# Drjay806/PRO-B-GAN

Measured on NVIDIA B200. Metric: generator+discriminator samples/sec (score_triplets pass, bf16 tensor-core mode), higher is better.
Workload: dtype bf16

## Files before the change

pro-b-gan_b200/csrc/gather.cuh:

```cuda
#pragma once
#include <cuda_bf16.h>
#include <stdint.h>

namespace pbg {

struct GatherParams {
  const float* node_emb;
  const float* rel_emb;
  long long N, R;
  int E, Z;
  const long long* heads; long long head_stride;
  const long long* rels;  long long rel_stride;
  const long long* tails; long long tail_stride;
  const float* h; const float* r; const float* t;
  const float* z;
  void* xg; int ldg;
  void* xd; int ldd;
  long long B;
  int* err_flag;
};

template <typename T>
__device__ __forceinline__ void store4(T* dst, float4 v);
template <>
__device__ __forceinline__ void store4<float>(float* dst, float4 v) {
  *reinterpret_cast<float4*>(dst) = v;
}
template <>
__device__ __forceinline__ void store4<__nv_bfloat16>(__nv_bfloat16* dst, float4 v) {
  __nv_bfloat162 lo = __floats2bfloat162_rn(v.x, v.y), hi = __floats2bfloat162_rn(v.z, v.w);
  uint2 w;
  w.x = *reinterpret_cast<uint32_t*>(&lo);
  w.y = *reinterpret_cast<uint32_t*>(&hi);
  *reinterpret_cast<uint2*>(dst) = w;
}

__device__ __forceinline__ float4 ld_stream4(const float* p) {
  float4 v;
  asm volatile("ld.global.nc.L1::no_allocate.v4.f32 {%0, %1, %2, %3}, [%4];"
               : "=f"(v.x), "=f"(v.y), "=f"(v.z), "=f"(v.w) : "l"(p));
  return v;
}

template <typename T>
__global__ void __launch_bounds__(256) gather_concat_kernel(const GatherParams p) {
  const int lane = threadIdx.x & 31;
  const long long warp_global = (static_cast<long long>(blockIdx.x) * blockDim.x + threadIdx.x) >> 5;
  const long long num_warps = (static_cast<long long>(gridDim.x) * blockDim.x) >> 5;
  const int E4 = p.E >> 2, Z4 = p.Z >> 2;
  T* xg = static_cast<T*>(p.xg);
  T* xd = static_cast<T*>(p.xd);

  for (long long b = warp_global; b < p.B; b += num_warps) {
    const float *hrow, *rrow, *trow = nullptr;
    bool bad = false;
    if (p.heads != nullptr) {
      long long i = p.heads[b * p.head_stride];
      if (i < 0) i += p.N;
      if (i < 0 || i >= p.N) { bad = true; i = 0; }
      hrow = p.node_emb + i * p.E;
    } else {
      hrow = p.h + b * p.E;
    }
    if (p.rels != nullptr) {
      long long i = p.rels[b * p.rel_stride];
      if (i < 0 || i >= p.R) { bad = true; i = 0; }
      rrow = p.rel_emb + i * p.E;
    } else {
      rrow = p.r + b * p.E;
    }
    if (p.tails != nullptr) {
      long long i = p.tails[b * p.tail_stride];
      if (i < 0) i += p.N;
      if (i < 0 || i >= p.N) { bad = true; i = 0; }
      trow = p.node_emb + i * p.E;
    } else if (xd != nullptr) {
      trow = p.t + b * p.E;
    }
    if (bad && lane == 0) atomicOr(p.err_flag, 1);

    T* g = xg ? xg + b * p.ldg : nullptr;
    T* d = xd ? xd + b * p.ldd : nullptr;
    for (int v = lane; v < E4; v += 32) {
      const float4 hv = ld_stream4(hrow + 4 * v);
      const float4 rv = ld_stream4(rrow + 4 * v);
      if (g) { store4<T>(g + 4 * v, hv); store4<T>(g + p.E + 4 * v, rv); }
      if (d) {
        store4<T>(d + 4 * v, hv);
        store4<T>(d + p.E + 4 * v, rv);
        store4<T>(d + 2 * p.E + 4 * v, ld_stream4(trow + 4 * v));
      }
    }
    if (g) {
      const float* zrow = p.z + b * p.Z;
      for (int v = lane; v < Z4; v += 32) store4<T>(g + 2 * p.E + 4 * v, ld_stream4(zrow + 4 * v));
      for (int v = (2 * p.E + p.Z) / 4 + lane; v < p.ldg / 4; v += 32)
        store4<T>(g + 4 * v, make_float4(0.f, 0.f, 0.f, 0.f));
    }
    if (d) {
      for (int v = (3 * p.E) / 4 + lane; v < p.ldd / 4; v += 32)
        store4<T>(d + 4 * v, make_float4(0.f, 0.f, 0.f, 0.f));
    }
  }
}

struct StageParams {
  GatherParams g;
  float* xt;
};
__global__ void __launch_bounds__(128, 12) stage_rows_kernel(const __grid_constant__ StageParams sp) {
  const int lane = threadIdx.x & 31;
  const long long warp_global = (static_cast<long long>(blockIdx.x) * blockDim.x + threadIdx.x) >> 5;
  const long long num_warps = (static_cast<long long>(gridDim.x) * blockDim.x) >> 5;
  const int E = sp.g.E, Z = sp.g.Z, E4 = E >> 2, Z4 = Z >> 2;
  const long long N = sp.g.N;
  __nv_bfloat16* const xg = static_cast<__nv_bfloat16*>(sp.g.xg);
  __nv_bfloat16* const xd = static_cast<__nv_bfloat16*>(sp.g.xd);
  for (long long b = warp_global; b < sp.g.B; b += num_warps) {
    bool bad = false;
    long long hi = sp.g.heads[b * 3], ri = sp.g.rels[b * 3], ti = sp.g.tails[b * 3];
    if (hi < 0) hi += N;
    if (ti < 0) ti += N;
    if (hi < 0 || hi >= N) { bad = true; hi = 0; }
    if (ri < 0 || ri >= sp.g.R) { bad = true; ri = 0; }
    if (ti < 0 || ti >= N) { bad = true; ti = 0; }
    if (bad && lane == 0) atomicOr(sp.g.err_flag, 1);
    const float* hrow = sp.g.node_emb + hi * E;
    const float* rrow = sp.g.rel_emb + ri * E;
    const float* trow = sp.g.node_emb + ti * E;
    __nv_bfloat16* g = xg ? xg + b * sp.g.ldg : nullptr;
    __nv_bfloat16* d = xd ? xd + b * sp.g.ldd : nullptr;
    for (int v = lane; v < E4; v += 32) {
      const float4 hv = ld_stream4(hrow + 4 * v);
      const float4 rv = ld_stream4(rrow + 4 * v);
      const float4 tv = ld_stream4(trow + 4 * v);
      if (g) {
        store4<__nv_bfloat16>(g + 4 * v, hv);
        store4<__nv_bfloat16>(g + E + 4 * v, rv);
      }
      if (d) {
        store4<__nv_bfloat16>(d + 4 * v, hv);
        store4<__nv_bfloat16>(d + E + 4 * v, rv);
        store4<__nv_bfloat16>(d + 2 * E + 4 * v, tv);
      }
      if (sp.xt) store4<float>(sp.xt + b * E + 4 * v, tv);
    }
    if (g) {
      for (int v = lane; v < Z4; v += 32) store4<__nv_bfloat16>(g + 2 * E + 4 * v, ld_stream4(sp.g.z + b * Z + 4 * v));
      for (int v = (2 * E + Z) / 4 + lane; v < sp.g.ldg / 4; v += 32)
        store4<__nv_bfloat16>(g + 4 * v, make_float4(0.f, 0.f, 0.f, 0.f));
    }
    if (d)
      for (int v = (3 * E) / 4 + lane; v < sp.g.ldd / 4; v += 32)
        store4<__nv_bfloat16>(d + 4 * v, make_float4(0.f, 0.f, 0.f, 0.f));
  }
}

__global__ void pack_bf16_kernel(const float* __restrict__ src, __nv_bfloat16* __restrict__ dst, int rows, int cols,
                                 int rows_p, int cols_p) {
  const long long total = static_cast<long long>(rows_p) * cols_p;
  for (long long i = static_cast<long long>(blockIdx.x) * blockDim.x + threadIdx.x; i < total;
       i += static_cast<long long>(gridDim.x) * blockDim.x) {
    const int r = static_cast<int>(i / cols_p), c = static_cast<int>(i % cols_p);
    dst[i] = __float2bfloat16_rn((r < rows && c < cols) ? src[static_cast<long long>(r) * cols + c] : 0.f);
  }
}

__global__ void pad_f32_kernel(const float* __restrict__ src, float* __restrict__ dst, int n, int n_p) {
  for (int i = blockIdx.x * blockDim.x + threadIdx.x; i < n_p; i += gridDim.x * blockDim.x)
    dst[i] = i < n ? src[i] : 0.f;
}

}
```

pro-b-gan_b200/csrc/pass2_kernel.cuh:

```cuda
#pragma once
#include <cuda.h>
#include "ptx.cuh"
#include "gather.cuh"
#include "tc_common.cuh"
#include "pass_common.cuh"

namespace pbg {

#ifndef PBG_STAGES
#define PBG_STAGES 5
#endif
#ifndef PBG_EPI_WARPS
#define PBG_EPI_WARPS 8
#endif
constexpr int kP2Stages = PBG_STAGES;
constexpr int kP2Epi = PBG_EPI_WARPS;
constexpr int kP2Slots = kP2Epi / 4;
constexpr int kP2Threads = 64 + 32 * kP2Epi;
static_assert(kP2Epi == 8 || kP2Epi == 16, "epilogue warps");
#ifndef PBG_ROLES_FIRST
#define PBG_ROLES_FIRST 0
#endif
constexpr int kProdWarp = PBG_ROLES_FIRST ? 0 : kP2Epi;
constexpr int kMmaWarp = PBG_ROLES_FIRST ? 1 : kP2Epi + 1;
constexpr int kEpiWarp0 = PBG_ROLES_FIRST ? 2 : 0;
constexpr int kTraceThread = kEpiWarp0 * 32;
#ifndef PBG_P2RING
#define PBG_P2RING 4
#endif
constexpr int kP2Ring = PBG_P2RING;
constexpr int kP2Rows = 256;
constexpr int kP2GroupsPerBlock = kP2Rows / 4;
constexpr int kP2GatherPerBlock = 4;
constexpr int kP2WarpsPerPair = 2 * kP2Epi;
constexpr int kMaxMirrors = 7;

#ifndef PBG_KB_PROBE
#define PBG_KB_PROBE 0
#endif
#if PBG_KB_PROBE
__device__ int g_probe_n;
#endif

struct P2Layer {
  int num_kb;
  int block_n;
  int n_tiles;
  int epi;
  int dep_kind;
  int out_kind;
  int ldo;
  int bias_off;
  const float* bias;
  __nv_bfloat16* out;
};

struct P2Segment { int kind, n_tiles, start, rb0, kind2, n_tiles2; };

struct alignas(64) Pass2Params {
  CUtensorMap tm_a[5];
  CUtensorMap tm_w[5];
  CUtensorMap tm_o[5];
  P2Layer layer[5];
  GatherParams gather;
  unsigned layer_mask;
  int gather_defer;
  int gather_external;
  int gather_ahead;
  int no_deps;
  int discard;
  const void* dead_xg;
  const void* dead_xd;
  int dead_ldg, dead_ldd;
  int poll_ns;
  int phase0_groups;
  int n_total;
  int n_seg;
  P2Segment seg[16];
  int nrb;
  int rb_cap;
  int M;
  float slope;
  PassSched* sched;
  int* ready;
  int* fin;
  void* gen_out; int out_f32; int n_valid; int ld_gen;
  float* cosine; const float* tail_tab; const long long* tail_idx; long long tail_stride; long long n_ent;
  float* part_g;
  int slots_g;
  const float* w3; float b3; float* logits; float* probs;
  int w3_off;
  float* part_d;
  int slots_d;
  int n_mirror;
  void* mir_gen[kMaxMirrors]; float* mir_cos[kMaxMirrors]; float* mir_logits[kMaxMirrors]; float* mir_probs[kMaxMirrors];
  void* mc_gen; float* mc_cos; float* mc_logits; float* mc_probs;
  long long* trace;
};
static_assert(sizeof(Pass2Params) <= 4096, "kernel parameter space");

struct P2Smem {
  static constexpr int kA = 128 * kBlockK * 2;
  static constexpr int kW = 128 * kBlockK * 2;
  static constexpr int kStage = kA + kW;
  static constexpr int kStagingOff = kP2Stages * kStage;
  static constexpr int kStagingPerWarp = 4096;
  static constexpr int kBiasOff = kStagingOff + kP2Epi * kStagingPerWarp;
  static constexpr int kBiasFloats = 6144;
  static constexpr int kBarOff = kBiasOff + kBiasFloats * 4;
  static constexpr int kXchgOff = kBarOff + 256;
  static constexpr int kXchgBytes = 4 * 32 * 3 * 4;
  static constexpr int kTotal = kXchgOff + kXchgBytes + 256 + 1024 ;
};
static_assert(P2Smem::kTotal <= 232448, "pass2: shared memory budget");

__device__ __forceinline__ void st_cluster_u32x2(uint32_t cluster_addr, uint2 v) {
  asm volatile("st.shared::cluster.v2.u32 [%0], {%1, %2};" ::"r"(cluster_addr), "r"(v.x), "r"(v.y) : "memory");
}
__device__ __forceinline__ void multimem_st_v4(void* mc_addr, uint4 v) {
  asm volatile("multimem.st.relaxed.sys.global.v4.f32 [%0], {%1, %2, %3, %4};" ::"l"(mc_addr), "f"(__uint_as_float(v.x)),
               "f"(__uint_as_float(v.y)), "f"(__uint_as_float(v.z)), "f"(__uint_as_float(v.w)) : "memory");
}
__device__ __forceinline__ void multimem_st_f32(float* mc_addr, float v) {
  asm volatile("multimem.st.relaxed.sys.global.f32 [%0], %1;" ::"l"(mc_addr), "f"(v) : "memory");
}
__device__ __forceinline__ float2 add2(float2 a, float2 b) {
  float2 d;
  asm("{\n\t.reg .b64 ra, rb, rd;\n\tmov.b64 ra, {%2, %3};\n\tmov.b64 rb, {%4, %5};\n\tadd.rn.f32x2 rd, ra, rb;\n\t"
      "mov.b64 {%0, %1}, rd;\n\t}\n"
      : "=f"(d.x), "=f"(d.y) : "f"(a.x), "f"(a.y), "f"(b.x), "f"(b.y));
  return d;
}
__device__ __forceinline__ float2 mul2(float2 a, float2 b) {
  float2 d;
  asm("{\n\t.reg .b64 ra, rb, rd;\n\tmov.b64 ra, {%2, %3};\n\tmov.b64 rb, {%4, %5};\n\tmul.rn.f32x2 rd, ra, rb;\n\t"
      "mov.b64 {%0, %1}, rd;\n\t}\n"
      : "=f"(d.x), "=f"(d.y) : "f"(a.x), "f"(a.y), "f"(b.x), "f"(b.y));
  return d;
}
__device__ __forceinline__ uint32_t bias_leaky_pack(uint32_t a0, uint32_t a1, float b0, float b1, float slope) {
  const float2 y = add2(make_float2(__uint_as_float(a0), __uint_as_float(a1)), make_float2(b0, b1));
  const float2 s = mul2(y, make_float2(slope, slope));
  return pack_bf16x2(fmaxf(y.x, s.x), fmaxf(y.y, s.y));
}

__device__ __forceinline__ int p2_dep_target(const Pass2Params& p, int dep_kind) {
  if (p.no_deps) return 0;
  if (dep_kind == DEP_X) return p.gather_external ? 0 : kP2GroupsPerBlock;
  const int producer = dep_kind == DEP_G0 ? IT_G_L0 : (dep_kind == DEP_D0 ? IT_D_L0 : IT_G_L1);
  return p.layer[producer].n_tiles * kP2WarpsPerPair;
}
__device__ __forceinline__ void p2_arrive(const Pass2Params& p, int dep_kind, int rb, int lane, bool async_stores,
                                          long long* t_wait = nullptr) {
  __syncwarp();
  if (lane == 0) {
    int* ctr = p.ready + dep_kind * p.rb_cap + rb;
    if (async_stores) {
      const long long t0 = t_wait ? clock64() : 0;
      tma_store_wait<0>();
      if (t_wait) *t_wait += clock64() - t0;
      red_relaxed_gpu_add(ctr, 1);
    } else {
      red_release_gpu_add(ctr, 1);
    }
  }
}
__device__ __forceinline__ void p2_arrive_done(const Pass2Params& p, int dep_kind, int rb, int lane) {
  if (lane == 0) red_relaxed_gpu_add(p.ready + dep_kind * p.rb_cap + rb, 1);
}
__device__ __forceinline__ void p2_poll_dep(const Pass2Params& p, int dep_kind, int rb) {
  const int target = p2_dep_target(p, dep_kind);
  const int* ctr = p.ready + dep_kind * p.rb_cap + rb;
  uint32_t spins = 0;
  while (ld_relaxed_gpu(ctr) < target) {
    __nanosleep(p.poll_ns);
#if PBG_HANG_GUARD
    if (++spins > 4000000u) pbg_wait_timed_out("dependency (kind, row block)", dep_kind, rb);
#endif
  }
  fence_proxy_async_all();
}

__device__ __forceinline__ void p2_discard(const void* base, size_t bytes, int part, int nparts, int lane) {
  const char* b = static_cast<const char*>(base);
  for (size_t off = static_cast<size_t>(part) * 4096 + static_cast<size_t>(lane) * 128; off < bytes; off += static_cast<size_t>(nparts) * 4096)
    asm volatile("discard.global.L2 [%0], 128;" ::"l"(b + off) : "memory");
}

__device__ __forceinline__ void p2_tail_load(float4 (&tv)[8], unsigned long long trow_bits, int col0, int n_valid, int lane) {
#pragma unroll
  for (int i = 0; i < 8; ++i) {
    const int r = i * 4 + (lane >> 3), t = lane & 7;
    const float* tp2 = reinterpret_cast<const float*>(__shfl_sync(0xffffffffu, trow_bits, r));
    tv[i] = make_float4(0.f, 0.f, 0.f, 0.f);
    if (tp2 != nullptr && col0 + t * 4 < n_valid) tv[i] = ld_stream4(tp2 + col0 + t * 4);
  }
}
__device__ __forceinline__ void p2_tail_stage(uint8_t* st, const float4 (&tv)[8], int lane) {
#pragma unroll
  for (int i = 0; i < 8; ++i) {
    const int r = i * 4 + (lane >> 3), t = lane & 7;
    *reinterpret_cast<float4*>(st + r * 128 + ((t ^ (r & 7)) << 4)) = tv[i];
  }
  __syncwarp();
}
__device__ __forceinline__ void p2_tail_dot(const uint8_t* st, const float* f, int col0, int n_valid, int lane, float& d, float& pp,
                                            float& tt) {
#pragma unroll
  for (int t = 0; t < 8; ++t) {
    const float4 x = *reinterpret_cast<const float4*>(st + lane * 128 + ((t ^ (lane & 7)) << 4));
    if (col0 + t * 4 < n_valid) {
      d += f[4 * t] * x.x + f[4 * t + 1] * x.y + f[4 * t + 2] * x.z + f[4 * t + 3] * x.w;
      pp += f[4 * t] * f[4 * t] + f[4 * t + 1] * f[4 * t + 1] + f[4 * t + 2] * f[4 * t + 2] + f[4 * t + 3] * f[4 * t + 3];
      tt += x.x * x.x + x.y * x.y + x.z * x.z + x.w * x.w;
    }
  }
  __syncwarp();
}

template <class F>
__device__ __forceinline__ void p2_gather_group_bulk(const GatherParams& g, long long group, int lane, uint8_t* st,
                                                     F&& before_staging, bool keep) {
  const long long r0 = group * 4;
  __nv_bfloat16* xg = static_cast<__nv_bfloat16*>(g.xg);
  __nv_bfloat16* xd = static_cast<__nv_bfloat16*>(g.xd);
  const float* src = nullptr;
  bool bad = false;
  if (lane < 12) {
    const long long row = r0 + lane / 3;
    const int which = lane % 3;
    if (row < g.B) {
      if (which == 0) {
        if (g.heads) { long long i = g.heads[row * g.head_stride]; if (i < 0) i += g.N; if (i < 0 || i >= g.N) { bad = true; i = 0; } src = g.node_emb + i * g.E; }
        else src = g.h + row * g.E;
      } else if (which == 1) {
        if (g.rels) { long long i = g.rels[row * g.rel_stride]; if (i < 0 || i >= g.R) { bad = true; i = 0; } src = g.rel_emb + i * g.E; }
        else src = g.r + row * g.E;
      } else if (g.tails) {
        long long i = g.tails[row * g.tail_stride]; if (i < 0) i += g.N; if (i < 0 || i >= g.N) { bad = true; i = 0; } src = g.node_emb + i * g.E;
      } else if (xd != nullptr) {
        src = g.t + row * g.E;
      }
    }
  }
  if (bad) atomicOr(g.err_flag, 1);
  const unsigned long long sp = reinterpret_cast<unsigned long long>(src);
  const int Z4 = g.Z >> 2;
  const int wg = 2 * g.E + g.Z, wd = 3 * g.E;
  float4 hv[4], rv[4], tv[4], zv[4];
#pragma unroll
  for (int j = 0; j < 4; ++j) {
    const float* ph = reinterpret_cast<const float*>(__shfl_sync(0xffffffffu, sp, j * 3 + 0));
    const float* pr = reinterpret_cast<const float*>(__shfl_sync(0xffffffffu, sp, j * 3 + 1));
    const float* pt = reinterpret_cast<const float*>(__shfl_sync(0xffffffffu, sp, j * 3 + 2));
    const long long row = r0 + j;
    hv[j] = rv[j] = tv[j] = zv[j] = make_float4(0.f, 0.f, 0.f, 0.f);
    if (row < g.B) {
      hv[j] = ld_stream4(ph + 4 * lane);
      rv[j] = ld_stream4(pr + 4 * lane);
      if (xd != nullptr) tv[j] = ld_stream4(pt + 4 * lane);
      if (xg != nullptr && lane < Z4) zv[j] = ld_stream4(g.z + row * g.Z + 4 * lane);
    }
  }
  before_staging();
  const long long nrow = min(4ll, g.B - r0);
  if (xg != nullptr) {
#pragma unroll
    for (int j = 0; j < 4; ++j) {
      __nv_bfloat16* o = reinterpret_cast<__nv_bfloat16*>(st) + j * wg;
      store4<__nv_bfloat16>(o + 4 * lane, hv[j]);
      store4<__nv_bfloat16>(o + g.E + 4 * lane, rv[j]);
      if (lane < Z4) store4<__nv_bfloat16>(o + 2 * g.E + 4 * lane, zv[j]);
    }
    fence_proxy_async_smem();
    __syncwarp();
    if (lane == 0 && nrow > 0) {
      if (keep) bulk_store_1d_hint(xg + r0 * wg, st, static_cast<uint32_t>(nrow * wg * 2), kEvictLast);
      else bulk_store_1d(xg + r0 * wg, st, static_cast<uint32_t>(nrow * wg * 2));
      tma_store_commit();
      if (xd != nullptr) tma_store_wait_read<0>();
    }
    __syncwarp();
  }
  if (xd != nullptr) {
#pragma unroll
    for (int j = 0; j < 4; ++j) {
      __nv_bfloat16* o = reinterpret_cast<__nv_bfloat16*>(st) + j * wd;
      store4<__nv_bfloat16>(o + 4 * lane, hv[j]);
      store4<__nv_bfloat16>(o + g.E + 4 * lane, rv[j]);
      store4<__nv_bfloat16>(o + 2 * g.E + 4 * lane, tv[j]);
    }
    fence_proxy_async_smem();
    __syncwarp();
    if (lane == 0 && nrow > 0) {
      if (keep) bulk_store_1d_hint(xd + r0 * wd, st, static_cast<uint32_t>(nrow * wd * 2), kEvictLast);
      else bulk_store_1d(xd + r0 * wd, st, static_cast<uint32_t>(nrow * wd * 2));
      tma_store_commit();
    }
  }
}

__device__ __forceinline__ uint32_t ring_dep(uint2 it) { return (it.x >> 24) << 3; }

template <bool TR, bool FASTG, bool BIASS>
__global__ void __cluster_dims__(2, 1, 1) __launch_bounds__(kP2Threads, 1)
pbg_pass2_kernel(const __grid_constant__ Pass2Params p) {
  using L = P2Smem;
  extern __shared__ uint8_t smem_raw[];
  uint8_t* smem = smem_raw + ((1024u - (smem_u32(smem_raw) & 1023u)) & 1023u);
  uint64_t* full_bar = reinterpret_cast<uint64_t*>(smem + L::kBarOff);
  uint64_t* empty_bar = full_bar + kP2Stages;
  uint64_t* tmem_full = empty_bar + kP2Stages;
  uint64_t* tmem_empty = tmem_full + 2;
  uint64_t* sched_full = tmem_empty + 2;
  uint64_t* sched_empty = sched_full + kP2Ring;
  uint64_t* bias_bar = sched_empty + kP2Ring;
  uint2* ring = reinterpret_cast<uint2*>(bias_bar + 1);
  uint32_t* tmem_slot = reinterpret_cast<uint32_t*>(ring + kP2Ring);
  int* last_flag = reinterpret_cast<int*>(tmem_slot + 1);
  volatile long long* t_issue = reinterpret_cast<volatile long long*>(smem + L::kXchgOff + L::kXchgBytes);
  float* xchg = reinterpret_cast<float*>(smem + L::kXchgOff);
  float* sbias = reinterpret_cast<float*>(smem + L::kBiasOff);

  const int warp = threadIdx.x >> 5;
  const int lane = threadIdx.x & 31;
  const uint32_t rank = cluster_ctarank();
  const bool leader = rank == 0;
  const long long t_entry = (TR && p.trace && threadIdx.x == 0) ? static_cast<long long>(globaltimer_ns()) : 0;
  asm volatile("griddepcontrol.launch_dependents;" ::: "memory");
  constexpr int kRingConsumers = 2 * (1 + kP2Epi) + 1;

  if (threadIdx.x == 0) {
    for (int i = 0; i < 5; ++i) {
      if (p.layer_mask & (1u << i)) {
        prefetch_tmap(&p.tm_a[i]);
        prefetch_tmap(&p.tm_w[i]);
        if (p.layer[i].epi == PEPI_STORE) prefetch_tmap(&p.tm_o[i]);
      }
    }
    for (int s = 0; s < kP2Stages; ++s) {
      mbar_init(&full_bar[s], 1);
      mbar_init(&empty_bar[s], 1);
    }
    for (int s = 0; s < 2; ++s) {
      mbar_init(&tmem_full[s], 1);
      mbar_init(&tmem_empty[s], kP2WarpsPerPair);
    }
    for (int s = 0; s < kP2Ring; ++s) {
      mbar_init(&sched_full[s], 1);
      mbar_init(&sched_empty[s], kRingConsumers);
    }
    mbar_init(bias_bar, 1);
    fence_mbar_init();
    if (BIASS) {
    uint32_t bytes = 0;
    for (int k = 0; k < 5; ++k)
      if (p.layer_mask & (1u << k)) bytes += static_cast<uint32_t>(p.layer[k].n_tiles * p.layer[k].block_n) * 4u;
    if (p.layer_mask & (1u << IT_D_L1)) bytes += static_cast<uint32_t>(p.layer[IT_D_L1].n_tiles * p.layer[IT_D_L1].block_n) * 4u;
    mbar_arrive_expect_tx(bias_bar, bytes);
    for (int k = 0; k < 5; ++k)
      if (p.layer_mask & (1u << k))
        bulk_load_1d(sbias + p.layer[k].bias_off, p.layer[k].bias, static_cast<uint32_t>(p.layer[k].n_tiles * p.layer[k].block_n) * 4u, bias_bar);
    if (p.layer_mask & (1u << IT_D_L1))
      bulk_load_1d(sbias + p.w3_off, p.w3, static_cast<uint32_t>(p.layer[IT_D_L1].n_tiles * p.layer[IT_D_L1].block_n) * 4u, bias_bar);
    }
  }
  if (warp == kMmaWarp) tmem_alloc_pair<512>(tmem_slot);
  tc_fence_before();
  __syncthreads();
  cluster_sync_all();
  tc_fence_after();
  asm volatile("griddepcontrol.wait;" ::: "memory");
  const uint32_t tmem_base = *tmem_slot;
  long long* const clk0 = reinterpret_cast<long long*>(smem + L::kXchgOff + L::kXchgBytes) + 8;
  if (blockIdx.x == 0 && threadIdx.x == 0) { clk0[0] = clock64(); clk0[1] = static_cast<long long>(globaltimer_ns()); }
  long long* const tr = (TR && p.trace) ? p.trace + kTraceSlots * blockIdx.x : nullptr;
  if (tr && threadIdx.x == 0) { tr[0] = clock64(); tr[14] = static_cast<long long>(globaltimer_ns()); tr[254] = t_entry; }

  const uint32_t lead_tmem_empty = mapa_u32(smem_u32(tmem_empty), 0);
  const uint32_t sched_empty_addr = mapa_u32(smem_u32(sched_empty), 1);
  const uint32_t ring_addr = mapa_u32(smem_u32(ring), 1);
  if (warp == kMmaWarp && !leader) {
    if (lane == 0) {
      uint32_t slot = 0, sphase = 0;
      const uint32_t lead_sched_full = mapa_u32(smem_u32(sched_full), 0);
      for (;;) {
        const int ticket = atomicAdd(&p.sched->q_head, 1);
        uint2 it = make_uint2(IT_END, 0u);
        if (ticket < p.n_total) {
          int sg = 0;
          while (sg + 1 < p.n_seg && ticket >= p.seg[sg + 1].start) ++sg;
          const int i = ticket - p.seg[sg].start;
          const int nt1 = p.seg[sg].n_tiles, nt = nt1 + p.seg[sg].n_tiles2;
          const int j = i % nt;
          it = make_uint2(static_cast<uint32_t>(j < nt1 ? p.seg[sg].kind : p.seg[sg].kind2) | (static_cast<uint32_t>(j < nt1 ? j : j - nt1) << 8),
                          static_cast<uint32_t>(p.seg[sg].rb0 + i / nt));
        }
        if ((it.x & 0xff) != IT_END) p2_poll_dep(p, p.layer[it.x & 0xff].dep_kind, static_cast<int>(it.y));
        mbar_wait_role(&sched_empty[slot], sphase ^ 1);
        ring[slot] = it;
        mbar_arrive(&sched_full[slot]);
        mbar_arrive_cluster(lead_sched_full + slot * 8);
        if (++slot == kP2Ring) { slot = 0; sphase ^= 1; }
        if ((it.x & 0xff) == IT_END) break;
      }
    }
    __syncwarp();
  } else if (warp == kProdWarp) {
    if (lane == 0) {
      uint32_t stage = 0, phase = 0, slot = 0, sphase = 0;
      long long w_dep = 0, w_empty = 0, n_items = 0;
      const uint32_t lead_full = mapa_u32(smem_u32(full_bar), 0);
      for (;;) {
        mbar_wait_role(&sched_full[slot], sphase);
        const uint2 it = ld_cluster_u32x2(ring_addr + slot * 8);
        mbar_arrive_remote(sched_empty_addr + slot * 8 + ring_dep(it));
        if (++slot == kP2Ring) { slot = 0; sphase ^= 1; }
        const int kind = it.x & 0xff;
        if (kind == IT_END) break;
        long long* ti = (tr && n_items < kTraceItems) ? tr + 16 + 4 * n_items : nullptr;
        if (ti) { ti[0] = (clock64() << 20) | (static_cast<long long>(it.y & 0xfff) << 8) | kind; }
        ++n_items;
        const int n_blk = (it.x >> 8) & 0xff;
        const int rb = static_cast<int>(it.y);
        const P2Layer& ly = p.layer[kind];
        const int w_rows = ly.block_n >> 1;
        const uint32_t bytes_pair = 2u * (L::kA + static_cast<uint32_t>(w_rows) * kBlockK * 2);
        const int a_row = rb * kP2Rows + static_cast<int>(rank) * 128;
        const int w_row = n_blk * ly.block_n + static_cast<int>(rank) * w_rows;
        for (int kb = 0; kb < ly.num_kb; ++kb) {
          if (tr) { const long long t = clock64(); mbar_wait_role(&empty_bar[stage], phase ^ 1); w_empty += clock64() - t; }
          else mbar_wait_role(&empty_bar[stage], phase ^ 1);
          uint8_t* sa = smem + stage * L::kStage;
          if (leader) mbar_arrive_expect_tx(&full_bar[stage], bytes_pair);
          if (tr) t_issue[stage] = clock64();
          tma_load_2d_pair(sa + L::kA, &p.tm_w[kind], lead_full + stage * 8, kb * kBlockK, w_row);
          tma_load_2d_pair(sa, &p.tm_a[kind], lead_full + stage * 8, kb * kBlockK, a_row);
          if (++stage == kP2Stages) { stage = 0; phase ^= 1; }
        }
      }
      if (tr) { tr[1] = w_empty; tr[2] = clock64(); tr[12] = n_items; if (leader) tr[11] = w_dep; }
    }
    __syncwarp();
  } else if (warp == kMmaWarp) {
    if (lane == 0) {
      uint32_t stage = 0, phase = 0, acc = 0, acc_phase = 0, slot = 0, sphase = 0;
      long long w_full = 0, w_tmem = 0, w_item = 0, n_kb = 0, lat_sum = 0, lat_n = 0, lat_max = 0;
      int n_it = 0;
#if PBG_KB_PROBE
      long long pr_clk[5] = {0, 0, 0, 0, 0}, pr_item = 0, pr_tmem = 0;
      int pr_tiles[5] = {0, 0, 0, 0, 0};
      const long long pr_begin = clock64();
#endif
      for (;;) {
#if PBG_KB_PROBE
        const long long pr_t0 = clock64();
#endif
        if (tr) { const long long t = clock64(); mbar_wait_role(&sched_full[slot], sphase); w_item += clock64() - t; }
        else mbar_wait_role(&sched_full[slot], sphase);
        const uint2 it = ld_cluster_u32x2(ring_addr + slot * 8);
        mbar_arrive_remote(sched_empty_addr + slot * 8 + ring_dep(it));
        if (++slot == kP2Ring) { slot = 0; sphase ^= 1; }
        const int kind = it.x & 0xff;
        if (kind == IT_END) break;
        const P2Layer& ly = p.layer[kind];
        const uint32_t idesc = make_idesc_bf16(kP2Rows, static_cast<uint32_t>(ly.block_n));
#if PBG_KB_PROBE
        const long long pr_t1 = clock64();
#endif
        if (tr) { const long long t = clock64(); mbar_wait_role(&tmem_empty[acc], acc_phase ^ 1); w_tmem += clock64() - t; }
        else mbar_wait_role(&tmem_empty[acc], acc_phase ^ 1);
        tc_fence_after();
#if PBG_KB_PROBE
        const long long pr_t2 = clock64();
        pr_item += pr_t1 - pr_t0; pr_tmem += pr_t2 - pr_t1;
#endif
        if (tr && n_it < kTraceItems) tr[16 + 4 * n_it + 1] = clock64();
        ++n_it;
        const uint32_t d_tmem = tmem_base + acc * 256;
        for (int kb = 0; kb < ly.num_kb; ++kb) {
          if (tr) {
            const long long t = clock64(); mbar_wait_role(&full_bar[stage], phase); const long long t1 = clock64();
            w_full += t1 - t; ++n_kb;
            const long long lat = t1 - t_issue[stage];
            if (t1 - t > 64) { lat_sum += lat; lat_n += 1; if (lat > lat_max) lat_max = lat; }
          } else mbar_wait_role(&full_bar[stage], phase);
          tc_fence_after();
          const uint32_t sa = smem_u32(smem + stage * L::kStage);
          const uint64_t da = make_kmajor_sw128_desc(sa);
          const uint64_t db = make_kmajor_sw128_desc(sa + L::kA);
#pragma unroll
          for (int k = 0; k < kBlockK / kUmmaK; ++k) umma_bf16_pair(d_tmem, da + 2 * k, db + 2 * k, idesc, (kb | k) != 0);
          umma_commit_pair(&empty_bar[stage], 3);
          if (++stage == kP2Stages) { stage = 0; phase ^= 1; }
        }
        umma_commit_pair(&tmem_full[acc], 3);
        if (++acc == 2) { acc = 0; acc_phase ^= 1; }
#if PBG_KB_PROBE
        pr_clk[kind] += clock64() - pr_t2; pr_tiles[kind] += 1;
#endif
      }
#if PBG_KB_PROBE
      {
        const int n = atomicAdd(&g_probe_n, 1), npairs = static_cast<int>(gridDim.x) / 2, pair = static_cast<int>(blockIdx.x) / 2;
        if (n / npairs == 30 && (pair == 0 || pair == npairs / 2 || pair == npairs - 1))
          printf("probe pair %d of %d (M=%d): MMA thread lifetime %lld clk; waiting for an item %lld, for a free accumulator %lld; "
                 "k-block loops (tiles: clk per tile) G.L0 %d: %lld  D.L0 %d: %lld  G.L1 %d: %lld  D.L1 %d: %lld  G.L2 %d: %lld\n",
                 pair, npairs, p.M, clock64() - pr_begin, pr_item, pr_tmem,
                 pr_tiles[0], pr_tiles[0] ? pr_clk[0] / pr_tiles[0] : 0, pr_tiles[1], pr_tiles[1] ? pr_clk[1] / pr_tiles[1] : 0,
                 pr_tiles[2], pr_tiles[2] ? pr_clk[2] / pr_tiles[2] : 0, pr_tiles[3], pr_tiles[3] ? pr_clk[3] / pr_tiles[3] : 0,
                 pr_tiles[4], pr_tiles[4] ? pr_clk[4] / pr_tiles[4] : 0);
      }
#endif
      if (tr) { tr[3] = w_full; tr[4] = w_tmem; tr[6] = clock64(); tr[9] = n_kb; tr[15] = w_item; tr[237] = lat_sum; tr[238] = lat_n; tr[239] = lat_max; }
    }
    __syncwarp();
  } else {
    const int wep = warp - kEpiWarp0;
    const int q = warp & 3;
    const int half = wep >> 2;
    uint8_t* st = smem + L::kStagingOff + (q * kP2Slots + half) * L::kStagingPerWarp;
    uint32_t acc = 0, acc_phase = 0, slot = 0, sphase = 0;
    long long w_acc = 0, busy = 0, ph_wr = 0, ph_ld = 0, ph_math = 0, ph_st = 0, ph_n = 0, ph_m1 = 0, ph_w2 = 0;
    int item_no = 0;
    const int row_in_blk = static_cast<int>(rank) * 128 + q * 32 + lane;
    bool more_groups = true;
    int pend_rb = -1;
    auto gather_flush = [&]() {
      if (pend_rb >= 0) {
        if (lane == 0) { tma_store_wait<0>(); if (!p.gather_ahead) red_relaxed_gpu_add(p.ready + DEP_X * p.rb_cap + pend_rb, 1); }
        __syncwarp();
        pend_rb = -1;
      }
    };
    auto gather_one = [&]() {
      int g = 0;
      if (lane == 0) g = atomicAdd(&p.sched->p0_next, 1);
      g = __shfl_sync(0xffffffffu, g, 0);
      if (g >= p.phase0_groups) { more_groups = false; return; }
      if (tr && threadIdx.x == kTraceThread) tr[249] = clock64();
      if (FASTG) {
        p2_gather_group_bulk(p.gather, g, lane, st, gather_flush, p.gather_ahead != 0);
        if (tr && threadIdx.x == kTraceThread) tr[250] = clock64();
        pend_rb = static_cast<int>(g / kP2GroupsPerBlock);
        if (!p.gather_defer) gather_flush();
      } else {
        pass_gather_group<2>(p.gather, g, lane);
        if (tr && threadIdx.x == kTraceThread) tr[250] = clock64();
        if (!p.gather_ahead) p2_arrive(p, DEP_X, g / kP2GroupsPerBlock, lane, false);
        else __syncwarp();
      }
    };
    if (!p.gather_ahead) {
      gather_one();
      gather_flush();
    }
    bool bias_ok = !BIASS;
    long long pf_wait = 0, pf_total = 0, pf_n = 0;
    bool pair_pending = false;
    auto pair_settle = [&]() {
      if (pair_pending) {
        if (half == 0 && lane == 0) tma_store_wait_read<0>();
        asm volatile("bar.sync %0, 64;" ::"r"(5 + q) : "memory");
        pair_pending = false;
      }
    };
    for (;;) {
      pair_settle();
      while (more_groups && !__all_sync(0xffffffffu, mbar_test_wait(&sched_full[slot], sphase))) gather_one();
      gather_flush();
      mbar_wait(&sched_full[slot], sphase);
      const uint2 it = ld_cluster_u32x2(ring_addr + slot * 8);
      __syncwarp();
      if (lane == 0) mbar_arrive_remote(sched_empty_addr + slot * 8 + ring_dep(it));
      if (++slot == kP2Ring) { slot = 0; sphase ^= 1; }
      const int kind = it.x & 0xff;
      if (kind == IT_END) break;
      while (more_groups && !__all_sync(0xffffffffu, mbar_test_wait(&tmem_full[acc], acc_phase))) gather_one();
      gather_flush();
      if (tr && threadIdx.x == kTraceThread && tr[5] == 0) tr[5] = clock64();
      if (!bias_ok) { mbar_wait(bias_bar, 0); bias_ok = true; }
      const int n_blk = (it.x >> 8) & 0xff;
      const int rb = static_cast<int>(it.y);
      long long* ti = (tr && threadIdx.x == kTraceThread && item_no < kTraceItems) ? tr + 16 + 4 * item_no : nullptr;
      ++item_no;
      const P2Layer& ly = p.layer[kind];
      const long long grow = static_cast<long long>(rb) * kP2Rows + row_in_blk;
      const bool row_ok = grow < p.M;
      const int n0 = n_blk * ly.block_n;
      const int n_chunks = ly.block_n >> 6;
      const uint32_t taddr = tmem_base + (static_cast<uint32_t>(q * 32) << 16) + acc * 256;

      const bool want_cos = ly.epi == PEPI_TANH && p.cosine != nullptr;
      unsigned long long trow_bits = 0ull;
      float4 tv2[8];
      if (want_cos) {
        const float* trow = nullptr;
        if (row_ok) {
          if (p.tail_idx != nullptr) {
            long long tid = p.tail_idx[grow * p.tail_stride];
            if (tid < 0) tid += p.n_ent;
            tid = (tid < 0 || tid >= p.n_ent) ? 0 : tid;
            trow = p.tail_tab + tid * p.n_valid;
          } else {
            trow = p.tail_tab + grow * p.n_valid;
          }
        }
        trow_bits = reinterpret_cast<unsigned long long>(trow);
        if (half < n_chunks) {
          float4 tv1[8];
          p2_tail_load(tv1, trow_bits, n0 + half * 64, p.n_valid, lane);
          p2_tail_load(tv2, trow_bits, n0 + half * 64 + 32, p.n_valid, lane);
          p2_tail_stage(st, tv1, lane);
        }
      }
      {
        const long long t = (tr && lane == 0) ? clock64() : 0;
        mbar_wait(&tmem_full[acc], acc_phase);
        if (tr && lane == 0) { w_acc += clock64() - t; }
        if (ti) ti[2] = clock64();
      }
      const long long t_busy0 = (tr && lane == 0) ? clock64() : 0;
      tc_fence_after();

      if (ly.epi == PEPI_STORE) {
        const bool tp = tr && threadIdx.x == kTraceThread;
        long long tq0 = 0, tq1 = 0, tq2 = 0, tq3 = 0, tq4 = 0, tq5 = 0, tq6 = 0;
        const float slope = p.slope;
        const float* const bias_tile = (BIASS ? sbias + ly.bias_off : ly.bias) + n0;
        const int row0 = rb * kP2Rows + static_cast<int>(rank) * 128 + q * 32;
        uint32_t va[32], vb[32];
        if (half < n_chunks) tmem_ld_32x32_ptr(taddr + half * 64, va);
        for (int c = half; c < n_chunks; c += kP2Slots) {
          if (tp) tq0 = clock64();
          const float4* b4 = reinterpret_cast<const float4*>(bias_tile + c * 64);
          if (tp) tq1 = clock64();
          uint8_t* sbuf = st;
          tmem_ld_wait();
          tmem_ld_32x32_ptr(taddr + c * 64 + 32, vb);
          if (tp) tq2 = clock64();
          {
            float4 bq[8];
#pragma unroll
            for (int t = 0; t < 8; ++t) bq[t] = b4[t];
            uint4 w[4];
#pragma unroll
            for (int t = 0; t < 4; ++t) {
              const float4 ba = bq[2 * t], bb = bq[2 * t + 1];
              w[t].x = bias_leaky_pack(va[8 * t + 0], va[8 * t + 1], ba.x, ba.y, slope);
              w[t].y = bias_leaky_pack(va[8 * t + 2], va[8 * t + 3], ba.z, ba.w, slope);
              w[t].z = bias_leaky_pack(va[8 * t + 4], va[8 * t + 5], bb.x, bb.y, slope);
              w[t].w = bias_leaky_pack(va[8 * t + 6], va[8 * t + 7], bb.z, bb.w, slope);
            }
            if (lane == 0) tma_store_wait_read<0>();
            __syncwarp();
#pragma unroll
            for (int t = 0; t < 4; ++t) *reinterpret_cast<uint4*>(sbuf + lane * 128 + ((t ^ (lane & 7)) << 4)) = w[t];
          }
          float4 bq[8];
#pragma unroll
          for (int t = 0; t < 8; ++t) bq[t] = b4[8 + t];
          if (tp) tq5 = clock64();
          tmem_ld_wait();
          if (tp) tq6 = clock64();
          if (c + kP2Slots < n_chunks) {
            tmem_ld_32x32_ptr(taddr + (c + kP2Slots) * 64, va);
          } else {
            tc_fence_before();
            __syncwarp();
            if (lane == 0) mbar_arrive_remote(lead_tmem_empty + acc * 8);
          }
#pragma unroll
          for (int t = 0; t < 4; ++t) {
            const float4 ba = bq[2 * t], bb = bq[2 * t + 1];
            uint4 w;
            w.x = bias_leaky_pack(vb[8 * t + 0], vb[8 * t + 1], ba.x, ba.y, slope);
            w.y = bias_leaky_pack(vb[8 * t + 2], vb[8 * t + 3], ba.z, ba.w, slope);
            w.z = bias_leaky_pack(vb[8 * t + 4], vb[8 * t + 5], bb.x, bb.y, slope);
            w.w = bias_leaky_pack(vb[8 * t + 6], vb[8 * t + 7], bb.z, bb.w, slope);
            *reinterpret_cast<uint4*>(sbuf + lane * 128 + (((4 + t) ^ (lane & 7)) << 4)) = w;
          }
          if (tp) tq3 = clock64();
          fence_proxy_async_smem();
          __syncwarp();
          if (lane == 0) {
            tma_store_2d(&p.tm_o[kind], sbuf, n0 + c * 64, row0);
            tma_store_commit();
          }
          if (tp) { tq4 = clock64(); ph_wr += tq1 - tq0; ph_ld += tq2 - tq1; ph_math += tq3 - tq2; ph_st += tq4 - tq3; ph_n += 1; ph_m1 += tq5 - tq2; ph_w2 += tq6 - tq5; }
        }
        if (half >= n_chunks) {
          tc_fence_before();
          __syncwarp();
          if (lane == 0) mbar_arrive_remote(lead_tmem_empty + acc * 8);
        }
        {
          const long long t0 = (tr && threadIdx.x == kTraceThread) ? clock64() : 0;
          p2_arrive(p, ly.out_kind, rb, lane, true, (tr && threadIdx.x == kTraceThread) ? &pf_wait : nullptr);
          if (tr && threadIdx.x == kTraceThread) { pf_total += clock64() - t0; pf_n += 1; }
        }
        if (p.discard && kind == IT_G_L1 && n_blk == 0 && p.dead_xg != nullptr)
          p2_discard(static_cast<const char*>(p.dead_xg) + static_cast<size_t>(rb) * kP2Rows * p.dead_ldg * 2,
                     static_cast<size_t>(kP2Rows) * p.dead_ldg * 2, static_cast<int>(rank) * kP2Epi + wep, kP2WarpsPerPair, lane);
      } else if (ly.epi == PEPI_ROWDOT) {
        const float slope = p.slope;
        float* part = p.part_d + (static_cast<size_t>(rb) * p.slots_d) * kP2Rows;
        for (int c = half; c < n_chunks; c += kP2Slots) {
          uint32_t v[64];
          tmem_ld_32x32_ptr(taddr + c * 64, v);
          tmem_ld_32x32_ptr(taddr + c * 64 + 32, v + 32);
          const float4* b4 = reinterpret_cast<const float4*>((BIASS ? sbias + ly.bias_off : ly.bias) + n0 + c * 64);
          const float4* w4 = reinterpret_cast<const float4*>((BIASS ? sbias + p.w3_off : p.w3) + n0 + c * 64);
          tmem_ld_wait();
          if (c + kP2Slots >= n_chunks) {
            tc_fence_before();
            __syncwarp();
            if (lane == 0) mbar_arrive_remote(lead_tmem_empty + acc * 8);
          }
          float rowdot = 0.f;
#pragma unroll
          for (int j = 0; j < 16; ++j) {
            const float4 b = b4[j], w = w4[j];
            rowdot = fmaf(leaky_max(__uint_as_float(v[4 * j + 0]) + b.x, slope), w.x, rowdot);
            rowdot = fmaf(leaky_max(__uint_as_float(v[4 * j + 1]) + b.y, slope), w.y, rowdot);
            rowdot = fmaf(leaky_max(__uint_as_float(v[4 * j + 2]) + b.z, slope), w.z, rowdot);
            rowdot = fmaf(leaky_max(__uint_as_float(v[4 * j + 3]) + b.w, slope), w.w, rowdot);
          }
          part[((n0 >> 6) + c) * kP2Rows + row_in_blk] = rowdot;
        }
        if (half >= n_chunks) {
          tc_fence_before();
          __syncwarp();
          if (lane == 0) mbar_arrive_remote(lead_tmem_empty + acc * 8);
        }
        if (p.discard && n_blk == 0 && p.dead_xd != nullptr)
          p2_discard(static_cast<const char*>(p.dead_xd) + static_cast<size_t>(rb) * kP2Rows * p.dead_ldd * 2,
                     static_cast<size_t>(kP2Rows) * p.dead_ldd * 2, static_cast<int>(rank) * kP2Epi + wep, kP2WarpsPerPair, lane);
        const int old = warp_publish_fetch(p.fin + FIN_D * p.rb_cap + rb, lane);
        if (old == ly.n_tiles * kP2WarpsPerPair - 1) {
          fence_acq_rel_gpu();
          __syncwarp();
          if (p.discard)
            p2_discard(reinterpret_cast<const char*>(p.layer[IT_D_L0].out) + static_cast<size_t>(rb) * kP2Rows * p.layer[IT_D_L0].ldo * 2,
                       static_cast<size_t>(kP2Rows) * p.layer[IT_D_L0].ldo * 2, 0, 1, lane);
          float s[kP2Rows / 32];
#pragma unroll
          for (int j = 0; j < kP2Rows / 32; ++j) s[j] = 0.f;
          for (int k = 0; k < p.slots_d; ++k) {
            float x[kP2Rows / 32];
#pragma unroll
            for (int j = 0; j < kP2Rows / 32; ++j) x[j] = __ldcg(part + k * kP2Rows + j * 32 + lane);
#pragma unroll
            for (int j = 0; j < kP2Rows / 32; ++j) s[j] += x[j];
          }
#pragma unroll
          for (int j = 0; j < kP2Rows / 32; ++j) {
            const long long gr = static_cast<long long>(rb) * kP2Rows + j * 32 + lane;
            if (gr < p.M) {
              const float logit = s[j] + p.b3;
              const float prob = 1.f / (1.f + __expf(-logit));
              p.logits[gr] = logit;
              if (p.probs != nullptr) p.probs[gr] = prob;
              for (int mi = 0; mi < p.n_mirror; ++mi) {
                p.mir_logits[mi][gr] = logit;
                if (p.mir_probs[mi] != nullptr) p.mir_probs[mi][gr] = prob;
              }
              if (p.mc_logits != nullptr) multimem_st_f32(p.mc_logits + gr, logit);
              if (p.mc_probs != nullptr) multimem_st_f32(p.mc_probs + gr, prob);
            }
          }
        }
      } else {
        const bool tpt = tr && threadIdx.x == kTraceThread;
        if (tpt) tr[232] = clock64();
        const bool want_out = p.gen_out != nullptr;
        const bool in_cta = ly.n_tiles == 1 && n_chunks == 2;
        float* part = p.part_g + (static_cast<size_t>(rb) * p.slots_g) * 3 * kP2Rows;
        for (int c = half; c < n_chunks; c += kP2Slots) {
          const int col0 = n0 + c * 64;
          if (want_cos && c != half) {
            float4 tv1[8];
            p2_tail_load(tv1, trow_bits, col0, p.n_valid, lane);
            p2_tail_load(tv2, trow_bits, col0 + 32, p.n_valid, lane);
            p2_tail_stage(st, tv1, lane);
          }
          uint32_t v[64];
          tmem_ld_32x32_ptr(taddr + c * 64, v);
          tmem_ld_32x32_ptr(taddr + c * 64 + 32, v + 32);
          const float4* b4 = reinterpret_cast<const float4*>((BIASS ? sbias + ly.bias_off : ly.bias) + col0);
          tmem_ld_wait();
          if (c + kP2Slots >= n_chunks) {
            tc_fence_before();
            __syncwarp();
            if (lane == 0) mbar_arrive_remote(lead_tmem_empty + acc * 8);
          }
          float* f = reinterpret_cast<float*>(v);
          if (tpt) tr[233] = clock64();
#pragma unroll
          for (int j = 0; j < 16; ++j) {
            const float4 b = b4[j];
            f[4 * j + 0] = tanh_fast(f[4 * j + 0] + b.x);
            f[4 * j + 1] = tanh_fast(f[4 * j + 1] + b.y);
            f[4 * j + 2] = tanh_fast(f[4 * j + 2] + b.z);
            f[4 * j + 3] = tanh_fast(f[4 * j + 3] + b.w);
          }
          if (tpt) tr[234] = clock64();
          if (want_cos) {
            float cs_dot = 0.f, cs_pp = 0.f, cs_tt = 0.f;
            p2_tail_dot(st, f, col0, p.n_valid, lane, cs_dot, cs_pp, cs_tt);
            p2_tail_stage(st, tv2, lane);
            p2_tail_dot(st, f + 32, col0 + 32, p.n_valid, lane, cs_dot, cs_pp, cs_tt);
            if (tpt) tr[245] = clock64();
            if (in_cta) {
              float* xq = xchg + (q * 32 + lane) * 3;
              if (half == 1) { xq[0] = cs_dot; xq[1] = cs_pp; xq[2] = cs_tt; }
              asm volatile("bar.sync %0, 64;" ::"r"(1 + q) : "memory");
              if (tpt) tr[255] = clock64();
              if (half == 0) {
                const float d = cs_dot + xq[0], pp = cs_pp + xq[1], tt = cs_tt + xq[2];
                if (row_ok) {
                  const float cs = d / (fmaxf(sqrtf(pp), 1e-8f) * fmaxf(sqrtf(tt), 1e-8f));
                  p.cosine[grow] = cs;
                  for (int mi = 0; mi < p.n_mirror; ++mi) p.mir_cos[mi][grow] = cs;
                  if (p.mc_cos != nullptr) multimem_st_f32(p.mc_cos + grow, cs);
                }
              }
              asm volatile("bar.sync %0, 64;" ::"r"(1 + q) : "memory");
            } else if (col0 < p.n_valid) {
              float* mine = part + (col0 >> 6) * 3 * kP2Rows;
              mine[row_in_blk] = cs_dot;
              mine[kP2Rows + row_in_blk] = cs_pp;
              mine[2 * kP2Rows + row_in_blk] = cs_tt;
            }
          }
          if (tpt) tr[235] = clock64();
          const bool bulk_mirror = p.n_mirror > 0 && (p.n_valid & 63) == 0;
          const bool pair_out = want_out && in_cta && !p.out_f32 && p.n_valid == 128 && p.ld_gen == 128;
          if (want_out && row_ok && !pair_out) {
            for (int mi = -1; mi < (bulk_mirror ? 0 : p.n_mirror); ++mi) {
              void* base = mi < 0 ? p.gen_out : p.mir_gen[mi];
              if (p.out_f32) {
                float* orow = static_cast<float*>(base) + grow * p.ld_gen + col0;
#pragma unroll
                for (int t = 0; t < 16; ++t)
                  if (col0 + t * 4 < p.n_valid)
                    *reinterpret_cast<float4*>(orow + t * 4) = make_float4(f[4 * t], f[4 * t + 1], f[4 * t + 2], f[4 * t + 3]);
              } else {
                __nv_bfloat16* orow = static_cast<__nv_bfloat16*>(base) + grow * p.ld_gen + col0;
#pragma unroll
                for (int t = 0; t < 8; ++t) {
                  uint4 w;
                  w.x = pack_bf16x2(f[8 * t + 0], f[8 * t + 1]);
                  w.y = pack_bf16x2(f[8 * t + 2], f[8 * t + 3]);
                  w.z = pack_bf16x2(f[8 * t + 4], f[8 * t + 5]);
                  w.w = pack_bf16x2(f[8 * t + 6], f[8 * t + 7]);
                  if (col0 + t * 8 < p.n_valid) *reinterpret_cast<uint4*>(orow + t * 8) = w;
                }
              }
            }
            if (p.mc_gen != nullptr) {
              if (p.out_f32) {
                char* orow = static_cast<char*>(p.mc_gen) + (static_cast<size_t>(grow) * p.ld_gen + col0) * 4;
#pragma unroll
                for (int t = 0; t < 16; ++t)
                  if (col0 + t * 4 < p.n_valid)
                    multimem_st_v4(orow + t * 16, make_uint4(__float_as_uint(f[4 * t]), __float_as_uint(f[4 * t + 1]),
                                                             __float_as_uint(f[4 * t + 2]), __float_as_uint(f[4 * t + 3])));
              } else {
                char* orow = static_cast<char*>(p.mc_gen) + (static_cast<size_t>(grow) * p.ld_gen + col0) * 2;
#pragma unroll
                for (int t = 0; t < 8; ++t) {
                  uint4 w;
                  w.x = pack_bf16x2(f[8 * t + 0], f[8 * t + 1]);
                  w.y = pack_bf16x2(f[8 * t + 2], f[8 * t + 3]);
                  w.z = pack_bf16x2(f[8 * t + 4], f[8 * t + 5]);
                  w.w = pack_bf16x2(f[8 * t + 6], f[8 * t + 7]);
                  if (col0 + t * 8 < p.n_valid) multimem_st_v4(orow + t * 16, w);
                }
              }
            }
            if (bulk_mirror && col0 < p.n_valid) {
              uint8_t* myrow = st + lane * 128;
              const int rounds = p.out_f32 ? 2 : 1;
              for (int rd = 0; rd < rounds; ++rd) {
                tma_store_wait_read<0>();
                if (p.out_f32) {
#pragma unroll
                  for (int t = 0; t < 8; ++t)
                    *reinterpret_cast<float4*>(myrow + t * 16) =
                        make_float4(f[32 * rd + 4 * t], f[32 * rd + 4 * t + 1], f[32 * rd + 4 * t + 2], f[32 * rd + 4 * t + 3]);
                } else {
#pragma unroll
                  for (int t = 0; t < 8; ++t) {
                    uint4 w;
                    w.x = pack_bf16x2(f[8 * t + 0], f[8 * t + 1]);
                    w.y = pack_bf16x2(f[8 * t + 2], f[8 * t + 3]);
                    w.z = pack_bf16x2(f[8 * t + 4], f[8 * t + 5]);
                    w.w = pack_bf16x2(f[8 * t + 6], f[8 * t + 7]);
                    *reinterpret_cast<uint4*>(myrow + t * 16) = w;
                  }
                }
                fence_proxy_async_smem();
                const size_t es = p.out_f32 ? 4 : 2;
                const size_t byte_off = (static_cast<size_t>(grow) * p.ld_gen + col0) * es + static_cast<size_t>(rd) * 128;
                for (int mi = 0; mi < p.n_mirror; ++mi) bulk_store_1d(static_cast<char*>(p.mir_gen[mi]) + byte_off, myrow, 128);
                tma_store_commit();
              }
            }
          }
          if (pair_out) {
            uint8_t* region = smem + L::kStagingOff + q * kP2Slots * L::kStagingPerWarp;
            asm volatile("bar.sync %0, 64;" ::"r"(5 + q) : "memory");
#pragma unroll
            for (int t = 0; t < 8; ++t) {
              uint4 w;
              w.x = pack_bf16x2(f[8 * t + 0], f[8 * t + 1]);
              w.y = pack_bf16x2(f[8 * t + 2], f[8 * t + 3]);
              w.z = pack_bf16x2(f[8 * t + 4], f[8 * t + 5]);
              w.w = pack_bf16x2(f[8 * t + 6], f[8 * t + 7]);
              *reinterpret_cast<uint4*>(region + lane * 256 + half * 128 + t * 16) = w;
            }
            fence_proxy_async_smem();
            asm volatile("bar.sync %0, 64;" ::"r"(5 + q) : "memory");
            if (half == 0 && lane == 0) {
              const long long row0 = grow - lane;
              const long long nrows = min(32ll, p.M - row0);
              if (nrows > 0) {
                bulk_store_1d(static_cast<char*>(p.gen_out) + row0 * 256, region, static_cast<uint32_t>(nrows * 256));
                for (int mi = 0; mi < p.n_mirror; ++mi)
                  bulk_store_1d(static_cast<char*>(p.mir_gen[mi]) + row0 * 256, region, static_cast<uint32_t>(nrows * 256));
                tma_store_commit();
              }
            }
            if (p.mc_gen != nullptr) {
              const long long row0 = grow - lane;
              const int nbytes = static_cast<int>(min(32ll, p.M - row0)) * 256;
              char* dst = static_cast<char*>(p.mc_gen) + row0 * 256;
#pragma unroll
              for (int i = 0; i < 8; ++i) {
                const int off = (i * 64 + half * 32 + lane) * 16;
                if (off < nbytes) multimem_st_v4(dst + off, *reinterpret_cast<const uint4*>(region + off));
              }
            }
            pair_pending = true;
          }
          if (want_out && p.n_mirror > 0 && !pair_out) {
            tma_store_wait_read<0>();
            __syncwarp();
          }
        }
        if (half >= n_chunks) {
          tc_fence_before();
          __syncwarp();
          if (lane == 0) mbar_arrive_remote(lead_tmem_empty + acc * 8);
        }
        if (p.discard && ly.n_tiles == 1) {
          const int part = static_cast<int>(rank) * kP2Epi + wep;
          p2_discard(reinterpret_cast<const char*>(p.layer[IT_G_L0].out) + static_cast<size_t>(rb) * kP2Rows * p.layer[IT_G_L0].ldo * 2,
                     static_cast<size_t>(kP2Rows) * p.layer[IT_G_L0].ldo * 2, part, kP2WarpsPerPair, lane);
          p2_discard(reinterpret_cast<const char*>(p.layer[IT_G_L1].out) + static_cast<size_t>(rb) * kP2Rows * p.layer[IT_G_L1].ldo * 2,
                     static_cast<size_t>(kP2Rows) * p.layer[IT_G_L1].ldo * 2, part, kP2WarpsPerPair, lane);
        }
        if (tpt) tr[236] = clock64();
        if (want_cos && !in_cta) {
          const int old = warp_publish_fetch(p.fin + FIN_G * p.rb_cap + rb, lane);
          if (old == ly.n_tiles * kP2WarpsPerPair - 1) {
            fence_acq_rel_gpu();
            __syncwarp();
            for (int r = lane; r < kP2Rows; r += 32) {
              const long long gr = static_cast<long long>(rb) * kP2Rows + r;
              float d = 0.f, pp = 0.f, tt = 0.f;
              for (int k = 0; k < p.slots_g; ++k) {
                d += __ldcg(part + (k * 3 + 0) * kP2Rows + r);
                pp += __ldcg(part + (k * 3 + 1) * kP2Rows + r);
                tt += __ldcg(part + (k * 3 + 2) * kP2Rows + r);
              }
              if (gr < p.M) {
                const float cs = d / (fmaxf(sqrtf(pp), 1e-8f) * fmaxf(sqrtf(tt), 1e-8f));
                p.cosine[gr] = cs;
                for (int mi = 0; mi < p.n_mirror; ++mi) p.mir_cos[mi][gr] = cs;
                if (p.mc_cos != nullptr) multimem_st_f32(p.mc_cos + gr, cs);
              }
            }
          }
        }
      }
      if (tr && lane == 0) busy += clock64() - t_busy0;
      if (ti) ti[3] = clock64();
      if (++acc == 2) { acc = 0; acc_phase ^= 1; }
    }
    if (p.gather_ahead) {
      pair_settle();
      while (more_groups) gather_one();
      gather_flush();
    }
    tma_store_wait_read<0>();
    if (tr && threadIdx.x == kTraceThread) {
      tr[7] = w_acc; tr[8] = clock64(); tr[10] = busy;
      tr[240] = ph_ld; tr[241] = ph_math; tr[242] = ph_st; tr[243] = ph_n; tr[244] = ph_wr;
      tr[251] = ph_m1; tr[252] = ph_w2;
      tr[246] = pf_wait; tr[247] = pf_total; tr[248] = pf_n;
    }
  }

  tc_fence_before();
  __syncthreads();
  cluster_sync_all();
  if (warp == kMmaWarp) {
    tc_fence_after();
    tmem_dealloc_pair<512>(tmem_base);
  }
  if (blockIdx.x == 0 && threadIdx.x == 0) {
    p.sched->clk_ticks = clock64() - clk0[0];
    p.sched->clk_ns = static_cast<long long>(globaltimer_ns()) - clk0[1];
  }
  if (threadIdx.x == 0) {
    const int old = atomicAdd(&p.sched->done, 1);
    *last_flag = (old == static_cast<int>(gridDim.x) - 1);
  }
  __syncthreads();
  if (*last_flag) {
    for (int k = 0; k < DEP_KINDS; ++k)
      for (int i = threadIdx.x; i < p.nrb; i += blockDim.x) p.ready[k * p.rb_cap + i] = 0;
    for (int k = 0; k < FIN_KINDS; ++k)
      for (int i = threadIdx.x; i < p.nrb; i += blockDim.x) p.fin[k * p.rb_cap + i] = 0;
    if (threadIdx.x == 0) { p.sched->q_head = 0; p.sched->q_tail = 0; p.sched->p0_next = 0; p.sched->init = 0; p.sched->done = 0; }
    if (tr && threadIdx.x == 0) { tr[13] = clock64(); tr[253] = static_cast<long long>(globaltimer_ns()); }
  }
}

}
```

pro-b-gan_b200/csrc/pass_common.cuh:

```cuda
#pragma once
#include <cuda.h>
#include "ptx.cuh"
#include "gather.cuh"
#include "tc_common.cuh"

namespace pbg {

enum : int { IT_G_L0 = 0, IT_D_L0 = 1, IT_G_L1 = 2, IT_D_L1 = 3, IT_G_L2 = 4, IT_GATHER = 5, IT_END = 255 };
enum : int { DEP_X = 0, DEP_G0 = 1, DEP_D0 = 2, DEP_G1 = 3, DEP_KINDS = 4 };
enum : int { FIN_G = 0, FIN_D = 1, FIN_KINDS = 2 };
enum : int { PEPI_STORE = 0, PEPI_TANH = 1, PEPI_ROWDOT = 2 };

constexpr int kEpiWarps = 8;
constexpr int kPassThreads = 64 + 32 * kEpiWarps;
constexpr int kTraceSlots = 256;
constexpr int kTraceItems = 54;


struct PassSched {
  int q_head;
  int q_tail;
  int p0_next;
  int init;
  int done;
  int pad_;
  long long clk_ticks, clk_ns;
};



__device__ __forceinline__ int ld_relaxed_gpu(const int* p) {
  int v;
  asm volatile("ld.relaxed.gpu.global.s32 %0, [%1];" : "=r"(v) : "l"(p) : "memory");
  return v;
}
__device__ __forceinline__ void fence_acq_rel_gpu() { asm volatile("fence.acq_rel.gpu;" ::: "memory"); }
__device__ __forceinline__ void red_release_gpu_add(int* p, int v) {
  asm volatile("red.release.gpu.global.add.s32 [%0], %1;" ::"l"(p), "r"(v) : "memory");
}
__device__ __forceinline__ void red_relaxed_gpu_add(int* p, int v) {
  asm volatile("red.relaxed.gpu.global.add.s32 [%0], %1;" ::"l"(p), "r"(v) : "memory");
}
__device__ __forceinline__ int atom_relaxed_gpu_add(int* p, int v) {
  int old;
  asm volatile("atom.relaxed.gpu.global.add.s32 %0, [%1], %2;" : "=r"(old) : "l"(p), "r"(v) : "memory");
  return old;
}
__device__ __forceinline__ int atom_release_gpu_add(int* p, int v) {
  int old;
  asm volatile("atom.release.gpu.global.add.s32 %0, [%1], %2;" : "=r"(old) : "l"(p), "r"(v) : "memory");
  return old;
}
__device__ __forceinline__ unsigned long long globaltimer_ns() {
  unsigned long long t;
  asm volatile("mov.u64 %0, %%globaltimer;" : "=l"(t));
  return t;
}
__device__ __forceinline__ void fence_proxy_async_all() { asm volatile("fence.proxy.async;" ::: "memory"); }

__device__ __forceinline__ void tmem_ld_32x32_ptr(uint32_t taddr, uint32_t* v) {
  asm volatile(
      "tcgen05.ld.sync.aligned.32x32b.x32.b32 "
      "{%0, %1, %2, %3, %4, %5, %6, %7, %8, %9, %10, %11, %12, %13, %14, %15, "
      "%16, %17, %18, %19, %20, %21, %22, %23, %24, %25, %26, %27, %28, %29, %30, %31}, [%32];"
      : "=r"(v[0]), "=r"(v[1]), "=r"(v[2]), "=r"(v[3]), "=r"(v[4]), "=r"(v[5]), "=r"(v[6]), "=r"(v[7]),
        "=r"(v[8]), "=r"(v[9]), "=r"(v[10]), "=r"(v[11]), "=r"(v[12]), "=r"(v[13]), "=r"(v[14]), "=r"(v[15]),
        "=r"(v[16]), "=r"(v[17]), "=r"(v[18]), "=r"(v[19]), "=r"(v[20]), "=r"(v[21]), "=r"(v[22]), "=r"(v[23]),
        "=r"(v[24]), "=r"(v[25]), "=r"(v[26]), "=r"(v[27]), "=r"(v[28]), "=r"(v[29]), "=r"(v[30]), "=r"(v[31])
      : "r"(taddr)
      : "memory");
}

__device__ __forceinline__ float leaky_max(float x, float slope) { return fmaxf(x, x * slope); }

template <int MODE = 0>
__device__ __forceinline__ void pass_gather_group(const GatherParams& g, long long group, int lane) {
  const long long r0 = group * 4;
  __nv_bfloat16* xg = static_cast<__nv_bfloat16*>(g.xg);
  __nv_bfloat16* xd = static_cast<__nv_bfloat16*>(g.xd);
  const float* src = nullptr;
  bool bad = false;
  if (lane < 12) {
    const long long row = r0 + lane / 3;
    const int which = lane % 3;
    if (row < g.B) {
      if (which == 0) {
        if (g.heads) { long long i = g.heads[row * g.head_stride]; if (i < 0) i += g.N; if (i < 0 || i >= g.N) { bad = true; i = 0; } src = g.node_emb + i * g.E; }
        else src = g.h + row * g.E;
      } else if (which == 1) {
        if (g.rels) { long long i = g.rels[row * g.rel_stride]; if (i < 0 || i >= g.R) { bad = true; i = 0; } src = g.rel_emb + i * g.E; }
        else src = g.r + row * g.E;
      } else if (g.tails) {
        long long i = g.tails[row * g.tail_stride]; if (i < 0) i += g.N; if (i < 0 || i >= g.N) { bad = true; i = 0; } src = g.node_emb + i * g.E;
      } else if (xd != nullptr) {
        src = g.t + row * g.E;
      }
    }
  }
  if (bad) atomicOr(g.err_flag, 1);
  const unsigned long long sp = reinterpret_cast<unsigned long long>(src);
  const int E4 = g.E >> 2, Z4 = g.Z >> 2;
  if (MODE == 1 || (MODE == 0 && E4 == 32 && Z4 <= 32)) {
    float4 hv[4], rv[4], tv[4], zv[4];
#pragma unroll
    for (int j = 0; j < 4; ++j) {
      const float* ph = reinterpret_cast<const float*>(__shfl_sync(0xffffffffu, sp, j * 3 + 0));
      const float* pr = reinterpret_cast<const float*>(__shfl_sync(0xffffffffu, sp, j * 3 + 1));
      const float* pt = reinterpret_cast<const float*>(__shfl_sync(0xffffffffu, sp, j * 3 + 2));
      const long long row = r0 + j;
      hv[j] = rv[j] = tv[j] = zv[j] = make_float4(0.f, 0.f, 0.f, 0.f);
      if (row < g.B) {
        hv[j] = ld_stream4(ph + 4 * lane);
        rv[j] = ld_stream4(pr + 4 * lane);
        if (xd != nullptr) tv[j] = ld_stream4(pt + 4 * lane);
        if (xg != nullptr && lane < Z4) zv[j] = ld_stream4(g.z + row * g.Z + 4 * lane);
      }
    }
#pragma unroll
    for (int j = 0; j < 4; ++j) {
      const long long row = r0 + j;
      if (row >= g.B) continue;
      if (xg != nullptr) {
        __nv_bfloat16* o = xg + row * g.ldg;
        store4<__nv_bfloat16>(o + 4 * lane, hv[j]);
        store4<__nv_bfloat16>(o + g.E + 4 * lane, rv[j]);
        if (lane < Z4) store4<__nv_bfloat16>(o + 2 * g.E + 4 * lane, zv[j]);
        for (int v = (2 * g.E + g.Z) / 4 + lane; v < g.ldg / 4; v += 32)
          store4<__nv_bfloat16>(o + 4 * v, make_float4(0.f, 0.f, 0.f, 0.f));
      }
      if (xd != nullptr) {
        __nv_bfloat16* o = xd + row * g.ldd;
        store4<__nv_bfloat16>(o + 4 * lane, hv[j]);
        store4<__nv_bfloat16>(o + g.E + 4 * lane, rv[j]);
        store4<__nv_bfloat16>(o + 2 * g.E + 4 * lane, tv[j]);
        for (int v = (3 * g.E) / 4 + lane; v < g.ldd / 4; v += 32)
          store4<__nv_bfloat16>(o + 4 * v, make_float4(0.f, 0.f, 0.f, 0.f));
      }
    }
  } else {
    for (int j = 0; j < 4; ++j) {
      const float* ph = reinterpret_cast<const float*>(__shfl_sync(0xffffffffu, sp, j * 3 + 0));
      const float* pr = reinterpret_cast<const float*>(__shfl_sync(0xffffffffu, sp, j * 3 + 1));
      const float* pt = reinterpret_cast<const float*>(__shfl_sync(0xffffffffu, sp, j * 3 + 2));
      const long long row = r0 + j;
      if (row >= g.B) continue;
      __nv_bfloat16* og = xg ? xg + row * g.ldg : nullptr;
      __nv_bfloat16* od = xd ? xd + row * g.ldd : nullptr;
      for (int v = lane; v < E4; v += 32) {
        const float4 h4 = ld_stream4(ph + 4 * v), r4 = ld_stream4(pr + 4 * v);
        if (og) { store4<__nv_bfloat16>(og + 4 * v, h4); store4<__nv_bfloat16>(og + g.E + 4 * v, r4); }
        if (od) {
          store4<__nv_bfloat16>(od + 4 * v, h4);
          store4<__nv_bfloat16>(od + g.E + 4 * v, r4);
          store4<__nv_bfloat16>(od + 2 * g.E + 4 * v, ld_stream4(pt + 4 * v));
        }
      }
      if (og) {
        for (int v = lane; v < Z4; v += 32) store4<__nv_bfloat16>(og + 2 * g.E + 4 * v, ld_stream4(g.z + row * g.Z + 4 * v));
        for (int v = (2 * g.E + g.Z) / 4 + lane; v < g.ldg / 4; v += 32)
          store4<__nv_bfloat16>(og + 4 * v, make_float4(0.f, 0.f, 0.f, 0.f));
      }
      if (od)
        for (int v = (3 * g.E) / 4 + lane; v < g.ldd / 4; v += 32)
          store4<__nv_bfloat16>(od + 4 * v, make_float4(0.f, 0.f, 0.f, 0.f));
    }
  }
}

__device__ __forceinline__ void warp_publish(int* counter, int lane) {
  __syncwarp();
  if (lane == 0) red_release_gpu_add(counter, 1);
}
__device__ __forceinline__ int warp_publish_fetch(int* counter, int lane) {
  __syncwarp();
  int old = 0;
  if (lane == 0) old = atom_release_gpu_add(counter, 1);
  return __shfl_sync(0xffffffffu, old, 0);
}


}
```

pro-b-gan_b200/csrc/pbg.cu:

```cuda
#include <cuda.h>
#include <cuda_runtime.h>
#include <cuda_bf16.h>

#include <algorithm>
#include <cstdarg>
#include <cstdio>
#include <cstring>
#include <cstdlib>
#include <map>
#include <tuple>
#include <new>
#include <string>
#include <vector>

#include "../../include/pbg.h"
#include "gather.cuh"
#include "gemm_f32.cuh"
#include "tc_common.cuh"
#include "pass_common.cuh"
#include "pass2_kernel.cuh"
#include "topk_kernel.cuh"
#include "index_rows.cuh"
#include "json_out.cuh"
#include "latent.cuh"

using namespace pbg;

namespace {

constexpr long long kMaxChunk = 65536;
constexpr int kPartSlotsG = 16;
constexpr int kPartSlotsD = 64;

inline int round_up(int v, int m) { return (v + m - 1) / m * m; }

struct Linear {
  int n = 0, k = 0;
  int np = 0, kp = 0;
  float* w_f32 = nullptr;
  float* b_f32 = nullptr;
  __nv_bfloat16* w_bf16 = nullptr;
  float* b_pad = nullptr;
  CUtensorMap tmap_w128;
  CUtensorMap tmap_w64;
};

struct Workspace {
  long long rows = 0;
  void *xg0 = nullptr, *xd0 = nullptr, *bufA = nullptr, *bufB = nullptr, *bufD = nullptr;
  CUtensorMap tm_xg0, tm_xd0, tm_bufA_g, tm_bufA_d, tm_bufB_g, tm_bufD_d;
  CUtensorMap tmo_bufA, tmo_bufB, tmo_bufD;
  int mb_cap = 0;
  int* ready = nullptr;
  int* fin = nullptr;
  PassSched* sched = nullptr;
  float* part_g = nullptr;
  float* part_d = nullptr;
};

struct TopkState {
  const float* table = nullptr; long long N = 0, n_pad = 0;
  __nv_bfloat16* tn = nullptr; float* inv_t = nullptr; CUtensorMap tm_t;
  long long q_cap = 0; __nv_bfloat16* qn = nullptr; float* inv_q = nullptr; CUtensorMap tm_q;
  size_t cand_cap = 0; unsigned* cand_grp = nullptr; unsigned* cand_mask = nullptr; int* cand_cnt = nullptr;
  size_t samp_cap = 0; int* samp_keys = nullptr;
  float* tau = nullptr; int* flag = nullptr;
  long long last_rows = 0; bool last_filtered = false;
  size_t score_cap = 0; float* score_buf = nullptr;
};

struct StageSlot {
  long long cap = 0;
  void *xg0 = nullptr, *xd0 = nullptr;
  float* xt = nullptr;
  float* z = nullptr;
  CUtensorMap tm_xg0, tm_xd0;
  long long B = -1;
  bool has_g = false, has_d = false;
  bool has_xt = false;
  const float* node_emb = nullptr; long long N = 0; const long long* tails = nullptr;
};

thread_local std::string g_create_error;

typedef CUresult (*EncodeTiledFn)(CUtensorMap*, CUtensorMapDataType, cuuint32_t, void*, const cuuint64_t*,
                                  const cuuint64_t*, const cuuint32_t*, const cuuint32_t*, CUtensorMapInterleave,
                                  CUtensorMapSwizzle, CUtensorMapL2promotion, CUtensorMapFloatOOBfill);

}

struct pbg_ctx {
  pbg_dims dims{};
  int num_sms = 0;
  int max_threads_sm = 0;
  bool g_loaded = false, d_loaded = false;
  int kg0 = 0, kg0p = 0, kd0 = 0, kd0p = 0, hgp = 0, hdp = 0, hd2 = 0, hmax = 0;
  Linear g[3], d[2];
  float* d_w3 = nullptr;
  float* d_w3_pad = nullptr;
  float d_b3 = 0.f;
  Workspace ws_bf16, ws_f32;
  StageSlot stage[2];
  int* err_flag = nullptr;
  int* err_flag_host = nullptr;
  cudaStream_t own_stream = nullptr;
  long long host_cap = 0;
  char* st_block = nullptr;
  EncodeTiledFn encode = nullptr;
  TopkState tk;
  bool lat_on = false;
  unsigned long long lat_seed = 0;
  LatentStream* lat_st = nullptr;
  long long lat_cap = 0;
  float* lat_z = nullptr;
  long long launches = 0;
  int launch_ctas = 0;
  int discard = 1;
  bool host_block = false;
  cudaEvent_t host_evt = nullptr;
  int n_mirror = 0;
  void* mir_gen[kMaxMirrors] = {}; float* mir_cos[kMaxMirrors] = {}; float* mir_logits[kMaxMirrors] = {}; float* mir_probs[kMaxMirrors] = {};
  void* mc_gen = nullptr; float *mc_cos = nullptr, *mc_logits = nullptr, *mc_probs = nullptr;
  bool profiling = false;
  long long* trace = nullptr;
  struct ProfRec { cudaEvent_t a, b; int kind; };
  std::vector<ProfRec> prof;
  std::string err;
};

namespace {

int fail(pbg_ctx* c, int code, const char* fmt, ...) {
  char buf[512];
  va_list ap;
  va_start(ap, fmt);
  vsnprintf(buf, sizeof buf, fmt, ap);
  va_end(ap);
  if (c) c->err = buf; else g_create_error = buf;
  return code;
}

struct LaunchScope {
  pbg_ctx* c; cudaStream_t s; cudaEvent_t b = nullptr;
  LaunchScope(pbg_ctx* c_, int kind, cudaStream_t s_) : c(c_), s(s_) {
    c->launches += 1;
    if (c->profiling) {
      cudaEvent_t a;
      cudaEventCreate(&a); cudaEventCreate(&b);
      cudaEventRecord(a, s);
      c->prof.push_back({a, b, kind});
    }
  }
  ~LaunchScope() { if (b) cudaEventRecord(b, s); }
};

#define PBG_CUDA(c, expr)                                                                               \
  do {                                                                                                  \
    cudaError_t e_ = (expr);                                                                            \
    if (e_ != cudaSuccess) return fail((c), PBG_ERR_CUDA, "%s failed: %s", #expr, cudaGetErrorString(e_)); \
  } while (0)

#define PBG_TRY(expr)            \
  do {                           \
    int s_ = (expr);             \
    if (s_ != PBG_OK) return s_; \
  } while (0)

int make_tmap(pbg_ctx* c, CUtensorMap* tm, const void* base, long long rows, int cols, int box_rows) {
  cuuint64_t dims[2] = {static_cast<cuuint64_t>(cols), static_cast<cuuint64_t>(rows)};
  cuuint64_t strides[1] = {static_cast<cuuint64_t>(cols) * 2};
  cuuint32_t box[2] = {static_cast<cuuint32_t>(kBlockK), static_cast<cuuint32_t>(box_rows)};
  cuuint32_t estr[2] = {1, 1};
  CUresult r = c->encode(tm, CU_TENSOR_MAP_DATA_TYPE_BFLOAT16, 2, const_cast<void*>(base), dims, strides, box, estr,
                         CU_TENSOR_MAP_INTERLEAVE_NONE, CU_TENSOR_MAP_SWIZZLE_128B, CU_TENSOR_MAP_L2_PROMOTION_L2_256B,
                         CU_TENSOR_MAP_FLOAT_OOB_FILL_NONE);
  if (r != CUDA_SUCCESS) return fail(c, PBG_ERR_CUDA, "cuTensorMapEncodeTiled failed (%d) rows=%lld cols=%d", (int)r, rows, cols);
  return PBG_OK;
}

void free_linear(Linear& l) {
  cudaFree(l.w_f32); cudaFree(l.b_f32); cudaFree(l.w_bf16); cudaFree(l.b_pad);
  l = Linear{};
}

void free_ws(Workspace& w) {
  cudaFree(w.xg0); cudaFree(w.xd0); cudaFree(w.bufA); cudaFree(w.bufB); cudaFree(w.bufD);
  cudaFree(w.ready); cudaFree(w.fin); cudaFree(w.sched); cudaFree(w.part_g); cudaFree(w.part_d);
  w = Workspace{};
}

int upload_linear(pbg_ctx* c, Linear& l, int n, int k, int kp, const float* w_host, const float* b_host) {
  free_linear(l);
  l.n = n; l.k = k; l.kp = kp;
  l.np = round_up(n, 128);
  PBG_CUDA(c, cudaMalloc(&l.w_f32, sizeof(float) * n * k));
  PBG_CUDA(c, cudaMalloc(&l.b_f32, sizeof(float) * n));
  PBG_CUDA(c, cudaMalloc(&l.w_bf16, sizeof(__nv_bfloat16) * (size_t)l.np * l.kp));
  PBG_CUDA(c, cudaMalloc(&l.b_pad, sizeof(float) * l.np));
  PBG_CUDA(c, cudaMemcpyAsync(l.w_f32, w_host, sizeof(float) * n * k, cudaMemcpyHostToDevice, c->own_stream));
  PBG_CUDA(c, cudaMemcpyAsync(l.b_f32, b_host, sizeof(float) * n, cudaMemcpyHostToDevice, c->own_stream));
  { LaunchScope ls(c, PBG_K_OTHER, c->own_stream);
    pack_bf16_kernel<<<c->num_sms * 4, 256, 0, c->own_stream>>>(l.w_f32, l.w_bf16, n, k, l.np, l.kp); }
  { LaunchScope ls(c, PBG_K_OTHER, c->own_stream);
    pad_f32_kernel<<<8, 256, 0, c->own_stream>>>(l.b_f32, l.b_pad, n, l.np); }
  PBG_CUDA(c, cudaGetLastError());
  PBG_CUDA(c, cudaStreamSynchronize(c->own_stream));
  PBG_TRY(make_tmap(c, &l.tmap_w128, l.w_bf16, l.np, l.kp, 128));
  return make_tmap(c, &l.tmap_w64, l.w_bf16, l.np, l.kp, 64);
}

int begin_growth(pbg_ctx* c, cudaStream_t s, const char* what) {
  cudaStreamCaptureStatus st = cudaStreamCaptureStatusNone;
  if (cudaStreamIsCapturing(s, &st) == cudaSuccess && st != cudaStreamCaptureStatusNone)
    return fail(c, PBG_ERR_INVALID, "%s must grow while the stream is being captured: call pbg_reserve() first", what);
  PBG_CUDA(c, cudaDeviceSynchronize());
  return PBG_OK;
}

long long pow2_cap(long long rows) {
  long long cap = 1024;
  while (cap < rows) cap *= 2;
  return std::min(cap, kMaxChunk);
}

template <class T>
int realloc_dev(pbg_ctx* c, T*& p, size_t bytes) {
  cudaFree(p); p = nullptr;
  PBG_CUDA(c, cudaMalloc(&p, bytes));
  return PBG_OK;
}

void free_stage(StageSlot& st) {
  cudaFree(st.xg0); cudaFree(st.xd0); cudaFree(st.xt); cudaFree(st.z);
  st = StageSlot{};
}

int ensure_ws(pbg_ctx* c, int prec, long long rows, cudaStream_t stream) {
  Workspace& w = prec == PBG_PREC_BF16 ? c->ws_bf16 : c->ws_f32;
  if (w.rows >= rows) return PBG_OK;
  PBG_TRY(begin_growth(c, stream, "the workspace"));
  const long long cap = pow2_cap(rows);
  free_ws(w);
  if (prec == PBG_PREC_BF16) {
    const size_t es = sizeof(__nv_bfloat16);
    PBG_CUDA(c, cudaMalloc(&w.xg0, es * cap * c->kg0p));
    PBG_CUDA(c, cudaMalloc(&w.xd0, es * cap * c->kd0p));
    PBG_CUDA(c, cudaMalloc(&w.bufA, es * cap * c->hmax));
    PBG_CUDA(c, cudaMalloc(&w.bufB, es * cap * c->hmax));
    PBG_CUDA(c, cudaMalloc(&w.bufD, es * cap * c->hdp));
    PBG_TRY(make_tmap(c, &w.tm_bufD_d, w.bufD, cap, c->hdp, kBlockM));
    PBG_TRY(make_tmap(c, &w.tmo_bufA, w.bufA, cap, c->hgp, 32));
    PBG_TRY(make_tmap(c, &w.tmo_bufB, w.bufB, cap, c->hgp, 32));
    PBG_TRY(make_tmap(c, &w.tmo_bufD, w.bufD, cap, c->hdp, 32));
    w.mb_cap = static_cast<int>(cap / kBlockM);
    PBG_CUDA(c, cudaMalloc(&w.ready, sizeof(int) * DEP_KINDS * w.mb_cap));
    PBG_CUDA(c, cudaMalloc(&w.fin, sizeof(int) * FIN_KINDS * w.mb_cap));
    PBG_CUDA(c, cudaMalloc(&w.sched, sizeof(PassSched)));
    PBG_CUDA(c, cudaMalloc(&w.part_g, sizeof(float) * w.mb_cap * kPartSlotsG * 3 * kBlockM));
    PBG_CUDA(c, cudaMalloc(&w.part_d, sizeof(float) * w.mb_cap * kPartSlotsD * kBlockM));
    PBG_CUDA(c, cudaMemset(w.ready, 0, sizeof(int) * DEP_KINDS * w.mb_cap));
    PBG_CUDA(c, cudaMemset(w.fin, 0, sizeof(int) * FIN_KINDS * w.mb_cap));
    PBG_CUDA(c, cudaMemset(w.sched, 0, sizeof(PassSched)));
    PBG_TRY(make_tmap(c, &w.tm_xg0, w.xg0, cap, c->kg0p, kBlockM));
    PBG_TRY(make_tmap(c, &w.tm_xd0, w.xd0, cap, c->kd0p, kBlockM));
    PBG_TRY(make_tmap(c, &w.tm_bufA_g, w.bufA, cap, c->hgp, kBlockM));
    PBG_TRY(make_tmap(c, &w.tm_bufA_d, w.bufA, cap, c->hdp, kBlockM));
    PBG_TRY(make_tmap(c, &w.tm_bufB_g, w.bufB, cap, c->hgp, kBlockM));
  } else {
    const size_t es = sizeof(float);
    const int hm = std::max(std::max(c->dims.g_hidden, c->dims.d_hidden), c->dims.embed_dim);
    PBG_CUDA(c, cudaMalloc(&w.xg0, es * cap * c->kg0));
    PBG_CUDA(c, cudaMalloc(&w.xd0, es * cap * c->kd0));
    PBG_CUDA(c, cudaMalloc(&w.bufA, es * cap * hm));
    PBG_CUDA(c, cudaMalloc(&w.bufB, es * cap * hm));
  }
  w.rows = cap;
  return PBG_OK;
}

int ensure_stage(pbg_ctx* c, StageSlot& st, long long rows, cudaStream_t stream) {
  if (st.cap >= rows) return PBG_OK;
  PBG_TRY(begin_growth(c, stream, "a staging slot"));
  const long long cap = pow2_cap(rows);
  free_stage(st);
  const size_t es = sizeof(__nv_bfloat16);
  PBG_CUDA(c, cudaMalloc(&st.xg0, es * cap * c->kg0p));
  PBG_CUDA(c, cudaMalloc(&st.xd0, es * cap * c->kd0p));
  PBG_CUDA(c, cudaMalloc(&st.xt, sizeof(float) * cap * c->dims.embed_dim));
  PBG_CUDA(c, cudaMalloc(&st.z, sizeof(float) * cap * c->dims.noise_dim));
  PBG_TRY(make_tmap(c, &st.tm_xg0, st.xg0, cap, c->kg0p, kBlockM));
  PBG_TRY(make_tmap(c, &st.tm_xd0, st.xd0, cap, c->kd0p, kBlockM));
  st.cap = cap;
  return PBG_OK;
}

int ensure_latents(pbg_ctx* c, long long rows, cudaStream_t stream) {
  if (c->lat_cap >= rows) return PBG_OK;
  PBG_TRY(begin_growth(c, stream, "the latent workspace"));
  const long long cap = pow2_cap(rows);
  c->lat_cap = 0;
  PBG_TRY(realloc_dev(c, c->lat_z, sizeof(float) * cap * c->dims.noise_dim));
  c->lat_cap = cap;
  return PBG_OK;
}

int check_draw_size(pbg_ctx* c, long long total_rows) {
  if (total_rows < 1) return fail(c, PBG_ERR_INVALID, "latent draw: total_rows must be positive");
  if (total_rows > 0x7fffffffll / c->dims.noise_dim)
    return fail(c, PBG_ERR_UNSUPPORTED, "latent draw: %lld x %d elements is above the 2^31 - 1 of one torch launch",
                total_rows, c->dims.noise_dim);
  return PBG_OK;
}

int launch_draw(pbg_ctx* c, unsigned long long seed, unsigned long long offset, LatentStream* st, bool advance,
                long long total_rows, long long row_begin, long long rows, float* out, cudaStream_t s) {
  if (rows <= 0) return PBG_OK;
  const long long Z = c->dims.noise_dim;
  const LatentGeometry g = latent_geometry(total_rows * Z, c->num_sms, c->max_threads_sm);
  LatentParams p{};
  p.seed = seed; p.offset = offset; p.st = st; p.advance = advance ? 1 : 0; p.inc = g.inc; p.T = g.T;
  p.e_begin = row_begin * Z; p.e_end = (row_begin + rows) * Z; p.out = out;
  const long long r_lo = p.e_begin / (4 * g.T), r_hi = (p.e_end - 1) / (4 * g.T);
  p.slot_begin = r_lo * g.T;
  const long long blocks = (r_hi - r_lo + 1) * g.T / kLatentThreads;
  { LaunchScope ls(c, PBG_K_OTHER, s);
    latent_draw_kernel<<<static_cast<unsigned>(blocks), kLatentThreads, 0, s>>>(p); }
  PBG_CUDA(c, cudaGetLastError());
  return PBG_OK;
}

int draw_stream(pbg_ctx* c, long long B, float* out, cudaStream_t s) {
  PBG_TRY(check_draw_size(c, B));
  return launch_draw(c, c->lat_seed, 0, c->lat_st, true, B, 0, B, out, s);
}

template <int ACT>
int launch_f32(pbg_ctx* c, int kind, const Linear& l, const float* A, long long lda, float* out, long long ldo, long long M,
               cudaStream_t s) {
  F32GemmParams p{A, lda, l.w_f32, l.k, l.b_f32, out, ldo, (int)M, l.n, l.k, c->dims.leaky_slope};
  dim3 grid((l.n + 63) / 64, (unsigned)((M + 63) / 64));
  { LaunchScope ls(c, kind, s);
    gemm_f32_kernel<ACT><<<grid, 256, 0, s>>>(p); }
  PBG_CUDA(c, cudaGetLastError());
  return PBG_OK;
}


int pass_grid(const pbg_ctx* c) {
  static const int env = [] { const char* e = getenv("PBG_GRID"); return e ? atoi(e) : 0; }();
  const int want = c->launch_ctas > 0 ? c->launch_ctas : env;
  return (want > 0 && want < c->num_sms) ? std::max(2, want) : c->num_sms;
}

struct Pass;
int launch_pass2(pbg_ctx* c, Workspace& w, const Pass& a, const GatherParams& gp, long long off, long long rows,
                 void* gen_out, float* scores, bool external_gather, const StageSlot* slot = nullptr, bool gather_ahead = false);

struct Pass {
  const float* node_emb = nullptr; long long N = 0;
  const float* rel_emb = nullptr;  long long R = 0;
  const long long *heads = nullptr, *rels = nullptr, *tails = nullptr;
  long long hs = 1, rs = 1, ts = 1;
  const float *h = nullptr, *r = nullptr, *t = nullptr, *z = nullptr;
  bool draw_z = false;
  void* gen_out = nullptr; int out_dtype = PBG_DT_F32;
  float *gen_scores = nullptr, *logits = nullptr, *probs = nullptr;
  bool run_g = false, run_d = false;
  long long B = 0; int prec = PBG_PREC_BF16; cudaStream_t stream = nullptr;
};

int run_chunk(pbg_ctx* c, const Pass& a, long long off, long long rows) {
  const int E = c->dims.embed_dim, Z = c->dims.noise_dim;
  const bool bf = a.prec == PBG_PREC_BF16;
  Workspace& w = bf ? c->ws_bf16 : c->ws_f32;
  cudaStream_t s = a.stream;

  GatherParams gp{};
  gp.node_emb = a.node_emb; gp.rel_emb = a.rel_emb; gp.N = a.N; gp.R = a.R; gp.E = E; gp.Z = Z;
  gp.heads = a.heads ? a.heads + off * a.hs : nullptr; gp.head_stride = a.hs;
  gp.rels = a.rels ? a.rels + off * a.rs : nullptr;    gp.rel_stride = a.rs;
  gp.tails = a.tails ? a.tails + off * a.ts : nullptr; gp.tail_stride = a.ts;
  gp.h = a.h ? a.h + off * E : nullptr; gp.r = a.r ? a.r + off * E : nullptr; gp.t = a.t ? a.t + off * E : nullptr;
  gp.z = a.z ? a.z + off * Z : nullptr;
  if (a.draw_z) {
    PBG_TRY(launch_draw(c, c->lat_seed, 0, c->lat_st, off + rows == a.B, a.B, off, rows, c->lat_z, s));
    gp.z = c->lat_z;
  }
  gp.xg = a.run_g ? w.xg0 : nullptr; gp.ldg = bf ? c->kg0p : c->kg0;
  gp.xd = a.run_d ? w.xd0 : nullptr; gp.ldd = bf ? c->kd0p : c->kd0;
  gp.B = rows; gp.err_flag = c->err_flag;
  const int gather_blocks = (int)std::min<long long>((rows + 7) / 8, (long long)c->num_sms * 8);
  if (!bf && (c->n_mirror > 0 || c->mc_gen || c->mc_cos || c->mc_logits || c->mc_probs))
    return fail(c, PBG_ERR_UNSUPPORTED, "result mirrors / multicast are a bf16-mode feature");
  static const bool split_env = [] { const char* e = getenv("PBG_SPLIT_GATHER"); return e && atoi(e) != 0; }();
  const bool split = bf && split_env && rows > 0;
  if (!bf) {
    LaunchScope ls(c, PBG_K_GATHER, s);
    gather_concat_kernel<float><<<gather_blocks, 256, 0, s>>>(gp);
  } else if (split) {
    LaunchScope ls(c, PBG_K_GATHER, s);
    gather_concat_kernel<__nv_bfloat16><<<gather_blocks, 256, 0, s>>>(gp);
  }
  PBG_CUDA(c, cudaGetLastError());

  const size_t out_es = a.out_dtype == PBG_DT_BF16 ? 2 : 4;
  void* gen_out = a.gen_out ? static_cast<char*>(a.gen_out) + (size_t)off * E * out_es : nullptr;
  float* scores = a.gen_scores ? a.gen_scores + off : nullptr;

  if (bf) {
    return launch_pass2(c, w, a, gp, off, rows, gen_out, scores, split);
  } else {
    float *xg0 = (float*)w.xg0, *xd0 = (float*)w.xd0, *bufA = (float*)w.bufA, *bufB = (float*)w.bufB;
    const int row_blocks = (int)std::min<long long>((rows + 7) / 8, (long long)c->num_sms * 8);
    if (a.run_g) {
      const int H = c->dims.g_hidden;
      PBG_TRY(launch_f32<ACT_LEAKY>(c, PBG_K_G_L0, c->g[0], xg0, c->kg0, bufA, H, rows, s));
      PBG_TRY(launch_f32<ACT_LEAKY>(c, PBG_K_G_L1, c->g[1], bufA, H, bufB, H, rows, s));
      float* pred = gen_out ? (float*)gen_out : bufA;
      PBG_TRY(launch_f32<ACT_TANH>(c, PBG_K_G_L2, c->g[2], bufB, H, pred, E, rows, s));
      if (scores) {
        { LaunchScope ls(c, PBG_K_OTHER, s);
          cosine_f32_kernel<<<row_blocks, 256, 0, s>>>(pred, E, a.node_emb, a.N, a.tails + off * a.ts, a.ts, E, rows,
                                                       scores); }
        PBG_CUDA(c, cudaGetLastError());
      }
    }
    if (a.run_d) {
      const int H = c->dims.d_hidden, H2 = c->hd2;
      PBG_TRY(launch_f32<ACT_LEAKY>(c, PBG_K_D_L0, c->d[0], xd0, c->kd0, bufA, H, rows, s));
      PBG_TRY(launch_f32<ACT_LEAKY>(c, PBG_K_D_L1, c->d[1], bufA, H, bufB, H2, rows, s));
      { LaunchScope ls(c, PBG_K_OTHER, s);
        rowdot_f32_kernel<<<row_blocks, 256, 0, s>>>(bufB, H2, c->d_w3, c->d_b3, H2, rows, a.logits + off,
                                                     a.probs ? a.probs + off : nullptr); }
      PBG_CUDA(c, cudaGetLastError());
    }
  }
  return PBG_OK;
}


template <class... KArgs, class... Args>
cudaError_t launch_pdl(bool pdl, void (*kern)(KArgs...), unsigned grid, unsigned block, size_t smem, cudaStream_t s, Args&&... args) {
  cudaLaunchConfig_t cfg = {};
  cfg.gridDim = dim3(grid); cfg.blockDim = dim3(block); cfg.dynamicSmemBytes = smem; cfg.stream = s;
  cudaLaunchAttribute at[1];
  at[0].id = cudaLaunchAttributeProgrammaticStreamSerialization;
  at[0].val.programmaticStreamSerializationAllowed = 1;
  cfg.attrs = at; cfg.numAttrs = pdl ? 1 : 0;
  return cudaLaunchKernelEx(&cfg, kern, static_cast<KArgs>(args)...);
}

using Pass2Kernel = void (*)(Pass2Params);
const Pass2Kernel kPass2[8] = {
    pbg_pass2_kernel<false, false, false>, pbg_pass2_kernel<false, false, true>, pbg_pass2_kernel<false, true, false>,
    pbg_pass2_kernel<false, true, true>,   pbg_pass2_kernel<true, false, false>, pbg_pass2_kernel<true, false, true>,
    pbg_pass2_kernel<true, true, false>,   pbg_pass2_kernel<true, true, true>};

const int kEpiOf[5] = {PEPI_STORE, PEPI_STORE, PEPI_STORE, PEPI_ROWDOT, PEPI_TANH};
const int kPredOf[5] = {DEP_X, DEP_X, DEP_G0, DEP_D0, DEP_G1};
const int kOutOf[5] = {DEP_G0, DEP_D0, DEP_G1, -1, -1};

void set_layer(Pass2Params& p, int k, const Linear& l, const CUtensorMap& amap, const CUtensorMap* omap,
               __nv_bfloat16* out, int ldo) {
  const int bn = (l.np % 256 == 0) ? 256 : 128;
  p.tm_a[k] = amap;
  p.tm_w[k] = bn == 256 ? l.tmap_w128 : l.tmap_w64;
  if (omap) p.tm_o[k] = *omap;
  p.layer[k] = P2Layer{l.kp / kBlockK, bn, l.np / bn, kEpiOf[k], kPredOf[k], kOutOf[k], ldo, -1, l.b_pad, out};
  p.layer_mask |= 1u << k;
}

int launch_pass2(pbg_ctx* c, Workspace& w, const Pass& a, const GatherParams& gp, long long off, long long rows,
                 void* gen_out, float* scores, bool external_gather, const StageSlot* slot, bool gather_ahead) {
  const int grid = pass_grid(c) & ~1;
  Pass2Params p;
  memset(&p, 0, sizeof p);
  const Linear* lin[5] = {&c->g[0], &c->d[0], &c->g[1], &c->d[1], &c->g[2]};
  const CUtensorMap* amap[5] = {slot ? &slot->tm_xg0 : &w.tm_xg0, slot ? &slot->tm_xd0 : &w.tm_xd0, &w.tm_bufA_g, &w.tm_bufD_d,
                                &w.tm_bufB_g};
  const CUtensorMap* omap[5] = {&w.tmo_bufA, &w.tmo_bufD, &w.tmo_bufB, nullptr, nullptr};
  const bool on[5] = {a.run_g, a.run_d, a.run_g, a.run_d, a.run_g};
  const int nrb = static_cast<int>((rows + kP2Rows - 1) / kP2Rows);
  __nv_bfloat16* outs[5] = {(__nv_bfloat16*)w.bufA, (__nv_bfloat16*)w.bufD, (__nv_bfloat16*)w.bufB, nullptr, nullptr};
  const int ldos[5] = {c->hgp, c->hdp, c->hgp, 0, 0};
  long long total = 0;
  for (int k = 0; k < 5; ++k) {
    if (!on[k]) continue;
    set_layer(p, k, *lin[k], *amap[k], omap[k], outs[k], ldos[k]);
    if (p.layer[k].n_tiles > 255) return fail(c, PBG_ERR_UNSUPPORTED, "layer too wide for the tile index");
    total += static_cast<long long>(nrb) * p.layer[k].n_tiles;
  }
  bool biass = false;
  {
    int off = 0;
    for (int k = 0; k < 5; ++k) if (on[k]) { p.layer[k].bias_off = off; off += lin[k]->np; }
    p.w3_off = off;
    if (on[IT_D_L1]) off += lin[IT_D_L1]->np;
    biass = off <= P2Smem::kBiasFloats;
  }
  if (on[IT_D_L1] && lin[IT_D_L1]->np / 64 > kPartSlotsD) return fail(c, PBG_ERR_UNSUPPORTED, "d_hidden too wide for the partial buffer");
  if (on[IT_G_L2] && lin[IT_G_L2]->np / 64 > kPartSlotsG / 2) return fail(c, PBG_ERR_UNSUPPORTED, "embed_dim too wide for the partial buffer");
  p.phase0_groups = external_gather ? 0 : nrb * kP2GroupsPerBlock;
  p.gather_external = external_gather ? 1 : 0;
  if (gather_ahead) {
    p.phase0_groups = static_cast<int>((gp.B + 3) / 4);
    p.gather_ahead = 1;
  }
  {
    static const int waves_env = [] { const char* e = getenv("PBG_WAVES"); return e ? atoi(e) : 1; }();
    const int waves = std::max(1, std::min(waves_env, std::min(nrb, 3)));
    static const int mix_env = [] { const char* e = getenv("PBG_MIX"); return e ? atoi(e) : 0; }();
    const bool mix = on[IT_D_L1] && on[IT_G_L2] && mix_env != 0;
    int start = 0;
    auto add_seg = [&](int k, int rb_lo, int rb_hi, int k2 = -1) {
      if (k < 0 || !on[k] || rb_hi == rb_lo) return;
      const int nt2 = (k2 >= 0 && on[k2]) ? p.layer[k2].n_tiles : 0;
      p.seg[p.n_seg++] = P2Segment{k, p.layer[k].n_tiles, start, rb_lo, nt2 ? k2 : k, nt2};
      start += (rb_hi - rb_lo) * (p.layer[k].n_tiles + nt2);
    };
    for (int wv = 0; wv < waves; ++wv) {
      const int rb_lo = static_cast<int>(static_cast<long long>(nrb) * wv / waves);
      const int rb_hi = static_cast<int>(static_cast<long long>(nrb) * (wv + 1) / waves);
      add_seg(IT_G_L0, rb_lo, rb_hi);
      add_seg(IT_D_L0, rb_lo, rb_hi);
    }
    add_seg(IT_G_L1, 0, nrb);
    if (mix) {
      add_seg(IT_D_L1, 0, nrb, IT_G_L2);
    } else {
      add_seg(IT_D_L1, 0, nrb);
      add_seg(IT_G_L2, 0, nrb);
    }
    if (start != total) return fail(c, PBG_ERR_INVALID, "internal: static item list does not cover the pass");
    p.n_total = start;
  }
  p.gather = gp;
  static const int poll_env = [] { const char* e = getenv("PBG_POLL_NS"); return e ? atoi(e) : 40; }();
  p.poll_ns = poll_env;
  static const int defer_env = [] { const char* e = getenv("PBG_GATHER_DEFER"); return e ? atoi(e) : 1; }();
  p.gather_defer = defer_env;
  p.discard = c->discard;
  if (!external_gather) {
    p.dead_xg = gp.xg; p.dead_xd = gp.xd;
  } else if (gather_ahead && slot) {
    p.dead_xg = a.run_g ? slot->xg0 : nullptr; p.dead_xd = a.run_d ? slot->xd0 : nullptr;
  }
  p.dead_ldg = c->kg0p; p.dead_ldd = c->kd0p;
  p.nrb = nrb; p.rb_cap = w.mb_cap; p.M = static_cast<int>(rows); p.slope = c->dims.leaky_slope;
  p.sched = w.sched; p.ready = w.ready; p.fin = w.fin;
  p.gen_out = gen_out; p.out_f32 = a.out_dtype == PBG_DT_F32; p.n_valid = c->dims.embed_dim; p.ld_gen = c->dims.embed_dim;
  if (scores && slot && slot->has_xt) {
    p.cosine = scores; p.tail_tab = slot->xt; p.n_ent = slot->cap; p.tail_idx = nullptr; p.tail_stride = 0;
  } else if (scores && slot) {
    p.cosine = scores; p.tail_tab = slot->node_emb; p.n_ent = slot->N; p.tail_idx = slot->tails; p.tail_stride = 3;
  } else if (scores) {
    p.cosine = scores; p.tail_tab = a.node_emb; p.n_ent = a.N;
    p.tail_idx = a.tails + off * a.ts; p.tail_stride = a.ts;
  }
  p.part_g = w.part_g; p.slots_g = on[IT_G_L2] ? (c->dims.embed_dim + 63) / 64 : 0;
  p.w3 = c->d_w3_pad; p.b3 = c->d_b3;
  p.logits = a.logits ? a.logits + off : nullptr;
  p.probs = a.probs ? a.probs + off : nullptr;
  p.part_d = w.part_d; p.slots_d = on[IT_D_L1] ? lin[IT_D_L1]->np / 64 : 0;
  p.trace = c->trace;
  p.n_mirror = c->n_mirror;
  for (int i = 0; i < c->n_mirror; ++i) {
    if (gen_out && !c->mir_gen[i]) return fail(c, PBG_ERR_INVALID, "result mirror %d has no gen_out buffer", i);
    if (scores && !c->mir_cos[i]) return fail(c, PBG_ERR_INVALID, "result mirror %d has no gen_scores buffer", i);
    if (a.logits && !c->mir_logits[i]) return fail(c, PBG_ERR_INVALID, "result mirror %d has no logits buffer", i);
    const size_t es = a.out_dtype == PBG_DT_BF16 ? 2 : 4;
    p.mir_gen[i] = c->mir_gen[i] ? static_cast<char*>(c->mir_gen[i]) + static_cast<size_t>(off) * c->dims.embed_dim * es : nullptr;
    p.mir_cos[i] = c->mir_cos[i] ? c->mir_cos[i] + off : nullptr;
    p.mir_logits[i] = c->mir_logits[i] ? c->mir_logits[i] + off : nullptr;
    p.mir_probs[i] = (c->mir_probs[i] && a.probs) ? c->mir_probs[i] + off : nullptr;
  }
  {
    const size_t es = a.out_dtype == PBG_DT_BF16 ? 2 : 4;
    p.mc_gen = (c->mc_gen && gen_out) ? static_cast<char*>(c->mc_gen) + static_cast<size_t>(off) * c->dims.embed_dim * es : nullptr;
    p.mc_cos = (c->mc_cos && scores) ? c->mc_cos + off : nullptr;
    p.mc_logits = (c->mc_logits && a.logits) ? c->mc_logits + off : nullptr;
    p.mc_probs = (c->mc_probs && a.probs) ? c->mc_probs + off : nullptr;
  }
  static const bool pdl = [] { const char* e = getenv("PBG_PDL"); return !e || atoi(e) != 0; }();
  const bool fastg = c->dims.embed_dim == 128 && c->dims.noise_dim % 4 == 0 && c->dims.noise_dim <= 128 &&
                     c->kg0p == c->kg0 && c->kd0p == c->kd0;
  const Pass2Kernel kern = kPass2[(p.trace ? 4 : 0) | (fastg ? 2 : 0) | (biass ? 1 : 0)];
  cudaError_t le;
  { LaunchScope ls(c, PBG_K_PASS, a.stream);
    le = launch_pdl(pdl, kern, grid, kP2Threads, P2Smem::kTotal, a.stream, p); }
  if (le == cudaSuccess) le = cudaGetLastError();
  if (le != cudaSuccess) {
    cudaFuncAttributes fa{};
    cudaFuncGetAttributes(&fa, kern);
    return fail(c, PBG_ERR_CUDA, "pass kernel launch failed: %s (grid %d x %d threads, %d regs/thread, %zu B static + %d B dynamic smem, "
                "max threads/block %d, max dynamic smem %d)", cudaGetErrorString(le), grid, kP2Threads, fa.numRegs,
                fa.sharedSizeBytes, P2Smem::kTotal, fa.maxThreadsPerBlock, fa.maxDynamicSharedSizeBytes);
  }
  return PBG_OK;
}

int run_pass(pbg_ctx* c, Pass a) {
  if (!c) return PBG_ERR_INVALID;
  if (a.B < 0) return fail(c, PBG_ERR_INVALID, "negative batch");
  if (a.prec != PBG_PREC_F32 && a.prec != PBG_PREC_BF16) return fail(c, PBG_ERR_INVALID, "unknown precision %d", a.prec);
  if (a.run_g && !c->g_loaded) return fail(c, PBG_ERR_NOT_LOADED, "generator weights not loaded");
  if (a.run_d && !c->d_loaded) return fail(c, PBG_ERR_NOT_LOADED, "discriminator weights not loaded");
  if (a.run_g && a.z == nullptr && !c->lat_on) return fail(c, PBG_ERR_INVALID, "generator needs latents z");
  a.draw_z = a.run_g && a.z == nullptr && a.B > 0;
  if (a.draw_z) PBG_TRY(check_draw_size(c, a.B));
  if (a.run_g && a.gen_out && a.prec == PBG_PREC_F32 && a.out_dtype != PBG_DT_F32)
    return fail(c, PBG_ERR_INVALID, "fp32 mode writes fp32 output");
  if (a.gen_scores && a.tails == nullptr) return fail(c, PBG_ERR_INVALID, "gen_scores needs tail ids");
  if (a.B == 0 || (!a.run_g && !a.run_d)) return PBG_OK;
  PBG_CUDA(c, cudaSetDevice(c->dims.device));
  const long long chunk = std::min(a.B, kMaxChunk);
  PBG_TRY(ensure_ws(c, a.prec, chunk, a.stream));
  if (a.draw_z) PBG_TRY(ensure_latents(c, chunk, a.stream));
  for (long long off = 0; off < a.B; off += chunk) PBG_TRY(run_chunk(c, a, off, std::min(chunk, a.B - off)));
  return PBG_OK;
}

}

extern "C" {

int pbg_abi_version(void) { return PBG_ABI_VERSION; }

const char* pbg_last_error(const pbg_ctx* ctx) { return ctx ? ctx->err.c_str() : g_create_error.c_str(); }

int64_t pbg_launch_count(const pbg_ctx* ctx) { return ctx ? ctx->launches : 0; }

int64_t pbg_format_f32_json(const float* v, size_t rows, int cols, int indent, int depth, char* out, size_t cap) {
  if ((!v && rows) || cols < 0 || depth < 0) return -(int64_t)fail(nullptr, PBG_ERR_INVALID, "format_f32_json: bad arguments");
  return (int64_t)pbg_host::format_rows<float>(v, rows, cols, indent, depth, out, cap, pbg_host::put_py_float);
}

int64_t pbg_format_i64_json(const int64_t* v, size_t rows, int cols, int indent, int depth, char* out, size_t cap) {
  if ((!v && rows) || cols < 0 || depth < 0) return -(int64_t)fail(nullptr, PBG_ERR_INVALID, "format_i64_json: bad arguments");
  return (int64_t)pbg_host::format_rows<int64_t>(v, rows, cols, indent, depth, out, cap, pbg_host::put_i64);
}

int64_t pbg_parse_index_rows(const char* text, size_t len, int cols, int64_t* out, size_t cap_rows) {
  if (!text || cols < 1 || cols > 8) return -(int64_t)fail(nullptr, PBG_ERR_INVALID, "parse_index_rows: null text or cols outside 1..8");
  const char* msg = nullptr;
  size_t off = 0;
  const long long rows = pbg_host::parse_index_rows(text, len, cols, out, cap_rows, &msg, &off);
  if (rows < 0) return -(int64_t)fail(nullptr, PBG_ERR_INVALID, "parse_index_rows: %s at byte %zu", msg, off);
  return rows;
}

int pbg_topk_prepare(pbg_ctx* c, const float* table, int64_t N, void* stream) {
  if (!c) return PBG_ERR_INVALID;
  if (!table || N <= 0) return fail(c, PBG_ERR_INVALID, "topk: null or empty table");
  const int E = c->dims.embed_dim;
  if (E % 4) return fail(c, PBG_ERR_UNSUPPORTED, "topk: embed_dim must be a multiple of 4");
  PBG_CUDA(c, cudaSetDevice(c->dims.device));
  cudaStream_t s = (cudaStream_t)stream;
  TopkState& t = c->tk;
  const long long n_pad = (N + 255) / 256 * 256;
  if (n_pad != t.n_pad) {
    PBG_TRY(begin_growth(c, s, "the top-k table"));
    t.n_pad = 0;
    PBG_TRY(realloc_dev(c, t.tn, sizeof(__nv_bfloat16) * n_pad * E));
    PBG_TRY(realloc_dev(c, t.inv_t, sizeof(float) * n_pad));
    t.n_pad = n_pad;
    if (E == 128) PBG_TRY(make_tmap(c, &t.tm_t, t.tn, n_pad, E, 128));
  }
  t.table = table; t.N = N;
  { LaunchScope ls(c, PBG_K_OTHER, s);
    if (E <= 128) topk_prepare_kernel<8, 1><<<c->num_sms * 8, 256, 0, s>>>(table, N, n_pad, E, t.tn, t.inv_t);
    else topk_prepare_kernel<2, 4><<<c->num_sms * 8, 256, 0, s>>>(table, N, n_pad, E, t.tn, t.inv_t); }
  PBG_CUDA(c, cudaGetLastError());
  return PBG_OK;
}

constexpr int kTkGeneralMaxK = 512;

namespace {
int topk_general(pbg_ctx* c, TopkState& t, const float* q, long long rows, int k, long long* oi, float* os, cudaStream_t s) {
  const int E = c->dims.embed_dim;
  const long long chunk = std::max<long long>(64, std::min<long long>(rows, (512ll << 20) / (4 * t.N)));
  const size_t need = static_cast<size_t>(chunk) * t.N;
  if (t.score_cap < need) {
    PBG_TRY(begin_growth(c, s, "the top-k score buffer"));
    t.score_cap = 0;
    PBG_TRY(realloc_dev(c, t.score_buf, sizeof(float) * need));
    t.score_cap = need;
  }
  const int threads = std::max(32, std::min(256, (200 * 1024 / (k * 8)) / 32 * 32));
  const size_t smem = static_cast<size_t>(E) * 4 + static_cast<size_t>(threads) * k * 8;
  for (long long off = 0; off < rows; off += chunk) {
    const long long r = std::min(chunk, rows - off);
    F32GemmParams gp{q + off * E, E, t.table, E, nullptr, t.score_buf, t.N, (int)r, (int)t.N, E, 0.f};
    dim3 grid((unsigned)((t.N + 63) / 64), (unsigned)((r + 63) / 64));
    { LaunchScope ls(c, PBG_K_OTHER, s);
      gemm_f32_kernel<ACT_NONE><<<grid, 256, 0, s>>>(gp); }
    PBG_CUDA(c, cudaGetLastError());
    { LaunchScope ls(c, PBG_K_OTHER, s);
      topk_select_kernel<<<static_cast<unsigned>(std::min<long long>(r, 6ll * c->num_sms)), kSelThreads, 0, s>>>(
          t.score_buf, t.inv_q + off, t.inv_t, t.N, k, r, oi + off * k, os + off * k, t.flag + off); }
    PBG_CUDA(c, cudaGetLastError());
    { LaunchScope ls(c, PBG_K_OTHER, s);
      topk_exact_kernel<<<static_cast<unsigned>(std::min<long long>(r, 2ll * c->num_sms)), threads, smem, s>>>(
          q + off * E, t.inv_q + off, t.table, t.inv_t, t.N, E, k, t.flag + off, 0, t.score_buf, oi + off * k, os + off * k, r); }
    PBG_CUDA(c, cudaGetLastError());
  }
  return PBG_OK;
}
}

int pbg_topk(pbg_ctx* c, const float* queries, int64_t B, int k, int64_t* out_idx, float* out_scores, void* stream) {
  if (!c) return PBG_ERR_INVALID;
  TopkState& t = c->tk;
  if (B < 0) return fail(c, PBG_ERR_INVALID, "negative batch");
  if (B == 0) return PBG_OK;
  if (!t.table) return fail(c, PBG_ERR_NOT_LOADED, "topk: no table prepared (pbg_topk_prepare)");
  if (!queries || !out_idx || !out_scores) return fail(c, PBG_ERR_INVALID, "null tensor");
  if (k < 1) return fail(c, PBG_ERR_INVALID, "topk: k must be positive");
  if (k > t.N) return fail(c, PBG_ERR_INVALID, "topk: k = %d exceeds the %lld rows of the table", k, t.N);
  if (k > kTkGeneralMaxK) return fail(c, PBG_ERR_UNSUPPORTED, "topk: k = %d is above the %d this library selects on the device", k, kTkGeneralMaxK);
  PBG_CUDA(c, cudaSetDevice(c->dims.device));
  cudaStream_t s = (cudaStream_t)stream;
  const int E = c->dims.embed_dim;
  const long long kChunk = k > 16 ? 4096 : 16384;
  const int stride = tk_sample_stride(k);
  const bool filter = E == 128 && k <= kTkMaxK && t.N >= std::max<long long>(16 * 256, 64ll * stride * k);
  for (long long off = 0; off < B; off += kChunk) {
    const long long rows = std::min(kChunk, B - off);
    const long long rows_pad = (rows + 255) / 256 * 256;
    const float* q = queries + off * E;
    if (t.q_cap < rows_pad) {
      PBG_TRY(begin_growth(c, s, "the top-k query buffers"));
      t.q_cap = 0;
      PBG_TRY(realloc_dev(c, t.qn, sizeof(__nv_bfloat16) * rows_pad * E));
      PBG_TRY(realloc_dev(c, t.inv_q, sizeof(float) * rows_pad));
      PBG_TRY(realloc_dev(c, t.flag, sizeof(int) * rows_pad));
      PBG_TRY(realloc_dev(c, t.tau, sizeof(float) * rows_pad));
      t.q_cap = rows_pad;
      if (E == 128) PBG_TRY(make_tmap(c, &t.tm_q, t.qn, rows_pad, E, 128));
    }
    { LaunchScope ls(c, PBG_K_OTHER, s);
      const unsigned pg = static_cast<unsigned>(std::min<long long>(c->num_sms * 8, (rows_pad + 7) / 8));
      if (E <= 128) topk_prepare_kernel<8, 1><<<pg, 256, 0, s>>>(q, rows, rows_pad, E, t.qn, t.inv_q);
      else topk_prepare_kernel<2, 4><<<pg, 256, 0, s>>>(q, rows, rows_pad, E, t.qn, t.inv_q); }
    PBG_CUDA(c, cudaGetLastError());
    long long* oi = reinterpret_cast<long long*>(out_idx) + off * k;
    float* os = out_scores + off * k;
    t.last_rows = rows; t.last_filtered = filter;
    if (!filter) {
      PBG_TRY(topk_general(c, t, q, rows, k, oi, os, s));
      continue;
    }
    const int grid = pass_grid(c) & ~1;
    const int npairs = grid / 2;
    const int n_rb = static_cast<int>(rows_pad / 256);
    const int n_tiles = static_cast<int>(t.n_pad / 256);
    auto split = [&](int tiles, TopkParams& p, bool align) {
      p.n_rb = n_rb;
      p.n_tiles = tiles;
      p.total = n_rb * tiles;
      p.span = std::max({1, (p.total + npairs - 1) / npairs, (tiles + kTkMaxRanges - 2) / (kTkMaxRanges - 1)});
      if (align && p.span < tiles) { const int pieces = std::max(1, tiles / p.span); p.span = (tiles + pieces - 1) / pieces; }
      p.n_ranges = 1;
      for (int rb = 0; rb < n_rb; ++rb)
        p.n_ranges = std::max(p.n_ranges, ((rb + 1) * tiles - 1) / p.span - (rb * tiles) / p.span + 1);
    };
    TopkParams ps, pm;
    memset(&ps, 0, sizeof ps); memset(&pm, 0, sizeof pm);
    ps.tm_q = pm.tm_q = t.tm_q; ps.tm_t = pm.tm_t = t.tm_t; ps.N = pm.N = t.N;
    ps.tile_stride = stride; pm.tile_stride = 1;
    split((n_tiles + stride - 1) / stride, ps, true);
    split(n_tiles, pm, false);
    const int n_slists = ps.n_ranges * 2, n_lists = pm.n_ranges * 2;
    const size_t need = static_cast<size_t>(rows_pad) * n_lists * kTkCand;
    const size_t sneed = static_cast<size_t>(rows_pad) * n_slists * kTkKeys;
    if (t.cand_cap < need || t.samp_cap < sneed) {
      PBG_TRY(begin_growth(c, s, "the top-k candidate buffers"));
      t.cand_cap = t.samp_cap = 0;
      PBG_TRY(realloc_dev(c, t.cand_grp, sizeof(unsigned) * need));
      PBG_TRY(realloc_dev(c, t.cand_mask, sizeof(unsigned) * need));
      PBG_TRY(realloc_dev(c, t.cand_cnt, sizeof(int) * need / kTkCand));
      PBG_TRY(realloc_dev(c, t.samp_keys, sizeof(int) * sneed));
      t.cand_cap = need; t.samp_cap = sneed;
    }
    ps.samp_keys = t.samp_keys;
    pm.tau = t.tau; pm.cand_grp = t.cand_grp; pm.cand_mask = t.cand_mask; pm.cand_cnt = t.cand_cnt;
    { LaunchScope ls(c, PBG_K_TOPK, s);
      PBG_CUDA(c, launch_pdl(true, pbg_topk_scan_kernel<TK_SAMPLE>, std::min(grid, 2 * ((ps.total + ps.span - 1) / ps.span)), kPassThreads, TkSmem::kTotal, s, ps)); }
    { LaunchScope ls(c, PBG_K_OTHER, s);
      PBG_CUDA(c, launch_pdl(false, topk_tau_kernel, static_cast<unsigned>((rows_pad + 7) / 8), 256, 0, s, t.samp_keys, n_slists, rows, rows_pad, k, t.tau)); }
    { LaunchScope ls(c, PBG_K_TOPK, s);
      PBG_CUDA(c, launch_pdl(true, pbg_topk_scan_kernel<TK_SCAN>, std::min(grid, 2 * ((pm.total + pm.span - 1) / pm.span)), kPassThreads, TkSmem::kTotal, s, pm)); }
    { LaunchScope ls(c, PBG_K_OTHER, s);
      PBG_CUDA(c, launch_pdl(false, topk_rescore_kernel, static_cast<unsigned>((rows + kTkRescoreWarps - 1) / kTkRescoreWarps), 32 * kTkRescoreWarps, 0, s,
                             q, t.inv_q, t.table, t.inv_t, t.cand_grp, t.cand_mask, t.cand_cnt, t.tau, n_lists, rows, t.N, k, oi, os, t.flag)); }
    {
      LaunchScope ls(c, PBG_K_OTHER, s);
      PBG_CUDA(c, launch_pdl(true, topk_exact_kernel, static_cast<unsigned>(std::min<long long>(rows, 2ll * c->num_sms)), 256,
                             static_cast<size_t>(E * 4 + 256 * k * 8), s, q, t.inv_q, t.table, t.inv_t, t.N, E, k, t.flag, 0, nullptr, oi, os, rows)); }
  }
  return PBG_OK;
}

int64_t pbg_topk_last_flagged(pbg_ctx* c, void* stream) {
  if (!c) return -1;
  TopkState& t = c->tk;
  if (!t.last_filtered || t.last_rows <= 0) return 0;
  if (cudaSetDevice(c->dims.device) != cudaSuccess) return -1;
  std::vector<int> h(static_cast<size_t>(t.last_rows));
  if (cudaMemcpyAsync(h.data(), t.flag, sizeof(int) * h.size(), cudaMemcpyDeviceToHost, (cudaStream_t)stream) != cudaSuccess) return -1;
  if (cudaStreamSynchronize((cudaStream_t)stream) != cudaSuccess) return -1;
  int64_t n = 0, why[5] = {0, 0, 0, 0, 0};
  for (int v : h) { n += v != 0; why[(v >= 0 && v <= 4) ? v : 0] += 1; }
  char buf[160];
  snprintf(buf, sizeof buf, "topk: %lld of %lld rows to the exact scan (list overflow %lld, too many candidates %lld, too few %lld, proof failed %lld)",
           (long long)n, t.last_rows, (long long)why[1], (long long)why[2], (long long)why[3], (long long)why[4]);
  c->err = buf;
  return n;
}

int pbg_set_result_mirrors(pbg_ctx* c, int n, void* const* gen_out, float* const* gen_scores, float* const* logits,
                           float* const* probs) {
  if (!c) return PBG_ERR_INVALID;
  if (n < 0 || n > kMaxMirrors) return fail(c, PBG_ERR_INVALID, "at most %d result mirrors", kMaxMirrors);
  c->n_mirror = n;
  for (int i = 0; i < kMaxMirrors; ++i) {
    c->mir_gen[i] = (i < n && gen_out) ? gen_out[i] : nullptr;
    c->mir_cos[i] = (i < n && gen_scores) ? gen_scores[i] : nullptr;
    c->mir_logits[i] = (i < n && logits) ? logits[i] : nullptr;
    c->mir_probs[i] = (i < n && probs) ? probs[i] : nullptr;
  }
  return PBG_OK;
}

int pbg_set_result_multicast(pbg_ctx* c, void* gen_out_mc, float* gen_scores_mc, float* logits_mc, float* probs_mc) {
  if (!c) return PBG_ERR_INVALID;
  c->mc_gen = gen_out_mc; c->mc_cos = gen_scores_mc; c->mc_logits = logits_mc; c->mc_probs = probs_mc;
  return PBG_OK;
}

int pbg_set_launch_width(pbg_ctx* c, int n_ctas) {
  if (!c) return PBG_ERR_INVALID;
  if (n_ctas < 0) return fail(c, PBG_ERR_INVALID, "launch width must be >= 0");
  c->launch_ctas = n_ctas;
  return PBG_OK;
}

int pbg_last_pass_sm_clock(pbg_ctx* c, void* stream, double* mhz_out) {
  if (!c || !mhz_out) return PBG_ERR_INVALID;
  *mhz_out = 0.0;
  Workspace& w = c->ws_bf16;
  if (!w.sched) return fail(c, PBG_ERR_INVALID, "no bf16-mode pass has run on this ctx");
  PBG_CUDA(c, cudaSetDevice(c->dims.device));
  cudaStream_t s = (cudaStream_t)stream;
  PassSched h;
  PBG_CUDA(c, cudaMemcpyAsync(&h, w.sched, sizeof h, cudaMemcpyDeviceToHost, s));
  PBG_CUDA(c, cudaStreamSynchronize(s));
  if (h.clk_ns > 0) *mhz_out = static_cast<double>(h.clk_ticks) / static_cast<double>(h.clk_ns) * 1e3;
  return PBG_OK;
}

int pbg_set_workspace_discard(pbg_ctx* c, int on) {
  if (!c) return PBG_ERR_INVALID;
  c->discard = on ? 1 : 0;
  return PBG_OK;
}

int pbg_create(pbg_ctx** out, const pbg_dims* dims) {
  if (!out || !dims) return fail(nullptr, PBG_ERR_INVALID, "null argument");
  *out = nullptr;
  const int E = dims->embed_dim, Z = dims->noise_dim, HG = dims->g_hidden, HD = dims->d_hidden;
  if (E <= 0 || Z <= 0 || HG <= 0 || HD <= 0) return fail(nullptr, PBG_ERR_INVALID, "dims must be positive");
  if (!(dims->leaky_slope >= 0.f && dims->leaky_slope <= 1.f))
    return fail(nullptr, PBG_ERR_UNSUPPORTED, "leaky_slope must be in [0, 1]");
  if (E % 8 || Z % 8 || HG % 8 || HD % 16)
    return fail(nullptr, PBG_ERR_UNSUPPORTED, "embed_dim, noise_dim, g_hidden must be multiples of 8 and d_hidden of 16");
  int ndev = 0;
  cudaError_t e = cudaGetDeviceCount(&ndev);
  if (e != cudaSuccess || ndev == 0)
    return fail(nullptr, PBG_ERR_UNSUPPORTED, "no CUDA device (%s); this library has no CPU fallback",
                e == cudaSuccess ? "device count 0" : cudaGetErrorString(e));
  if (dims->device < 0 || dims->device >= ndev) return fail(nullptr, PBG_ERR_INVALID, "device %d out of range", dims->device);
  cudaDeviceProp prop;
  if ((e = cudaGetDeviceProperties(&prop, dims->device)) != cudaSuccess)
    return fail(nullptr, PBG_ERR_CUDA, "cudaGetDeviceProperties: %s", cudaGetErrorString(e));
  if (prop.major != 10)
    return fail(nullptr, PBG_ERR_UNSUPPORTED, "device %d is sm_%d%d; the kernels are sm_100a only (no fallback)",
                dims->device, prop.major, prop.minor);
  pbg_ctx* c = new (std::nothrow) pbg_ctx();
  if (!c) return fail(nullptr, PBG_ERR_NOMEM, "out of host memory");
  c->dims = *dims;
  c->num_sms = prop.multiProcessorCount;
  c->max_threads_sm = prop.maxThreadsPerMultiProcessor;
  if (const char* e = getenv("PBG_DISCARD")) c->discard = atoi(e) != 0;
  if (const char* e = getenv("PBG_HOST_SYNC")) c->host_block = strcmp(e, "block") == 0;
  c->kg0 = 2 * E + Z; c->kg0p = round_up(c->kg0, kBlockK);
  c->kd0 = 3 * E;     c->kd0p = round_up(c->kd0, kBlockK);
  c->hgp = round_up(HG, 128); c->hdp = round_up(HD, 128);
  c->hd2 = HD / 2;
  c->hmax = std::max(c->hgp, c->hdp);
  auto bail = [&](int code) { g_create_error = c->err; pbg_destroy(c); return code; };
  if (cudaSetDevice(dims->device) != cudaSuccess) { c->err = "cudaSetDevice failed"; return bail(PBG_ERR_CUDA); }
  e = cudaSuccess;
  for (Pass2Kernel k : kPass2)
    if (e == cudaSuccess) e = cudaFuncSetAttribute(k, cudaFuncAttributeMaxDynamicSharedMemorySize, P2Smem::kTotal);
  if (e == cudaSuccess) e = cudaFuncSetAttribute(pbg_topk_scan_kernel<TK_SAMPLE>, cudaFuncAttributeMaxDynamicSharedMemorySize, TkSmem::kTotal);
  if (e == cudaSuccess) e = cudaFuncSetAttribute(pbg_topk_scan_kernel<TK_SCAN>, cudaFuncAttributeMaxDynamicSharedMemorySize, TkSmem::kTotal);
  if (e == cudaSuccess) e = cudaFuncSetAttribute(topk_exact_kernel, cudaFuncAttributeMaxDynamicSharedMemorySize, 220 * 1024);
  if (e != cudaSuccess) { c->err = std::string("cudaFuncSetAttribute failed: ") + cudaGetErrorString(e); return bail(PBG_ERR_CUDA); }
  void* fn = nullptr;
  cudaDriverEntryPointQueryResult qres;
  if (cudaGetDriverEntryPoint("cuTensorMapEncodeTiled", &fn, cudaEnableDefault, &qres) != cudaSuccess || !fn) {
    c->err = "cuTensorMapEncodeTiled not available from the driver";
    return bail(PBG_ERR_CUDA);
  }
  c->encode = reinterpret_cast<EncodeTiledFn>(fn);
  if (cudaStreamCreateWithFlags(&c->own_stream, cudaStreamNonBlocking) != cudaSuccess ||
      cudaMalloc(&c->err_flag, sizeof(int)) != cudaSuccess ||
      cudaMemset(c->err_flag, 0, sizeof(int)) != cudaSuccess ||
      cudaMallocHost(&c->err_flag_host, sizeof(int)) != cudaSuccess ||
      cudaMalloc(&c->lat_st, sizeof(LatentStream)) != cudaSuccess ||
      cudaMemset(c->lat_st, 0, sizeof(LatentStream)) != cudaSuccess) {
    c->err = std::string("ctx allocation failed: ") + cudaGetErrorString(cudaGetLastError());
    return bail(PBG_ERR_CUDA);
  }
  *c->err_flag_host = 0;
  *out = c;
  return PBG_OK;
}

void pbg_destroy(pbg_ctx* c) {
  if (!c) return;
  cudaSetDevice(c->dims.device);
  cudaDeviceSynchronize();
  for (auto& l : c->g) free_linear(l);
  for (auto& l : c->d) free_linear(l);
  cudaFree(c->d_w3); cudaFree(c->d_w3_pad);
  free_ws(c->ws_bf16); free_ws(c->ws_f32);
  free_stage(c->stage[0]); free_stage(c->stage[1]);
  cudaFree(c->err_flag); cudaFree(c->trace);
  cudaFree(c->lat_st); cudaFree(c->lat_z);
  cudaFree(c->tk.tn); cudaFree(c->tk.inv_t); cudaFree(c->tk.qn); cudaFree(c->tk.inv_q);
  cudaFree(c->tk.cand_grp); cudaFree(c->tk.cand_mask); cudaFree(c->tk.cand_cnt); cudaFree(c->tk.flag);
  cudaFree(c->tk.samp_keys); cudaFree(c->tk.tau); cudaFree(c->tk.score_buf);

  if (c->err_flag_host) cudaFreeHost(c->err_flag_host);
  if (c->host_evt) cudaEventDestroy(c->host_evt);
  cudaFree(c->st_block);
  if (c->own_stream) cudaStreamDestroy(c->own_stream);
  delete c;
}

int pbg_load_generator(pbg_ctx* c, const float* p, size_t n_floats) {
  if (!c || !p) return PBG_ERR_INVALID;
  const size_t E = c->dims.embed_dim, H = c->dims.g_hidden, K0 = c->kg0;
  const size_t want = H * K0 + H + H * H + H + E * H + E;
  if (n_floats != want) return fail(c, PBG_ERR_INVALID, "generator blob has %zu floats, expected %zu", n_floats, want);
  PBG_CUDA(c, cudaSetDevice(c->dims.device));
  c->g_loaded = false;
  const float* w1 = p;            const float* b1 = w1 + H * K0;
  const float* w2 = b1 + H;       const float* b2 = w2 + H * H;
  const float* w3 = b2 + H;       const float* b3 = w3 + E * H;
  PBG_TRY(upload_linear(c, c->g[0], (int)H, (int)K0, c->kg0p, w1, b1));
  PBG_TRY(upload_linear(c, c->g[1], (int)H, (int)H, c->hgp, w2, b2));
  PBG_TRY(upload_linear(c, c->g[2], (int)E, (int)H, c->hgp, w3, b3));
  c->g_loaded = true;
  return PBG_OK;
}

int pbg_load_discriminator(pbg_ctx* c, const float* p, size_t n_floats) {
  if (!c || !p) return PBG_ERR_INVALID;
  const size_t H = c->dims.d_hidden, H2 = c->hd2, K0 = c->kd0;
  const size_t want = H * K0 + H + H2 * H + H2 + H2 + 1;
  if (n_floats != want) return fail(c, PBG_ERR_INVALID, "discriminator blob has %zu floats, expected %zu", n_floats, want);
  PBG_CUDA(c, cudaSetDevice(c->dims.device));
  c->d_loaded = false;
  const float* w1 = p;            const float* b1 = w1 + H * K0;
  const float* w2 = b1 + H;       const float* b2 = w2 + H2 * H;
  const float* w3 = b2 + H2;      const float* b3 = w3 + H2;
  PBG_TRY(upload_linear(c, c->d[0], (int)H, (int)K0, c->kd0p, w1, b1));
  PBG_TRY(upload_linear(c, c->d[1], (int)H2, (int)H, c->hdp, w2, b2));
  cudaFree(c->d_w3); cudaFree(c->d_w3_pad); c->d_w3 = c->d_w3_pad = nullptr;
  const int np = c->d[1].np;
  PBG_CUDA(c, cudaMalloc(&c->d_w3, sizeof(float) * H2));
  PBG_CUDA(c, cudaMalloc(&c->d_w3_pad, sizeof(float) * np));
  PBG_CUDA(c, cudaMemcpyAsync(c->d_w3, w3, sizeof(float) * H2, cudaMemcpyHostToDevice, c->own_stream));
  { LaunchScope ls(c, PBG_K_OTHER, c->own_stream);
    pad_f32_kernel<<<8, 256, 0, c->own_stream>>>(c->d_w3, c->d_w3_pad, (int)H2, np); }
  PBG_CUDA(c, cudaGetLastError());
  PBG_CUDA(c, cudaStreamSynchronize(c->own_stream));
  c->d_b3 = *b3;
  c->d_loaded = true;
  return PBG_OK;
}

int pbg_generator_forward(pbg_ctx* c, const float* h, const float* r, const float* z, void* out, int64_t B,
                          int precision, int out_dtype, void* stream) {
  if (!c) return PBG_ERR_INVALID;
  if (B > 0 && (!h || !r || !out)) return fail(c, PBG_ERR_INVALID, "null tensor");
  Pass a; a.h = h; a.r = r; a.z = z; a.gen_out = out; a.out_dtype = out_dtype; a.run_g = true;
  a.B = B; a.prec = precision; a.stream = (cudaStream_t)stream;
  return run_pass(c, a);
}

int pbg_generator_forward_gather(pbg_ctx* c, const float* node_emb, int64_t N, const float* rel_emb, int64_t R,
                                 const int64_t* heads, int64_t head_stride, const int64_t* rels, int64_t rel_stride,
                                 const float* z, void* out, int64_t B, int precision, int out_dtype, void* stream) {
  if (!c) return PBG_ERR_INVALID;
  if (B > 0 && (!node_emb || !rel_emb || !heads || !rels || !out)) return fail(c, PBG_ERR_INVALID, "null tensor");
  Pass a; a.node_emb = node_emb; a.N = N; a.rel_emb = rel_emb; a.R = R;
  a.heads = (const long long*)heads; a.hs = head_stride; a.rels = (const long long*)rels; a.rs = rel_stride;
  a.z = z; a.gen_out = out; a.out_dtype = out_dtype; a.run_g = true;
  a.B = B; a.prec = precision; a.stream = (cudaStream_t)stream;
  return run_pass(c, a);
}

int pbg_discriminator_forward(pbg_ctx* c, const float* h, const float* r, const float* t, float* logits, float* probs,
                              int64_t B, int precision, void* stream) {
  if (!c) return PBG_ERR_INVALID;
  if (B > 0 && (!h || !r || !t || !logits)) return fail(c, PBG_ERR_INVALID, "null tensor");
  Pass a; a.h = h; a.r = r; a.t = t; a.logits = logits; a.probs = probs; a.run_d = true;
  a.B = B; a.prec = precision; a.stream = (cudaStream_t)stream;
  return run_pass(c, a);
}

int pbg_discriminator_score_triplets(pbg_ctx* c, const float* node_emb, int64_t N, const float* rel_emb, int64_t R,
                                     const int64_t* triplets, float* logits, float* probs, int64_t B, int precision,
                                     void* stream) {
  return pbg_score_triplets(c, node_emb, N, rel_emb, R, triplets, nullptr, nullptr, PBG_DT_F32, nullptr, logits, probs,
                            B, precision, stream);
}

int pbg_score_triplets(pbg_ctx* c, const float* node_emb, int64_t N, const float* rel_emb, int64_t R,
                       const int64_t* triplets, const float* z, void* gen_out, int out_dtype, float* gen_scores,
                       float* logits, float* probs, int64_t B, int precision, void* stream) {
  if (!c) return PBG_ERR_INVALID;
  if (B > 0 && (!node_emb || !rel_emb || !triplets)) return fail(c, PBG_ERR_INVALID, "null tensor");
  Pass a; a.node_emb = node_emb; a.N = N; a.rel_emb = rel_emb; a.R = R;
  const long long* t = (const long long*)triplets;
  a.heads = t; a.rels = t + 1; a.tails = t + 2; a.hs = a.rs = a.ts = 3;
  a.z = z; a.gen_out = gen_out; a.out_dtype = out_dtype; a.gen_scores = gen_scores;
  a.logits = logits; a.probs = probs;
  a.run_g = (gen_out != nullptr || gen_scores != nullptr); a.run_d = (logits != nullptr);
  a.B = B; a.prec = precision; a.stream = (cudaStream_t)stream;
  return run_pass(c, a);
}

int pbg_reserve(pbg_ctx* c, int64_t rows, int precision, int stage_slots) {
  if (!c) return PBG_ERR_INVALID;
  if (rows <= 0) return fail(c, PBG_ERR_INVALID, "reserve: rows must be positive");
  if (precision != PBG_PREC_F32 && precision != PBG_PREC_BF16) return fail(c, PBG_ERR_INVALID, "unknown precision %d", precision);
  if (stage_slots < 0 || stage_slots > 2) return fail(c, PBG_ERR_INVALID, "reserve: stage_slots must be 0, 1 or 2");
  PBG_CUDA(c, cudaSetDevice(c->dims.device));
  const long long chunk = std::min<long long>(rows, kMaxChunk);
  PBG_TRY(ensure_ws(c, precision, chunk, nullptr));
  PBG_TRY(ensure_latents(c, chunk, nullptr));
  for (int i = 0; i < stage_slots; ++i) PBG_TRY(ensure_stage(c, c->stage[i], chunk, nullptr));
  return PBG_OK;
}

int pbg_draw_latents(pbg_ctx* c, uint64_t seed, uint64_t offset, int64_t total_rows, int64_t row_begin, int64_t rows,
                     float* z_out, uint64_t* offset_after, void* stream) {
  if (!c) return PBG_ERR_INVALID;
  PBG_TRY(check_draw_size(c, total_rows));
  if (row_begin < 0 || rows < 0 || row_begin + rows > total_rows)
    return fail(c, PBG_ERR_INVALID, "latent draw: rows [%lld, %lld) outside the %lld of the draw", (long long)row_begin,
                (long long)(row_begin + rows), (long long)total_rows);
  if (rows > 0 && !z_out) return fail(c, PBG_ERR_INVALID, "null tensor");
  if (offset % 4) return fail(c, PBG_ERR_INVALID, "latent draw: the Philox offset must be a multiple of 4, as torch's");
  PBG_CUDA(c, cudaSetDevice(c->dims.device));
  PBG_TRY(launch_draw(c, seed, offset, nullptr, false, total_rows, row_begin, rows, z_out, (cudaStream_t)stream));
  if (offset_after)
    *offset_after = offset + latent_geometry(total_rows * c->dims.noise_dim, c->num_sms, c->max_threads_sm).inc;
  return PBG_OK;
}

int pbg_set_latent_stream(pbg_ctx* c, int enable, uint64_t seed, uint64_t offset) {
  if (!c) return PBG_ERR_INVALID;
  if (offset % 4) return fail(c, PBG_ERR_INVALID, "latent stream: the Philox offset must be a multiple of 4, as torch's");
  PBG_CUDA(c, cudaSetDevice(c->dims.device));
  PBG_CUDA(c, cudaDeviceSynchronize());
  const LatentStream st{offset, 0u};
  PBG_CUDA(c, cudaMemcpy(c->lat_st, &st, sizeof st, cudaMemcpyHostToDevice));
  c->lat_on = enable != 0;
  c->lat_seed = seed;
  return PBG_OK;
}

int pbg_get_latent_stream(pbg_ctx* c, uint64_t* seed, uint64_t* offset, void* stream) {
  if (!c || !seed || !offset) return PBG_ERR_INVALID;
  PBG_CUDA(c, cudaSetDevice(c->dims.device));
  LatentStream st{};
  PBG_CUDA(c, cudaMemcpyAsync(&st, c->lat_st, sizeof st, cudaMemcpyDeviceToHost, (cudaStream_t)stream));
  PBG_CUDA(c, cudaStreamSynchronize((cudaStream_t)stream));
  *seed = c->lat_seed;
  *offset = st.offset;
  return PBG_OK;
}

namespace {
GatherParams slot_gather(const pbg_ctx* c, const StageSlot& st, const float* node_emb, long long N, const float* rel_emb,
                         long long R, const long long* t, const float* z, long long B, bool gen, bool disc) {
  GatherParams gp{};
  gp.node_emb = node_emb; gp.rel_emb = rel_emb; gp.N = N; gp.R = R; gp.E = c->dims.embed_dim; gp.Z = c->dims.noise_dim;
  gp.heads = t; gp.rels = t + 1; gp.tails = t + 2; gp.head_stride = gp.rel_stride = gp.tail_stride = 3;
  gp.z = z;
  gp.xg = gen ? st.xg0 : nullptr; gp.ldg = c->kg0p;
  gp.xd = disc ? st.xd0 : nullptr; gp.ldd = c->kd0p;
  gp.B = B; gp.err_flag = c->err_flag;
  return gp;
}

int staged_pass(pbg_ctx* c, int slot, void* gen_out, int out_dtype, float* gen_scores, float* logits, float* probs,
                void* stream, Pass& a) {
  if (slot < 0 || slot > 1) return fail(c, PBG_ERR_INVALID, "score_staged: slot must be 0 or 1");
  const StageSlot& st = c->stage[slot];
  if (st.B <= 0) return fail(c, PBG_ERR_INVALID, "score_staged: nothing staged in slot %d", slot);
  a.gen_out = gen_out; a.out_dtype = out_dtype; a.gen_scores = gen_scores; a.logits = logits; a.probs = probs;
  a.run_g = (gen_out != nullptr || gen_scores != nullptr); a.run_d = (logits != nullptr);
  if (a.run_g && !st.has_g) return fail(c, PBG_ERR_INVALID, "score_staged: slot %d holds no generator operands", slot);
  if (a.run_d && !st.has_d) return fail(c, PBG_ERR_INVALID, "score_staged: slot %d holds no discriminator operands", slot);
  a.B = st.B; a.prec = PBG_PREC_BF16; a.stream = (cudaStream_t)stream;
  return PBG_OK;
}
}

int pbg_stage_triplets(pbg_ctx* c, int slot, const float* node_emb, int64_t N, const float* rel_emb, int64_t R,
                       const int64_t* triplets, const float* z, int64_t B, int want_gen, int want_disc, void* stream) {
  if (!c) return PBG_ERR_INVALID;
  if (slot < 0 || slot > 1) return fail(c, PBG_ERR_INVALID, "stage: slot must be 0 or 1");
  if (B <= 0 || B > kMaxChunk) return fail(c, PBG_ERR_INVALID, "stage: B must be in [1, %lld]", kMaxChunk);
  if (!node_emb || !rel_emb || !triplets) return fail(c, PBG_ERR_INVALID, "null tensor");
  if (!want_gen && !want_disc) return fail(c, PBG_ERR_INVALID, "stage: nothing to stage");
  if (want_gen && !c->g_loaded) return fail(c, PBG_ERR_NOT_LOADED, "generator weights not loaded");
  if (want_disc && !c->d_loaded) return fail(c, PBG_ERR_NOT_LOADED, "discriminator weights not loaded");
  if (want_gen && !z && !c->lat_on) return fail(c, PBG_ERR_INVALID, "generator needs latents z");
  PBG_CUDA(c, cudaSetDevice(c->dims.device));
  cudaStream_t s = (cudaStream_t)stream;
  StageSlot& st = c->stage[slot];
  PBG_TRY(ensure_stage(c, st, B, s));
  if (want_gen && !z) {
    PBG_TRY(draw_stream(c, B, st.z, s));
    z = st.z;
  }
  const long long* t = (const long long*)triplets;
  StageParams sp{};
  sp.g = slot_gather(c, st, node_emb, N, rel_emb, R, t, z, B, want_gen != 0, want_disc != 0);
  sp.xt = want_gen ? st.xt : nullptr;
  const int blocks = (int)std::min<long long>((B + 3) / 4, (long long)c->num_sms * 16);
  { LaunchScope ls(c, PBG_K_GATHER, s);
    stage_rows_kernel<<<blocks, 128, 0, s>>>(sp); }
  PBG_CUDA(c, cudaGetLastError());
  st.B = B; st.has_g = want_gen != 0; st.has_d = want_disc != 0; st.has_xt = want_gen != 0;
  st.node_emb = node_emb; st.N = N; st.tails = t + 2;
  return PBG_OK;
}

int pbg_score_staged(pbg_ctx* c, int slot, void* gen_out, int out_dtype, float* gen_scores, float* logits, float* probs,
                     void* stream) {
  if (!c) return PBG_ERR_INVALID;
  Pass a;
  PBG_TRY(staged_pass(c, slot, gen_out, out_dtype, gen_scores, logits, probs, stream, a));
  if (!a.run_g && !a.run_d) return PBG_OK;
  PBG_CUDA(c, cudaSetDevice(c->dims.device));
  PBG_TRY(ensure_ws(c, PBG_PREC_BF16, a.B, a.stream));
  GatherParams gp{};
  return launch_pass2(c, c->ws_bf16, a, gp, 0, a.B, gen_out, gen_scores, true, &c->stage[slot]);
}

int pbg_score_staged_stage_next(pbg_ctx* c, int slot, void* gen_out, int out_dtype, float* gen_scores, float* logits, float* probs,
                                const float* node_emb, int64_t N, const float* rel_emb, int64_t R, const int64_t* next_triplets,
                                const float* next_z, int64_t next_B, void* stream) {
  if (!c) return PBG_ERR_INVALID;
  Pass a;
  PBG_TRY(staged_pass(c, slot, gen_out, out_dtype, gen_scores, logits, probs, stream, a));
  StageSlot& st = c->stage[slot];
  StageSlot& nx = c->stage[1 - slot];
  if (next_B <= 0 || next_B > kMaxChunk) return fail(c, PBG_ERR_INVALID, "stage next: B must be in [1, %lld]", kMaxChunk);
  if (!node_emb || !rel_emb || !next_triplets) return fail(c, PBG_ERR_INVALID, "null tensor");
  if (!a.run_g && !a.run_d) return fail(c, PBG_ERR_INVALID, "score_staged_stage_next: no result requested");
  if (a.run_g && !next_z && !c->lat_on) return fail(c, PBG_ERR_INVALID, "generator needs latents z");
  PBG_CUDA(c, cudaSetDevice(c->dims.device));
  PBG_TRY(ensure_ws(c, PBG_PREC_BF16, a.B, a.stream));
  PBG_TRY(ensure_stage(c, nx, next_B, a.stream));
  if (a.run_g && !next_z) {
    PBG_TRY(draw_stream(c, next_B, nx.z, a.stream));
    next_z = nx.z;
  }
  const long long* t = reinterpret_cast<const long long*>(next_triplets);
  const GatherParams gp = slot_gather(c, nx, node_emb, N, rel_emb, R, t, next_z, next_B, a.run_g, a.run_d);
  PBG_TRY(launch_pass2(c, c->ws_bf16, a, gp, 0, a.B, gen_out, gen_scores, true, &st, true));
  st.B = -1;
  nx.B = next_B; nx.has_g = a.run_g; nx.has_d = a.run_d; nx.has_xt = false;
  nx.node_emb = node_emb; nx.N = N; nx.tails = t + 2;
  return PBG_OK;
}

int pbg_linear_bf16(pbg_ctx* c, int model, int layer, const void* a, void* out, int64_t M, void* stream) {
  if (!c || !a || !out || M <= 0) return c ? fail(c, PBG_ERR_INVALID, "bad argument") : PBG_ERR_INVALID;
  if (model == 0 && !c->g_loaded) return fail(c, PBG_ERR_NOT_LOADED, "generator weights not loaded");
  if (model == 1 && !c->d_loaded) return fail(c, PBG_ERR_NOT_LOADED, "discriminator weights not loaded");
  if (model < 0 || model > 1 || layer < 0 || layer > (model == 0 ? 2 : 1)) return fail(c, PBG_ERR_INVALID, "no such layer");
  if (M > kMaxChunk) return fail(c, PBG_ERR_INVALID, "linear_bf16: at most %lld rows", kMaxChunk);
  PBG_CUDA(c, cudaSetDevice(c->dims.device));
  cudaStream_t s = (cudaStream_t)stream;
  PBG_TRY(ensure_ws(c, PBG_PREC_BF16, M, s));
  Workspace& w = c->ws_bf16;
  static const int kind_of[2][3] = {{IT_G_L0, IT_G_L1, IT_G_L2}, {IT_D_L0, IT_D_L1, -1}};
  const int k = kind_of[model][layer];
  const Linear& l = model == 0 ? c->g[layer] : c->d[layer];
  const bool store = kEpiOf[k] == PEPI_STORE;
  CUtensorMap amap, omap;
  PBG_TRY(make_tmap(c, &amap, a, M, l.kp, kBlockM));
  if (store) PBG_TRY(make_tmap(c, &omap, out, M, l.np, 32));
  Pass2Params p;
  memset(&p, 0, sizeof p);
  set_layer(p, k, l, amap, store ? &omap : nullptr, store ? static_cast<__nv_bfloat16*>(out) : nullptr, l.np);
  const int nrb = static_cast<int>((M + kP2Rows - 1) / kP2Rows);
  p.seg[0] = P2Segment{k, p.layer[k].n_tiles, 0, 0, k, 0};
  p.n_seg = 1; p.n_total = nrb * p.layer[k].n_tiles;
  p.no_deps = 1; p.gather_external = 1; p.phase0_groups = 0;
  p.poll_ns = 40; p.gather_defer = 1;
  p.nrb = nrb; p.rb_cap = w.mb_cap; p.M = static_cast<int>(M); p.slope = c->dims.leaky_slope;
  p.sched = w.sched; p.ready = w.ready; p.fin = w.fin;
  p.part_g = w.part_g; p.part_d = w.part_d;
  if (k == IT_G_L2) {
    p.gen_out = out; p.out_f32 = 1; p.n_valid = c->dims.embed_dim; p.ld_gen = c->dims.embed_dim;
    p.slots_g = (c->dims.embed_dim + 63) / 64;
  }
  if (k == IT_D_L1) {
    if (l.np / 64 > kPartSlotsD) return fail(c, PBG_ERR_UNSUPPORTED, "d_hidden too wide for the partial buffer");
    p.w3 = c->d_w3_pad; p.b3 = c->d_b3; p.logits = static_cast<float*>(out); p.slots_d = l.np / 64;
  }
  p.w3_off = -1;
  const int grid = pass_grid(c) & ~1;
  cudaError_t le;
  { LaunchScope ls(c, model == 0 ? PBG_K_G_L0 + layer : PBG_K_D_L0 + layer, s);
    le = launch_pdl(false, kPass2[0], grid, kP2Threads, P2Smem::kTotal, s, p); }
  if (le == cudaSuccess) le = cudaGetLastError();
  if (le != cudaSuccess) return fail(c, PBG_ERR_CUDA, "single-layer pass launch failed: %s", cudaGetErrorString(le));
  return PBG_OK;
}

int pbg_profile_enable(pbg_ctx* c, int enable) {
  if (!c) return PBG_ERR_INVALID;
  c->profiling = enable != 0;
  return PBG_OK;
}

int pbg_profile_read(pbg_ctx* c, double* ms, int64_t* count) {
  if (!c || !ms || !count) return PBG_ERR_INVALID;
  PBG_CUDA(c, cudaSetDevice(c->dims.device));
  PBG_CUDA(c, cudaDeviceSynchronize());
  for (auto& r : c->prof) {
    float t = 0.f;
    if (cudaEventElapsedTime(&t, r.a, r.b) == cudaSuccess && r.kind >= 0 && r.kind < PBG_NUM_KERNEL_KINDS) {
      ms[r.kind] += t; count[r.kind] += 1;
    }
    cudaEventDestroy(r.a); cudaEventDestroy(r.b);
  }
  c->prof.clear();
  return PBG_OK;
}

int pbg_debug_trace(pbg_ctx* c, int enable, int64_t* host_out, int64_t n_slots) {
  if (!c) return PBG_ERR_INVALID;
  PBG_CUDA(c, cudaSetDevice(c->dims.device));
  PBG_CUDA(c, cudaDeviceSynchronize());
  const size_t n = static_cast<size_t>(c->num_sms) * kTraceSlots;
  if (host_out && c->trace) {
    std::vector<long long> tmp(n);
    PBG_CUDA(c, cudaMemcpy(tmp.data(), c->trace, n * sizeof(long long), cudaMemcpyDeviceToHost));
    for (size_t i = 0; i < n && i < static_cast<size_t>(n_slots); ++i) host_out[i] = tmp[i];
  }
  if (enable && !c->trace) {
    PBG_CUDA(c, cudaMalloc(&c->trace, n * sizeof(long long)));
  } else if (!enable && c->trace) {
    cudaFree(c->trace); c->trace = nullptr;
  }
  if (c->trace) PBG_CUDA(c, cudaMemset(c->trace, 0, n * sizeof(long long)));
  return PBG_OK;
}

int pbg_check_indices(pbg_ctx* c, void* stream) {
  if (!c) return PBG_ERR_INVALID;
  cudaStream_t s = (cudaStream_t)stream;
  PBG_CUDA(c, cudaSetDevice(c->dims.device));
  PBG_CUDA(c, cudaMemcpyAsync(c->err_flag_host, c->err_flag, sizeof(int), cudaMemcpyDeviceToHost, s));
  if (c->host_block) {
    if (!c->host_evt) PBG_CUDA(c, cudaEventCreateWithFlags(&c->host_evt, cudaEventBlockingSync | cudaEventDisableTiming));
    PBG_CUDA(c, cudaEventRecord(c->host_evt, s));
    PBG_CUDA(c, cudaEventSynchronize(c->host_evt));
  } else {
    PBG_CUDA(c, cudaStreamSynchronize(s));
  }
  if (*c->err_flag_host != 0) {
    PBG_CUDA(c, cudaMemsetAsync(c->err_flag, 0, sizeof(int), s));
    PBG_CUDA(c, cudaStreamSynchronize(s));
    return fail(c, PBG_ERR_INDEX, "index out of range in embedding gather");
  }
  return PBG_OK;
}

namespace {
int score_host(pbg_ctx* c, const float* node_emb, int64_t N, const float* rel_emb, int64_t R, const int64_t* triplets_host,
               const float* z_host, float* gen_out_host, float* gen_scores_host, float* logits_host, float* probs_host,
               int64_t B, int precision, bool packed) {
  if (!c) return PBG_ERR_INVALID;
  if (B < 0) return fail(c, PBG_ERR_INVALID, "negative batch");
  if (B == 0) return PBG_OK;
  if (!triplets_host) return fail(c, PBG_ERR_INVALID, "null triplets");
  const bool run_g = gen_out_host || gen_scores_host;
  if (run_g && !z_host && !c->lat_on) return fail(c, PBG_ERR_INVALID, "generator needs latents z");
  PBG_CUDA(c, cudaSetDevice(c->dims.device));
  const int E = c->dims.embed_dim, Z = c->dims.noise_dim;
  cudaStream_t s = c->own_stream;
  if (c->host_cap < B) {
    PBG_TRY(begin_growth(c, s, "the host staging block"));
    c->host_cap = 0;
    const size_t per_row = sizeof(long long) * 3 + sizeof(float) * (Z + 3 + E);
    PBG_TRY(realloc_dev(c, c->st_block, per_row * B + 64));
    c->host_cap = B;
  }
  auto up16 = [](size_t v) { return (v + 15) & ~static_cast<size_t>(15); };
  char* b0 = c->st_block;
  size_t off = 0;
  long long* trip = reinterpret_cast<long long*>(b0 + off);  off = up16(off + sizeof(long long) * 3 * B);
  float* z = reinterpret_cast<float*>(b0 + off);             off += sizeof(float) * Z * B;
  float* scores = reinterpret_cast<float*>(b0 + off);        off += sizeof(float) * B;
  float* logits = reinterpret_cast<float*>(b0 + off);        off += sizeof(float) * B;
  float* probs = reinterpret_cast<float*>(b0 + off);         off = up16(off + sizeof(float) * B);
  float* gen = reinterpret_cast<float*>(b0 + off);
  const bool one_h2d = packed && z_host && reinterpret_cast<char*>(z) == reinterpret_cast<char*>(trip) + sizeof(long long) * 3 * B;
  if (one_h2d) {
    PBG_CUDA(c, cudaMemcpyAsync(trip, triplets_host, sizeof(long long) * 3 * B + sizeof(float) * Z * B, cudaMemcpyHostToDevice, s));
  } else {
    PBG_CUDA(c, cudaMemcpyAsync(trip, triplets_host, sizeof(long long) * 3 * B, cudaMemcpyHostToDevice, s));
    if (run_g && z_host) PBG_CUDA(c, cudaMemcpyAsync(z, z_host, sizeof(float) * Z * B, cudaMemcpyHostToDevice, s));
  }
  PBG_TRY(pbg_score_triplets(c, node_emb, N, rel_emb, R, (const int64_t*)trip, run_g && z_host ? z : nullptr,
                             gen_out_host ? gen : nullptr, PBG_DT_F32, gen_scores_host ? scores : nullptr,
                             logits_host ? logits : nullptr, probs_host ? probs : nullptr, B, precision, s));
  if (packed) {
    PBG_CUDA(c, cudaMemcpyAsync(gen_scores_host, scores, sizeof(float) * 3 * B, cudaMemcpyDeviceToHost, s));
  } else {
    if (gen_scores_host) PBG_CUDA(c, cudaMemcpyAsync(gen_scores_host, scores, sizeof(float) * B, cudaMemcpyDeviceToHost, s));
    if (logits_host) PBG_CUDA(c, cudaMemcpyAsync(logits_host, logits, sizeof(float) * B, cudaMemcpyDeviceToHost, s));
    if (probs_host) PBG_CUDA(c, cudaMemcpyAsync(probs_host, probs, sizeof(float) * B, cudaMemcpyDeviceToHost, s));
  }
  if (gen_out_host) PBG_CUDA(c, cudaMemcpyAsync(gen_out_host, gen, sizeof(float) * E * B, cudaMemcpyDeviceToHost, s));
  return pbg_check_indices(c, s);
}
}

int pbg_score_triplets_host(pbg_ctx* c, const float* node_emb, int64_t N, const float* rel_emb, int64_t R,
                            const int64_t* triplets_host, const float* z_host, float* gen_out_host,
                            float* gen_scores_host, float* logits_host, float* probs_host, int64_t B, int precision) {
  return score_host(c, node_emb, N, rel_emb, R, triplets_host, z_host, gen_out_host, gen_scores_host, logits_host, probs_host, B,
                    precision, false);
}

int pbg_score_triplets_host_packed(pbg_ctx* c, const float* node_emb, int64_t N, const float* rel_emb, int64_t R,
                                   const void* in_block_host, float* out_block_host, int64_t B, int precision) {
  if (!c) return PBG_ERR_INVALID;
  if (B > 0 && (!in_block_host || !out_block_host)) return fail(c, PBG_ERR_INVALID, "null block");
  const int64_t* trip = static_cast<const int64_t*>(in_block_host);
  const float* z = reinterpret_cast<const float*>(static_cast<const char*>(in_block_host) + sizeof(long long) * 3 * B);
  return score_host(c, node_emb, N, rel_emb, R, trip, z, nullptr, out_block_host, out_block_host + B, out_block_host + 2 * B, B,
                    precision, true);
}

int pbg_score_triplets_host_ids(pbg_ctx* c, const float* node_emb, int64_t N, const float* rel_emb, int64_t R,
                                const int64_t* triplets_host, float* out_block_host, int64_t B, int precision) {
  if (!c) return PBG_ERR_INVALID;
  if (!c->lat_on) return fail(c, PBG_ERR_INVALID, "score_triplets_host_ids draws the latents: enable the latent stream first");
  if (B > 0 && (!triplets_host || !out_block_host)) return fail(c, PBG_ERR_INVALID, "null block");
  return score_host(c, node_emb, N, rel_emb, R, triplets_host, nullptr, nullptr, out_block_host, out_block_host + B,
                    out_block_host + 2 * B, B, precision, true);
}

}
```

Baseline: 178.5 million.

## Fold relation-embedding slice of first layers into a per-relation partial table

Splits the first generator and discriminator layers so the relation-embedding K-slice is computed once per distinct relation (a small bf16 table of relation rows) into an fp32 partial-product buffer. The main layer GEMM then skips those K blocks, and the epilogue adds the partial product back into TMEM, selected by each row's relation id. This removes the redundant relation columns from the per-sample matmul. In exchange it adds new item kinds, dependency counters with acquire loads, extra fp32 loads and TMEM read-modify-writes in the epilogue, and relation-table copy work in the gather phase.

```diff
diff --git a/pro-b-gan_b200/csrc/gather.cuh b/pro-b-gan_b200/csrc/gather.cuh
--- a/pro-b-gan_b200/csrc/gather.cuh
+++ b/pro-b-gan_b200/csrc/gather.cuh
@@ -18,6 +18,8 @@
   void* xd; int ldd;
   long long B;
   int* err_flag;
+  int* rid;
+  __nv_bfloat16* relc; int rel_rows;
 };
 
 template <typename T>
@@ -40,6 +42,16 @@
   asm volatile("ld.global.nc.L1::no_allocate.v4.f32 {%0, %1, %2, %3}, [%4];"
                : "=f"(v.x), "=f"(v.y), "=f"(v.z), "=f"(v.w) : "l"(p));
   return v;
+}
+
+__device__ __forceinline__ void rel_copy_group(const GatherParams& g, long long group, int lane) {
+  for (int j = 0; j < 4; ++j) {
+    const long long row = group * 4 + j;
+    for (int v = lane; v < g.E / 4; v += 32) {
+      const float4 x = row < g.R ? ld_stream4(g.rel_emb + row * g.E + 4 * v) : make_float4(0.f, 0.f, 0.f, 0.f);
+      store4<__nv_bfloat16>(g.relc + row * g.E + 4 * v, x);
+    }
+  }
 }
 
 template <typename T>
@@ -116,7 +128,9 @@
   const long long N = sp.g.N;
   __nv_bfloat16* const xg = static_cast<__nv_bfloat16*>(sp.g.xg);
   __nv_bfloat16* const xd = static_cast<__nv_bfloat16*>(sp.g.xd);
-  for (long long b = warp_global; b < sp.g.B; b += num_warps) {
+  const long long n_rel = sp.g.relc ? sp.g.rel_rows / 4 : 0;
+  for (long long b = warp_global; b < sp.g.B + n_rel; b += num_warps) {
+    if (b >= sp.g.B) { rel_copy_group(sp.g, b - sp.g.B, lane); continue; }
     bool bad = false;
     long long hi = sp.g.heads[b * 3], ri = sp.g.rels[b * 3], ti = sp.g.tails[b * 3];
     if (hi < 0) hi += N;
@@ -125,6 +139,7 @@
     if (ri < 0 || ri >= sp.g.R) { bad = true; ri = 0; }
     if (ti < 0 || ti >= N) { bad = true; ti = 0; }
     if (bad && lane == 0) atomicOr(sp.g.err_flag, 1);
+    if (sp.g.rid && lane == 0) sp.g.rid[b] = static_cast<int>(ri);
     const float* hrow = sp.g.node_emb + hi * E;
     const float* rrow = sp.g.rel_emb + ri * E;
     const float* trow = sp.g.node_emb + ti * E;
diff --git a/pro-b-gan_b200/csrc/pass2_kernel.cuh b/pro-b-gan_b200/csrc/pass2_kernel.cuh
--- a/pro-b-gan_b200/csrc/pass2_kernel.cuh
+++ b/pro-b-gan_b200/csrc/pass2_kernel.cuh
@@ -53,15 +53,21 @@
   int bias_off;
   const float* bias;
   __nv_bfloat16* out;
+  int a_k0, w_k0;
+  int skip0, nskip;
+  int dep2;
+  float* prel;
+  int ldp;
+  int p_rows;
 };
 
 struct P2Segment { int kind, n_tiles, start, rb0, kind2, n_tiles2; };
 
 struct alignas(64) Pass2Params {
-  CUtensorMap tm_a[5];
+  CUtensorMap tm_a[IT_KINDS];
   CUtensorMap tm_w[5];
   CUtensorMap tm_o[5];
-  P2Layer layer[5];
+  P2Layer layer[IT_KINDS];
   GatherParams gather;
   unsigned layer_mask;
   int gather_defer;
@@ -74,6 +80,10 @@
   int dead_ldg, dead_ldd;
   int poll_ns;
   int phase0_groups;
+  int rel_groups;
+  int rel_table, rel_nrb;
+  const int* rid;
+  const long long* rel_idx; long long rel_stride; long long n_rel;
   int n_total;
   int n_seg;
   P2Segment seg[16];
@@ -144,11 +154,19 @@
   return pack_bf16x2(fmaxf(y.x, s.x), fmaxf(y.y, s.y));
 }
 
+__device__ __forceinline__ int w_layer(int kind) { return kind == IT_G_R ? IT_G_L0 : kind == IT_D_R ? IT_D_L0 : kind; }
+
 __device__ __forceinline__ int p2_dep_target(const Pass2Params& p, int dep_kind) {
   if (p.no_deps) return 0;
   if (dep_kind == DEP_X) return p.gather_external ? 0 : kP2GroupsPerBlock;
+  if (dep_kind == DEP_REL) return p.gather_external ? 0 : p.rel_groups;
+  if (dep_kind == DEP_PG || dep_kind == DEP_PD)
+    return p.layer[dep_kind == DEP_PG ? IT_G_R : IT_D_R].n_tiles * kP2WarpsPerPair * (p.rel_table ? p.rel_nrb : 1);
   const int producer = dep_kind == DEP_G0 ? IT_G_L0 : (dep_kind == DEP_D0 ? IT_D_L0 : IT_G_L1);
   return p.layer[producer].n_tiles * kP2WarpsPerPair;
+}
+__device__ __forceinline__ int p2_dep_index(const Pass2Params& p, int dep_kind, int rb) {
+  return (p.rel_table && dep_kind >= DEP_REL) ? 0 : rb;
 }
 __device__ __forceinline__ void p2_arrive(const Pass2Params& p, int dep_kind, int rb, int lane, bool async_stores,
                                           long long* t_wait = nullptr) {
@@ -168,11 +186,11 @@
 __device__ __forceinline__ void p2_arrive_done(const Pass2Params& p, int dep_kind, int rb, int lane) {
   if (lane == 0) red_relaxed_gpu_add(p.ready + dep_kind * p.rb_cap + rb, 1);
 }
-__device__ __forceinline__ void p2_poll_dep(const Pass2Params& p, int dep_kind, int rb) {
+__device__ __forceinline__ void p2_poll_dep(const Pass2Params& p, int dep_kind, int rb, bool acquire = false) {
   const int target = p2_dep_target(p, dep_kind);
-  const int* ctr = p.ready + dep_kind * p.rb_cap + rb;
+  const int* ctr = p.ready + dep_kind * p.rb_cap + p2_dep_index(p, dep_kind, rb);
   uint32_t spins = 0;
-  while (ld_relaxed_gpu(ctr) < target) {
+  while ((acquire ? ld_acquire_gpu(ctr) : ld_relaxed_gpu(ctr)) < target) {
     __nanosleep(p.poll_ns);
 #if PBG_HANG_GUARD
     if (++spins > 4000000u) pbg_wait_timed_out("dependency (kind, row block)", dep_kind, rb);
@@ -234,7 +252,10 @@
         if (g.heads) { long long i = g.heads[row * g.head_stride]; if (i < 0) i += g.N; if (i < 0 || i >= g.N) { bad = true; i = 0; } src = g.node_emb + i * g.E; }
         else src = g.h + row * g.E;
       } else if (which == 1) {
-        if (g.rels) { long long i = g.rels[row * g.rel_stride]; if (i < 0 || i >= g.R) { bad = true; i = 0; } src = g.rel_emb + i * g.E; }
+        if (g.rels) {
+          long long i = g.rels[row * g.rel_stride]; if (i < 0 || i >= g.R) { bad = true; i = 0; } src = g.rel_emb + i * g.E;
+          if (g.rid) g.rid[row] = static_cast<int>(i);
+        }
         else src = g.r + row * g.E;
       } else if (g.tails) {
         long long i = g.tails[row * g.tail_stride]; if (i < 0) i += g.N; if (i < 0 || i >= g.N) { bad = true; i = 0; } src = g.node_emb + i * g.E;
@@ -299,6 +320,19 @@
     }
   }
 }
+
+__device__ __forceinline__ void tmem_st_32x32_ptr(uint32_t taddr, const uint32_t* v) {
+  asm volatile(
+      "tcgen05.st.sync.aligned.32x32b.x32.b32 [%0], "
+      "{%1, %2, %3, %4, %5, %6, %7, %8, %9, %10, %11, %12, %13, %14, %15, %16, "
+      "%17, %18, %19, %20, %21, %22, %23, %24, %25, %26, %27, %28, %29, %30, %31, %32};"
+      ::"r"(taddr), "r"(v[0]), "r"(v[1]), "r"(v[2]), "r"(v[3]), "r"(v[4]), "r"(v[5]), "r"(v[6]), "r"(v[7]),
+        "r"(v[8]), "r"(v[9]), "r"(v[10]), "r"(v[11]), "r"(v[12]), "r"(v[13]), "r"(v[14]), "r"(v[15]),
+        "r"(v[16]), "r"(v[17]), "r"(v[18]), "r"(v[19]), "r"(v[20]), "r"(v[21]), "r"(v[22]), "r"(v[23]),
+        "r"(v[24]), "r"(v[25]), "r"(v[26]), "r"(v[27]), "r"(v[28]), "r"(v[29]), "r"(v[30]), "r"(v[31])
+      : "memory");
+}
+__device__ __forceinline__ void tmem_st_wait() { asm volatile("tcgen05.wait::st.sync.aligned;" ::: "memory"); }
 
 __device__ __forceinline__ uint32_t ring_dep(uint2 it) { return (it.x >> 24) << 3; }
 
@@ -331,10 +365,10 @@
   constexpr int kRingConsumers = 2 * (1 + kP2Epi) + 1;
 
   if (threadIdx.x == 0) {
-    for (int i = 0; i < 5; ++i) {
+    for (int i = 0; i < IT_KINDS; ++i) {
       if (p.layer_mask & (1u << i)) {
         prefetch_tmap(&p.tm_a[i]);
-        prefetch_tmap(&p.tm_w[i]);
+        if (i < 5) prefetch_tmap(&p.tm_w[i]);
         if (p.layer[i].epi == PEPI_STORE) prefetch_tmap(&p.tm_o[i]);
       }
     }
@@ -396,7 +430,11 @@
           it = make_uint2(static_cast<uint32_t>(j < nt1 ? p.seg[sg].kind : p.seg[sg].kind2) | (static_cast<uint32_t>(j < nt1 ? j : j - nt1) << 8),
                           static_cast<uint32_t>(p.seg[sg].rb0 + i / nt));
         }
-        if ((it.x & 0xff) != IT_END) p2_poll_dep(p, p.layer[it.x & 0xff].dep_kind, static_cast<int>(it.y));
+        if ((it.x & 0xff) != IT_END) {
+          const P2Layer& ly = p.layer[it.x & 0xff];
+          p2_poll_dep(p, ly.dep_kind, static_cast<int>(it.y));
+          if (ly.dep2 >= 0) p2_poll_dep(p, ly.dep2, static_cast<int>(it.y), true);
+        }
         mbar_wait_role(&sched_empty[slot], sphase ^ 1);
         ring[slot] = it;
         mbar_arrive(&sched_full[slot]);
@@ -429,13 +467,14 @@
         const int a_row = rb * kP2Rows + static_cast<int>(rank) * 128;
         const int w_row = n_blk * ly.block_n + static_cast<int>(rank) * w_rows;
         for (int kb = 0; kb < ly.num_kb; ++kb) {
+          if (kb == ly.skip0) kb += ly.nskip;
           if (tr) { const long long t = clock64(); mbar_wait_role(&empty_bar[stage], phase ^ 1); w_empty += clock64() - t; }
           else mbar_wait_role(&empty_bar[stage], phase ^ 1);
           uint8_t* sa = smem + stage * L::kStage;
           if (leader) mbar_arrive_expect_tx(&full_bar[stage], bytes_pair);
           if (tr) t_issue[stage] = clock64();
-          tma_load_2d_pair(sa + L::kA, &p.tm_w[kind], lead_full + stage * 8, kb * kBlockK, w_row);
-          tma_load_2d_pair(sa, &p.tm_a[kind], lead_full + stage * 8, kb * kBlockK, a_row);
+          tma_load_2d_pair(sa + L::kA, &p.tm_w[w_layer(kind)], lead_full + stage * 8, ly.w_k0 + kb * kBlockK, w_row);
+          tma_load_2d_pair(sa, &p.tm_a[kind], lead_full + stage * 8, ly.a_k0 + kb * kBlockK, a_row);
           if (++stage == kP2Stages) { stage = 0; phase ^= 1; }
         }
       }
@@ -448,8 +487,8 @@
       long long w_full = 0, w_tmem = 0, w_item = 0, n_kb = 0, lat_sum = 0, lat_n = 0, lat_max = 0;
       int n_it = 0;
 #if PBG_KB_PROBE
-      long long pr_clk[5] = {0, 0, 0, 0, 0}, pr_item = 0, pr_tmem = 0;
-      int pr_tiles[5] = {0, 0, 0, 0, 0};
+      long long pr_clk[IT_KINDS] = {}, pr_item = 0, pr_tmem = 0;
+      int pr_tiles[IT_KINDS] = {};
       const long long pr_begin = clock64();
 #endif
       for (;;) {
@@ -479,6 +518,8 @@
         ++n_it;
         const uint32_t d_tmem = tmem_base + acc * 256;
         for (int kb = 0; kb < ly.num_kb; ++kb) {
+          if (kb == ly.skip0) kb += ly.nskip;
+          const bool first = kb == (ly.skip0 == 0 ? ly.nskip : 0);
           if (tr) {
             const long long t = clock64(); mbar_wait_role(&full_bar[stage], phase); const long long t1 = clock64();
             w_full += t1 - t; ++n_kb;
@@ -490,7 +531,7 @@
           const uint64_t da = make_kmajor_sw128_desc(sa);
           const uint64_t db = make_kmajor_sw128_desc(sa + L::kA);
 #pragma unroll
-          for (int k = 0; k < kBlockK / kUmmaK; ++k) umma_bf16_pair(d_tmem, da + 2 * k, db + 2 * k, idesc, (kb | k) != 0);
+          for (int k = 0; k < kBlockK / kUmmaK; ++k) umma_bf16_pair(d_tmem, da + 2 * k, db + 2 * k, idesc, !first || k != 0);
           umma_commit_pair(&empty_bar[stage], 3);
           if (++stage == kP2Stages) { stage = 0; phase ^= 1; }
         }
@@ -538,6 +579,13 @@
       if (lane == 0) g = atomicAdd(&p.sched->p0_next, 1);
       g = __shfl_sync(0xffffffffu, g, 0);
       if (g >= p.phase0_groups) { more_groups = false; return; }
+      if (g < p.rel_groups) {
+        rel_copy_group(p.gather, g, lane);
+        if (!p.gather_ahead) p2_arrive(p, DEP_REL, 0, lane, false);
+        else __syncwarp();
+        return;
+      }
+      g -= p.rel_groups;
       if (tr && threadIdx.x == kTraceThread) tr[249] = clock64();
       if (FASTG) {
         p2_gather_group_bulk(p.gather, g, lane, st, gather_flush, p.gather_ahead != 0);
@@ -556,6 +604,7 @@
       gather_flush();
     }
     bool bias_ok = !BIASS;
+    bool p_acquired = false;
     long long pf_wait = 0, pf_total = 0, pf_n = 0;
     bool pair_pending = false;
     auto pair_settle = [&]() {
@@ -614,6 +663,29 @@
           p2_tail_stage(st, tv1, lane);
         }
       }
+      const float* prow = nullptr;
+      if (ly.dep2 >= 0 && row_ok) {
+        long long pi = grow;
+        if (p.rel_table) {
+          if (p.rid != nullptr) {
+            pi = p.rid[grow];
+          } else {
+            pi = p.rel_idx[grow * p.rel_stride];
+            if (pi < 0 || pi >= p.n_rel) pi = 0;
+          }
+        }
+        prow = ly.prel + pi * ly.ldp + n0;
+      }
+      if (ly.dep2 >= 0) {
+        if (!p_acquired) {
+          if (lane == 0) (void)ld_acquire_gpu(p.ready + ly.dep2 * p.rb_cap);
+          __syncwarp();
+          p_acquired = true;
+        }
+        if (prow != nullptr)
+          for (int c = half * 2; c < 2 * n_chunks; c += ((c & 1) ? 2 * kP2Slots - 1 : 1))
+            asm volatile("prefetch.global.L1 [%0];" ::"l"(prow + c * 32));
+      }
       {
         const long long t = (tr && lane == 0) ? clock64() : 0;
         mbar_wait(&tmem_full[acc], acc_phase);
@@ -629,6 +701,26 @@
         const float slope = p.slope;
         const float* const bias_tile = (BIASS ? sbias + ly.bias_off : ly.bias) + n0;
         const int row0 = rb * kP2Rows + static_cast<int>(rank) * 128 + q * 32;
+        if (ly.dep2 >= 0) {
+          for (int c = half * 2; c < 2 * n_chunks; c += ((c & 1) ? 2 * kP2Slots - 1 : 1)) {
+            float4 pv[8];
+#pragma unroll
+            for (int t = 0; t < 8; ++t)
+              pv[t] = prow != nullptr ? __ldca(reinterpret_cast<const float4*>(prow + c * 32) + t) : make_float4(0.f, 0.f, 0.f, 0.f);
+            uint32_t v[32];
+            tmem_ld_32x32_ptr(taddr + c * 32, v);
+            tmem_ld_wait();
+#pragma unroll
+            for (int t = 0; t < 8; ++t) {
+              v[4 * t + 0] = __float_as_uint(__uint_as_float(v[4 * t + 0]) + pv[t].x);
+              v[4 * t + 1] = __float_as_uint(__uint_as_float(v[4 * t + 1]) + pv[t].y);
+              v[4 * t + 2] = __float_as_uint(__uint_as_float(v[4 * t + 2]) + pv[t].z);
+              v[4 * t + 3] = __float_as_uint(__uint_as_float(v[4 * t + 3]) + pv[t].w);
+            }
+            tmem_st_32x32_ptr(taddr + c * 32, v);
+          }
+          tmem_st_wait();
+        }
         uint32_t va[32], vb[32];
         if (half < n_chunks) tmem_ld_32x32_ptr(taddr + half * 64, va);
         for (int c = half; c < n_chunks; c += kP2Slots) {
@@ -702,6 +794,31 @@
         if (p.discard && kind == IT_G_L1 && n_blk == 0 && p.dead_xg != nullptr)
           p2_discard(static_cast<const char*>(p.dead_xg) + static_cast<size_t>(rb) * kP2Rows * p.dead_ldg * 2,
                      static_cast<size_t>(kP2Rows) * p.dead_ldg * 2, static_cast<int>(rank) * kP2Epi + wep, kP2WarpsPerPair, lane);
+      } else if (ly.epi == PEPI_F32) {
+        const long long prow_i = static_cast<long long>(rb) * kP2Rows + row_in_blk;
+        float* orow = ly.prel + prow_i * ly.ldp + n0;
+        for (int c = half; c < n_chunks; c += kP2Slots) {
+          uint32_t v[64];
+          tmem_ld_32x32_ptr(taddr + c * 64, v);
+          tmem_ld_32x32_ptr(taddr + c * 64 + 32, v + 32);
+          tmem_ld_wait();
+          if (c + kP2Slots >= n_chunks) {
+            tc_fence_before();
+            __syncwarp();
+            if (lane == 0) mbar_arrive_remote(lead_tmem_empty + acc * 8);
+          }
+          if (prow_i < ly.p_rows) {
+#pragma unroll
+            for (int t = 0; t < 16; ++t)
+              *reinterpret_cast<uint4*>(orow + c * 64 + 4 * t) = make_uint4(v[4 * t], v[4 * t + 1], v[4 * t + 2], v[4 * t + 3]);
+          }
+        }
+        if (half >= n_chunks) {
+          tc_fence_before();
+          __syncwarp();
+          if (lane == 0) mbar_arrive_remote(lead_tmem_empty + acc * 8);
+        }
+        p2_arrive(p, ly.out_kind, p2_dep_index(p, ly.out_kind, rb), lane, false);
       } else if (ly.epi == PEPI_ROWDOT) {
         const float slope = p.slope;
         float* part = p.part_d + (static_cast<size_t>(rb) * p.slots_d) * kP2Rows;
diff --git a/pro-b-gan_b200/csrc/pass_common.cuh b/pro-b-gan_b200/csrc/pass_common.cuh
--- a/pro-b-gan_b200/csrc/pass_common.cuh
+++ b/pro-b-gan_b200/csrc/pass_common.cuh
@@ -6,10 +6,10 @@
 
 namespace pbg {
 
-enum : int { IT_G_L0 = 0, IT_D_L0 = 1, IT_G_L1 = 2, IT_D_L1 = 3, IT_G_L2 = 4, IT_GATHER = 5, IT_END = 255 };
-enum : int { DEP_X = 0, DEP_G0 = 1, DEP_D0 = 2, DEP_G1 = 3, DEP_KINDS = 4 };
+enum : int { IT_G_L0 = 0, IT_D_L0 = 1, IT_G_L1 = 2, IT_D_L1 = 3, IT_G_L2 = 4, IT_G_R = 5, IT_D_R = 6, IT_KINDS = 7, IT_END = 255 };
+enum : int { DEP_X = 0, DEP_G0 = 1, DEP_D0 = 2, DEP_G1 = 3, DEP_REL = 4, DEP_PG = 5, DEP_PD = 6, DEP_KINDS = 7 };
 enum : int { FIN_G = 0, FIN_D = 1, FIN_KINDS = 2 };
-enum : int { PEPI_STORE = 0, PEPI_TANH = 1, PEPI_ROWDOT = 2 };
+enum : int { PEPI_STORE = 0, PEPI_TANH = 1, PEPI_ROWDOT = 2, PEPI_F32 = 3 };
 
 constexpr int kEpiWarps = 8;
 constexpr int kPassThreads = 64 + 32 * kEpiWarps;
@@ -32,6 +32,11 @@
 __device__ __forceinline__ int ld_relaxed_gpu(const int* p) {
   int v;
   asm volatile("ld.relaxed.gpu.global.s32 %0, [%1];" : "=r"(v) : "l"(p) : "memory");
+  return v;
+}
+__device__ __forceinline__ int ld_acquire_gpu(const int* p) {
+  int v;
+  asm volatile("ld.acquire.gpu.global.s32 %0, [%1];" : "=r"(v) : "l"(p) : "memory");
   return v;
 }
 __device__ __forceinline__ void fence_acq_rel_gpu() { asm volatile("fence.acq_rel.gpu;" ::: "memory"); }
@@ -88,7 +93,10 @@
         if (g.heads) { long long i = g.heads[row * g.head_stride]; if (i < 0) i += g.N; if (i < 0 || i >= g.N) { bad = true; i = 0; } src = g.node_emb + i * g.E; }
         else src = g.h + row * g.E;
       } else if (which == 1) {
-        if (g.rels) { long long i = g.rels[row * g.rel_stride]; if (i < 0 || i >= g.R) { bad = true; i = 0; } src = g.rel_emb + i * g.E; }
+        if (g.rels) {
+          long long i = g.rels[row * g.rel_stride]; if (i < 0 || i >= g.R) { bad = true; i = 0; } src = g.rel_emb + i * g.E;
+          if (g.rid) g.rid[row] = static_cast<int>(i);
+        }
         else src = g.r + row * g.E;
       } else if (g.tails) {
         long long i = g.tails[row * g.tail_stride]; if (i < 0) i += g.N; if (i < 0 || i >= g.N) { bad = true; i = 0; } src = g.node_emb + i * g.E;
diff --git a/pro-b-gan_b200/csrc/pbg.cu b/pro-b-gan_b200/csrc/pbg.cu
--- a/pro-b-gan_b200/csrc/pbg.cu
+++ b/pro-b-gan_b200/csrc/pbg.cu
@@ -31,6 +31,7 @@
 constexpr long long kMaxChunk = 65536;
 constexpr int kPartSlotsG = 16;
 constexpr int kPartSlotsD = 64;
+constexpr int kRelTableCap = 512;
 
 inline int round_up(int v, int m) { return (v + m - 1) / m * m; }
 
@@ -50,6 +51,8 @@
   void *xg0 = nullptr, *xd0 = nullptr, *bufA = nullptr, *bufB = nullptr, *bufD = nullptr;
   CUtensorMap tm_xg0, tm_xd0, tm_bufA_g, tm_bufA_d, tm_bufB_g, tm_bufD_d;
   CUtensorMap tmo_bufA, tmo_bufB, tmo_bufD;
+  __nv_bfloat16* relc = nullptr; CUtensorMap tm_relc;
+  float *prel_g = nullptr, *prel_d = nullptr;
   int mb_cap = 0;
   int* ready = nullptr;
   int* fin = nullptr;
@@ -75,6 +78,9 @@
   float* xt = nullptr;
   float* z = nullptr;
   CUtensorMap tm_xg0, tm_xd0;
+  __nv_bfloat16* relc = nullptr; CUtensorMap tm_relc;
+  int* rid = nullptr;
+  int rel_rows = 0;
   long long B = -1;
   bool has_g = false, has_d = false;
   bool has_xt = false;
@@ -95,6 +101,7 @@
   int max_threads_sm = 0;
   bool g_loaded = false, d_loaded = false;
   int kg0 = 0, kg0p = 0, kd0 = 0, kd0p = 0, hgp = 0, hdp = 0, hd2 = 0, hmax = 0;
+  bool fold = false;
   Linear g[3], d[2];
   float* d_w3 = nullptr;
   float* d_w3_pad = nullptr;
@@ -186,6 +193,7 @@
 void free_ws(Workspace& w) {
   cudaFree(w.xg0); cudaFree(w.xd0); cudaFree(w.bufA); cudaFree(w.bufB); cudaFree(w.bufD);
   cudaFree(w.ready); cudaFree(w.fin); cudaFree(w.sched); cudaFree(w.part_g); cudaFree(w.part_d);
+  cudaFree(w.relc); cudaFree(w.prel_g); cudaFree(w.prel_d);
   w = Workspace{};
 }
 
@@ -231,7 +239,7 @@
 }
 
 void free_stage(StageSlot& st) {
-  cudaFree(st.xg0); cudaFree(st.xd0); cudaFree(st.xt); cudaFree(st.z);
+  cudaFree(st.xg0); cudaFree(st.xd0); cudaFree(st.xt); cudaFree(st.z); cudaFree(st.relc); cudaFree(st.rid);
   st = StageSlot{};
 }
 
@@ -266,6 +274,12 @@
     PBG_TRY(make_tmap(c, &w.tm_bufA_g, w.bufA, cap, c->hgp, kBlockM));
     PBG_TRY(make_tmap(c, &w.tm_bufA_d, w.bufA, cap, c->hdp, kBlockM));
     PBG_TRY(make_tmap(c, &w.tm_bufB_g, w.bufB, cap, c->hgp, kBlockM));
+    if (c->fold) {
+      PBG_TRY(realloc_dev(c, w.relc, sizeof(__nv_bfloat16) * kRelTableCap * c->dims.embed_dim));
+      PBG_TRY(realloc_dev(c, w.prel_g, sizeof(float) * cap * c->hgp));
+      PBG_TRY(realloc_dev(c, w.prel_d, sizeof(float) * cap * c->hdp));
+      PBG_TRY(make_tmap(c, &w.tm_relc, w.relc, kRelTableCap, c->dims.embed_dim, kBlockM));
+    }
   } else {
     const size_t es = sizeof(float);
     const int hm = std::max(std::max(c->dims.g_hidden, c->dims.d_hidden), c->dims.embed_dim);
@@ -290,6 +304,11 @@
   PBG_CUDA(c, cudaMalloc(&st.z, sizeof(float) * cap * c->dims.noise_dim));
   PBG_TRY(make_tmap(c, &st.tm_xg0, st.xg0, cap, c->kg0p, kBlockM));
   PBG_TRY(make_tmap(c, &st.tm_xd0, st.xd0, cap, c->kd0p, kBlockM));
+  if (c->fold) {
+    PBG_TRY(realloc_dev(c, st.relc, sizeof(__nv_bfloat16) * kRelTableCap * c->dims.embed_dim));
+    PBG_TRY(realloc_dev(c, st.rid, sizeof(int) * cap));
+    PBG_TRY(make_tmap(c, &st.tm_relc, st.relc, kRelTableCap, c->dims.embed_dim, kBlockM));
+  }
   st.cap = cap;
   return PBG_OK;
 }
@@ -466,8 +485,24 @@
   p.tm_a[k] = amap;
   p.tm_w[k] = bn == 256 ? l.tmap_w128 : l.tmap_w64;
   if (omap) p.tm_o[k] = *omap;
-  p.layer[k] = P2Layer{l.kp / kBlockK, bn, l.np / bn, kEpiOf[k], kPredOf[k], kOutOf[k], ldo, -1, l.b_pad, out};
+  p.layer[k] = P2Layer{l.kp / kBlockK, bn, l.np / bn, kEpiOf[k], kPredOf[k], kOutOf[k], ldo, -1, l.b_pad, out,
+                       0, 0, -1, 0, -1, nullptr, 0, 0};
   p.layer_mask |= 1u << k;
+}
+
+void set_fold(const pbg_ctx* c, Pass2Params& p, int k, const CUtensorMap& rmap, bool table, float* prel, int p_rows) {
+  const int E = c->dims.embed_dim, kr = k == IT_G_L0 ? IT_G_R : IT_D_R;
+  P2Layer& l0 = p.layer[k];
+  l0.skip0 = E / kBlockK; l0.nskip = E / kBlockK;
+  l0.dep2 = k == IT_G_L0 ? DEP_PG : DEP_PD;
+  l0.prel = prel; l0.ldp = l0.n_tiles * l0.block_n;
+  P2Layer r = l0;
+  r.num_kb = E / kBlockK; r.epi = PEPI_F32; r.dep_kind = table ? DEP_REL : DEP_X; r.out_kind = l0.dep2;
+  r.ldo = 0; r.bias_off = -1; r.bias = nullptr; r.out = nullptr;
+  r.a_k0 = table ? 0 : E; r.w_k0 = E; r.skip0 = -1; r.nskip = 0; r.dep2 = -1; r.p_rows = p_rows;
+  p.layer[kr] = r;
+  p.tm_a[kr] = rmap;
+  p.layer_mask |= 1u << kr;
 }
 
 int launch_pass2(pbg_ctx* c, Workspace& w, const Pass& a, const GatherParams& gp, long long off, long long rows,
@@ -479,8 +514,14 @@
   const CUtensorMap* amap[5] = {slot ? &slot->tm_xg0 : &w.tm_xg0, slot ? &slot->tm_xd0 : &w.tm_xd0, &w.tm_bufA_g, &w.tm_bufD_d,
                                 &w.tm_bufB_g};
   const CUtensorMap* omap[5] = {&w.tmo_bufA, &w.tmo_bufD, &w.tmo_bufB, nullptr, nullptr};
-  const bool on[5] = {a.run_g, a.run_d, a.run_g, a.run_d, a.run_g};
+  const bool on[IT_KINDS] = {a.run_g, a.run_d, a.run_g, a.run_d, a.run_g, a.run_g && c->fold, a.run_d && c->fold};
   const int nrb = static_cast<int>((rows + kP2Rows - 1) / kP2Rows);
+  GatherParams g = gp;
+  int rel_rows = 0;
+  if (c->fold && slot) rel_rows = slot->rel_rows;
+  else if (c->fold && !external_gather && gp.rels && gp.R >= 1 && gp.R <= kRelTableCap) rel_rows = round_up(static_cast<int>(gp.R), kP2Rows);
+  const bool table = rel_rows > 0;
+  const int rel_nrb = table ? rel_rows / kP2Rows : nrb;
   __nv_bfloat16* outs[5] = {(__nv_bfloat16*)w.bufA, (__nv_bfloat16*)w.bufD, (__nv_bfloat16*)w.bufB, nullptr, nullptr};
   const int ldos[5] = {c->hgp, c->hdp, c->hgp, 0, 0};
   long long total = 0;
@@ -490,6 +531,19 @@
     if (p.layer[k].n_tiles > 255) return fail(c, PBG_ERR_UNSUPPORTED, "layer too wide for the tile index");
     total += static_cast<long long>(nrb) * p.layer[k].n_tiles;
   }
+  for (int k = IT_G_L0; k <= IT_D_L0; ++k) {
+    if (!on[k] || !c->fold) continue;
+    const CUtensorMap& rmap = !table ? *amap[k] : slot ? slot->tm_relc : w.tm_relc;
+    set_fold(c, p, k, rmap, table, k == IT_G_L0 ? w.prel_g : w.prel_d, table ? rel_rows : static_cast<int>(rows));
+    total += static_cast<long long>(rel_nrb) * p.layer[k].n_tiles;
+  }
+  p.rel_table = table ? 1 : 0; p.rel_nrb = rel_nrb;
+  if (table && slot) {
+    p.rid = slot->rid;
+  } else if (table) {
+    g.relc = w.relc; g.rel_rows = rel_rows;
+    p.rel_idx = a.rels + off * a.rs; p.rel_stride = a.rs; p.n_rel = a.R;
+  }
   bool biass = false;
   {
     int off = 0;
@@ -500,10 +554,11 @@
   }
   if (on[IT_D_L1] && lin[IT_D_L1]->np / 64 > kPartSlotsD) return fail(c, PBG_ERR_UNSUPPORTED, "d_hidden too wide for the partial buffer");
   if (on[IT_G_L2] && lin[IT_G_L2]->np / 64 > kPartSlotsG / 2) return fail(c, PBG_ERR_UNSUPPORTED, "embed_dim too wide for the partial buffer");
-  p.phase0_groups = external_gather ? 0 : nrb * kP2GroupsPerBlock;
+  p.rel_groups = g.relc ? g.rel_rows / 4 : 0;
+  p.phase0_groups = external_gather ? 0 : p.rel_groups + nrb * kP2GroupsPerBlock;
   p.gather_external = external_gather ? 1 : 0;
   if (gather_ahead) {
-    p.phase0_groups = static_cast<int>((gp.B + 3) / 4);
+    p.phase0_groups = p.rel_groups + static_cast<int>((gp.B + 3) / 4);
     p.gather_ahead = 1;
   }
   {
@@ -518,6 +573,8 @@
       p.seg[p.n_seg++] = P2Segment{k, p.layer[k].n_tiles, start, rb_lo, nt2 ? k2 : k, nt2};
       start += (rb_hi - rb_lo) * (p.layer[k].n_tiles + nt2);
     };
+    add_seg(IT_G_R, 0, rel_nrb);
+    add_seg(IT_D_R, 0, rel_nrb);
     for (int wv = 0; wv < waves; ++wv) {
       const int rb_lo = static_cast<int>(static_cast<long long>(nrb) * wv / waves);
       const int rb_hi = static_cast<int>(static_cast<long long>(nrb) * (wv + 1) / waves);
@@ -534,7 +591,7 @@
     if (start != total) return fail(c, PBG_ERR_INVALID, "internal: static item list does not cover the pass");
     p.n_total = start;
   }
-  p.gather = gp;
+  p.gather = g;
   static const int poll_env = [] { const char* e = getenv("PBG_POLL_NS"); return e ? atoi(e) : 40; }();
   p.poll_ns = poll_env;
   static const int defer_env = [] { const char* e = getenv("PBG_GATHER_DEFER"); return e ? atoi(e) : 1; }();
@@ -899,6 +956,7 @@
   c->hgp = round_up(HG, 128); c->hdp = round_up(HD, 128);
   c->hd2 = HD / 2;
   c->hmax = std::max(c->hgp, c->hdp);
+  c->fold = E % kBlockK == 0;
   auto bail = [&](int code) { g_create_error = c->err; pbg_destroy(c); return code; };
   if (cudaSetDevice(dims->device) != cudaSuccess) { c->err = "cudaSetDevice failed"; return bail(PBG_ERR_CUDA); }
   e = cudaSuccess;
@@ -1108,6 +1166,9 @@
   gp.xg = gen ? st.xg0 : nullptr; gp.ldg = c->kg0p;
   gp.xd = disc ? st.xd0 : nullptr; gp.ldd = c->kd0p;
   gp.B = B; gp.err_flag = c->err_flag;
+  if (c->fold && R >= 1 && R <= kRelTableCap) {
+    gp.rid = st.rid; gp.relc = st.relc; gp.rel_rows = round_up(static_cast<int>(R), kP2Rows);
+  }
   return gp;
 }
 
@@ -1151,7 +1212,7 @@
   { LaunchScope ls(c, PBG_K_GATHER, s);
     stage_rows_kernel<<<blocks, 128, 0, s>>>(sp); }
   PBG_CUDA(c, cudaGetLastError());
-  st.B = B; st.has_g = want_gen != 0; st.has_d = want_disc != 0; st.has_xt = want_gen != 0;
+  st.B = B; st.has_g = want_gen != 0; st.has_d = want_disc != 0; st.has_xt = want_gen != 0; st.rel_rows = sp.g.rel_rows;
   st.node_emb = node_emb; st.N = N; st.tails = t + 2;
   return PBG_OK;
 }
@@ -1191,7 +1252,7 @@
   const GatherParams gp = slot_gather(c, nx, node_emb, N, rel_emb, R, t, next_z, next_B, a.run_g, a.run_d);
   PBG_TRY(launch_pass2(c, c->ws_bf16, a, gp, 0, a.B, gen_out, gen_scores, true, &st, true));
   st.B = -1;
-  nx.B = next_B; nx.has_g = a.run_g; nx.has_d = a.run_d; nx.has_xt = false;
+  nx.B = next_B; nx.has_g = a.run_g; nx.has_d = a.run_d; nx.has_xt = false; nx.rel_rows = gp.rel_rows;
   nx.node_emb = node_emb; nx.N = N; nx.tails = t + 2;
   return PBG_OK;
 }
@@ -1234,6 +1295,18 @@
   }
   p.w3_off = -1;
   const int grid = pass_grid(c) & ~1;
+  const bool fold = c->fold && (k == IT_G_L0 || k == IT_D_L0);
+  if (fold) {
+    const int kr = k == IT_G_L0 ? IT_G_R : IT_D_R;
+    set_fold(c, p, k, amap, false, k == IT_G_L0 ? w.prel_g : w.prel_d, static_cast<int>(M));
+    p.seg[0] = P2Segment{kr, p.layer[kr].n_tiles, 0, 0, kr, 0};
+    cudaError_t le;
+    { LaunchScope ls(c, model == 0 ? PBG_K_G_L0 : PBG_K_D_L0, s);
+      le = launch_pdl(false, kPass2[0], grid, kP2Threads, P2Smem::kTotal, s, p); }
+    if (le == cudaSuccess) le = cudaGetLastError();
+    if (le != cudaSuccess) return fail(c, PBG_ERR_CUDA, "single-layer pass launch failed: %s", cudaGetErrorString(le));
+    p.seg[0] = P2Segment{k, p.layer[k].n_tiles, 0, 0, k, 0};
+  }
   cudaError_t le;
   { LaunchScope ls(c, model == 0 ? PBG_K_G_L0 + layer : PBG_K_D_L0 + layer, s);
     le = launch_pdl(false, kPass2[0], grid, kP2Threads, P2Smem::kTotal, s, p); }
```

After: 123.2 million, median of 6. 0.69x the previous value.
